# catree/InvCompCamTrack

Measured on AMD Instinct MI355X. Metric: aligned_Mpix_per_s (IC-GN, 1920x1080, 3-level pyramid), higher is better.
Workload: dtype f32; 1 GPU; R1080p-dense-se3: reference-faithful 6-DoF SE(3) tracker, 1920x1080, 3-level pyramid, 32400 8x8 patches tiling the frame, maxiter 10 fixed; points_per_pair_per_gpu=32400, psz=8, levels=3, maxiter=10, kernel_variant=0, collective=n/a, concurrent_streams=1, parallelism=single GPU

## Files before the change

include/ictr.h:

```cpp
#ifndef ICTR_H
#define ICTR_H

#include <stdbool.h>
#include <stddef.h>
#include <stdint.h>

#ifdef __cplusplus
extern "C" {
#endif

#define ICTR_OK 0
#define ICTR_ERR_INVALID 1
#define ICTR_ERR_NO_DEVICE 2
#define ICTR_ERR_HIP 3
#define ICTR_ERR_STATE 4

typedef struct ictr_optparam {
  int maxpttrack;
  int psz;
  int pszd2;
  int pszd2m3;
  int novals;
  int lv_f;
  int lv_l;
  bool donorm;
  bool dopatchnorm;
  int maxiter;
  float normdp_ratio;
  int verbosity;
} ictr_optparam;

int ictr_optparam_init(ictr_optparam *op, int lv_f, int lv_l, int psz, int maxiter, float normdp_ratio,
                       int donorm, int dopatchnorm, int maxpttrack, int verbosity);

const char *ictr_last_error(void);
int ictr_version(void);
int ictr_device_count(void);
int ictr_set_device(int device);
int ictr_stream_read_bandwidth(size_t bytes, int reps, double *gbps_out);
int ictr_debug_transpose_reduce(const float *vals, float *out, int *patch_of_lane, int *kind_of_lane,
                                int patches_per_wave );
int ictr_debug_wave_solve(const float *H36, const float *b6, int64_t n, int through_state, float *x6, int *rank,
                          int *nonzero, int *rowmap6, int *colmap6, float *lu36);
int ictr_debug_se3(const float *in, int64_t n, int log_not_exp, float *out);

typedef struct ictr_cam ictr_cam;
int ictr_cam_create(ictr_cam **out, int noscales, const float *fc, const float *cc, const int *wh, int padding);
void ictr_cam_destroy(ictr_cam *cam);
float ictr_cam_getfx(const ictr_cam *cam, int sc);
float ictr_cam_getfy(const ictr_cam *cam, int sc);
float ictr_cam_getcx(const ictr_cam *cam, int sc);
float ictr_cam_getcy(const ictr_cam *cam, int sc);
float ictr_cam_getswo(const ictr_cam *cam, int sc);
float ictr_cam_getsho(const ictr_cam *cam, int sc);
float ictr_cam_getsw(const ictr_cam *cam, int sc);
float ictr_cam_getsh(const ictr_cam *cam, int sc);

void ictr_se3_coeff_to_group_f(float *G12, const float *p6);
void ictr_se3_coeff_to_group_d(double *G12, const double *p6);
void ictr_se3_group_to_coeff_f(float *p6, const float *G12);
void ictr_se3_group_to_coeff_d(double *p6, const double *G12);
void ictr_solve6(const float *H36, const float *b6, float *x6);

typedef struct ictr_pyramid ictr_pyramid;
int ictr_pyramid_create(ictr_pyramid **out, const float *img, int w, int h, int lv_f, int getgrad, int pad);
int ictr_pyramid_create_device(ictr_pyramid **out, const float *img_dev, int w, int h, int lv_f, int getgrad,
                               int pad, void *hip_stream);
int ictr_pyramid_rebuild_device(ictr_pyramid *pyr, const float *img_dev, void *hip_stream);
int ictr_pyramid_rebuild(ictr_pyramid *pyr, const float *img, void *hip_stream);
int ictr_pyramid_create_from_host_planes(ictr_pyramid **out, const float **img_pyr, const float **dx_pyr,
                                         const float **dy_pyr, int w, int h, int lv_f, int pad);
void ictr_pyramid_destroy(ictr_pyramid *pyr);
int ictr_pyramid_levels(const ictr_pyramid *pyr);
int ictr_pyramid_level_dims(const ictr_pyramid *pyr, int level, int *sw, int *sh);
int ictr_pyramid_download(const ictr_pyramid *pyr, int level, int which, float *host_out);
const float *ictr_pyramid_device_plane(const ictr_pyramid *pyr, int level, int which);

int ictr_get_patch(const ictr_pyramid *pyr, int level, const float *mids, int64_t K, int psz, int dopatchnorm,
                   float *out);
int ictr_get_patch_grad(const ictr_pyramid *pyr, int level, const float *mids, int64_t K, int psz, int dopatchnorm,
                        float *out, float *out_dx, float *out_dy);
int ictr_ncc_score(const ictr_pyramid *pyr_back, const ictr_pyramid *pyr_ref, const ictr_pyramid *pyr_fwd, int level,
                   const float *mids, int64_t K, int psz, float w_back, float w_fwd, float *out_corr);

typedef struct ictr_pose ictr_pose;
int ictr_pose_create(ictr_pose **out, const ictr_cam *cam, const ictr_optparam *op);
void ictr_pose_destroy(ictr_pose *pose);
int ictr_pose_setpose_se3(ictr_pose *pose, const double *p_in, const double *meanshift3, double varval);
int ictr_pose_addpose_se3(ictr_pose *pose, const float *dp6);
int ictr_pose_subpose_se3(ictr_pose *pose, const float *dp6);
int ictr_pose_getpose_se3(const ictr_pose *pose, double *p_out6);
int ictr_pose_project_pt(const ictr_pose *pose, const float *pt3d, float *pt2d, int64_t nopoints, int sc);
int ictr_pose_project_pt_save_rotated(const ictr_pose *pose, const float *pt3d, float *pt3d_rot, float *pt2d,
                                      int64_t nopoints, int sc);
int ictr_pose_get_state(const ictr_pose *pose, float *p6, float *G12);

typedef struct ictr_odometer ictr_odometer;
int ictr_odometer_create(ictr_odometer **out, ictr_pose *pose, const ictr_optparam *op);
void ictr_odometer_destroy(ictr_odometer *odo);
int ictr_odometer_set3dpoints(ictr_odometer *odo, double *pt_in, int64_t nopoints_in);
int ictr_odometer_setpose(ictr_odometer *odo, const double *p_in, const ictr_pyramid *pyr_ref,
                          const ictr_pyramid *pyr_new);
int ictr_odometer_setpose_host(ictr_odometer *odo, const double *p_in, const float **img_ref,
                               const float **img_ref_dx, const float **img_ref_dy, const float **img_new);
int ictr_odometer_trackpose(ictr_odometer *odo, double *p_out);
const float *ictr_odometer_get2dpoints(ictr_odometer *odo);
int ictr_odometer_set_stream(ictr_odometer *odo, void *hip_stream);

typedef struct ictr_trace_rec {
  int level;
  int iter;
  float H[36];
  float b[6];
  float dp[6];
  float p[6];
} ictr_trace_rec;
int ictr_odometer_enable_trace(ictr_odometer *odo, int enable);
int ictr_odometer_trace(ictr_odometer *odo, ictr_trace_rec *out, int64_t capacity, int64_t *count);
int ictr_odometer_read_buffer(ictr_odometer *odo, int which, float *host_out, int64_t count);
int ictr_odometer_get_norm(const ictr_odometer *odo, double *meanshift3, double *varval);
#define ICTR_VARIANT_ANY_SIZE 0x2
#define ICTR_VARIANT_H_BY_SETUP 0x100
#define ICTR_VARIANT_LAUNCHES 0x2000
#define ICTR_VARIANT_ONE_LAUNCH 0x4000
#define ICTR_VARIANT_NO_GRAPH 0x8000
#define ICTR_VARIANT_SEPARATE_BEGIN 0x40000
#define ICTR_VARIANT_NO_TEAMS 0x80000
#define ICTR_VARIANT_NO_RESIDENT 0x200000
#define ICTR_VARIANT_DEBUG_MUTE 0x2000000
#define ICTR_VARIANT_GRAD_PLANES 0x8000000
#define ICTR_VARIANT_DYNAMIC_LOOP 0x10000000
#define ICTR_VARIANT_ALL                                                                                            \
  (ICTR_VARIANT_ANY_SIZE | ICTR_VARIANT_H_BY_SETUP | ICTR_VARIANT_LAUNCHES | ICTR_VARIANT_ONE_LAUNCH |              \
   ICTR_VARIANT_NO_GRAPH | ICTR_VARIANT_SEPARATE_BEGIN | ICTR_VARIANT_NO_TEAMS | ICTR_VARIANT_NO_RESIDENT |         \
   ICTR_VARIANT_DEBUG_MUTE | ICTR_VARIANT_GRAD_PLANES | ICTR_VARIANT_DYNAMIC_LOOP)
int ictr_odometer_set_variant(ictr_odometer *odo, int variant);
int ictr_odometer_set_team(ictr_odometer *odo, int target_points, int min_points, int max_points);
int ictr_odometer_set_robust(ictr_odometer *odo, int flags, float huber_k);
int ictr_odometer_last_path(const ictr_odometer *odo);
int ictr_odometer_last_team(const ictr_odometer *odo);

typedef struct ictr_batch ictr_batch;
int ictr_batch_create(ictr_batch **out, const ictr_cam *cam, const ictr_optparam *op, int64_t nproblems);
void ictr_batch_destroy(ictr_batch *b);
int ictr_batch_set_stream(ictr_batch *b, void *hip_stream);
int ictr_batch_set3dpoints(ictr_batch *b, int64_t problem, double *pt_in, int64_t nopoints_in);
int ictr_batch_set3dpoints_norm(ictr_batch *b, int64_t problem, double *pt_in, int64_t nopoints_in,
                                const double *meanshift3, double varval);
int ictr_batch_get_norm(const ictr_batch *b, int64_t problem, double *meanshift3, double *varval);
int ictr_batch_setpose(ictr_batch *b, int64_t problem, const double *p_in, const ictr_pyramid *pyr_ref,
                       const ictr_pyramid *pyr_new);
int ictr_batch_setpose_all(ictr_batch *b, const double *p_all, const ictr_pyramid *pyr_ref,
                           const ictr_pyramid *pyr_new);
int ictr_batch_track_async(ictr_batch *b);
int ictr_batch_get_poses(ictr_batch *b, double *p_out);
int ictr_batch_get_iterations(ictr_batch *b, int *iters);
int ictr_batch_get2dpoints(ictr_batch *b, int64_t problem, float *host_out );
int ictr_batch_set_variant(ictr_batch *b, int variant);
int ictr_batch_set_team(ictr_batch *b, int target_points, int min_points, int max_points);
#define ICTR_ROBUST_CLEAN 1
#define ICTR_ROBUST_COMPOSE 2
#define ICTR_ROBUST_HUBER 4
int ictr_batch_set_robust(ictr_batch *b, int flags, float huber_k);
int ictr_batch_read_buffer(ictr_batch *b, int64_t problem, int which, float *host_out, int64_t count);
int ictr_batch_set_timing(ictr_batch *b, int enable);
int ictr_batch_get_level_times(ictr_batch *b, float *ms_setup, float *ms_iters);
int ictr_batch_get_kernel_times(ictr_batch *b, float *ms_kernel);
int ictr_batch_get_first_iter_times(ictr_batch *b, float *ms_first);
int ictr_timebase_mark(void);
int ictr_batch_get_kernel_intervals(ictr_batch *b, float *start_ms, float *end_ms);
int ictr_batch_get_setup_intervals(ictr_batch *b, float *start_ms, float *end_ms);
int ictr_batch_last_path(const ictr_batch *b);
int ictr_batch_last_team(const ictr_batch *b);

int ictr_batch_enable_sharding(ictr_batch *b, int enable);
float *ictr_batch_reduction_buffer(ictr_batch *b);
int ictr_batch_set_reduction_buffer(ictr_batch *b, float *dev_ptr);
int ictr_batch_begin(ictr_batch *b);
int ictr_batch_level_allreduce_needed(ictr_batch *b);
int ictr_batch_level_accumulate(ictr_batch *b, int level);
int ictr_batch_level_finish(ictr_batch *b, int level);
int ictr_batch_iter_accumulate(ictr_batch *b, int level);
int ictr_batch_iter_finish(ictr_batch *b, int level);

int ictr_flow_gather(const void *disp_u, const void *disp_v, int is_f64, int fields_on_device, int H, int W,
                     const double *xy, int64_t K, double *out);
int ictr_extract_bil_patches(const double *img, int H, int W, int C, const double *pts, int64_t K, int pz, double *out);

typedef struct ictr_p2p ictr_p2p;
int ictr_p2p_create(ictr_p2p **out, int rank, int world, int64_t count );
int ictr_p2p_handle_bytes(void);
int ictr_p2p_local_handle(ictr_p2p *p, void *handle_out);
int ictr_p2p_connect(ictr_p2p *p, const void *all_handles);
int ictr_p2p_allreduce(ictr_p2p *p, float *dev_buf, int64_t count, void *hip_stream);
int ictr_p2p_error(ictr_p2p *p);
void ictr_p2p_destroy(ictr_p2p *p);
int ictr_batch_set_peer_exchange(ictr_batch *b, ictr_p2p *p);

int ictr_patchflow(const ictr_pyramid *pyr_a, const ictr_pyramid *pyr_b, const float *pts, int64_t K, int psz, int lv_f,
                   int lv_l, int maxiter, float eps, float *out, int *status, int *iters);
float ictr_patchflow_last_kernel_ms(void);

typedef struct ictr_icgn ictr_icgn;
#define ICTR_WARP_TRANSLATION 0
#define ICTR_WARP_SE2 1
#define ICTR_WARP_AFFINE 2
#define ICTR_WARP_HOMOGRAPHY 3
int ictr_icgn_create(ictr_icgn **out, int model, int w, int h, int lv_f, int lv_l, int maxiter, float eps,
                     const int *region_xywh, int64_t nproblems);
void ictr_icgn_destroy(ictr_icgn *g);
int ictr_icgn_set_stream(ictr_icgn *g, void *hip_stream);
int ictr_icgn_set_frames(ictr_icgn *g, int64_t problem, const ictr_pyramid *tmpl, const ictr_pyramid *cur);
int ictr_icgn_set_warp(ictr_icgn *g, int64_t problem, const double *M9);
int ictr_icgn_set_timing(ictr_icgn *g, int enable);
int ictr_icgn_run_async(ictr_icgn *g);
int ictr_icgn_get_results(ictr_icgn *g, double *M9_out, int *iters, float *last_dp);
int ictr_icgn_get_kernel_times(ictr_icgn *g, float *ms_per_level);
int ictr_icgn_set_rows(ictr_icgn *g, int row_lo, int row_hi);
int ictr_icgn_enable_sharding(ictr_icgn *g, int enable, float *red_dev );
int ictr_icgn_begin(ictr_icgn *g);
int ictr_icgn_hess_accumulate(ictr_icgn *g, int level);
int ictr_icgn_hess_finish(ictr_icgn *g, int level);
int ictr_icgn_iter_accumulate(ictr_icgn *g, int level);
int ictr_icgn_iter_finish(ictr_icgn *g, int level);

typedef struct ictr_sequence ictr_sequence;
int ictr_sequence_create(ictr_sequence **out, const ictr_cam *cam, const ictr_optparam *op, int64_t nworld, int stride);
void ictr_sequence_destroy(ictr_sequence *s);
int ictr_sequence_set_points(ictr_sequence *s, const double *pt3d);
int ictr_sequence_set_frames(ictr_sequence *s, const float *frames, int64_t nframes, int w, int h, int on_device);
int ictr_sequence_set_stream(ictr_sequence *s, void *hip_stream);
int ictr_sequence_set_robust(ictr_sequence *s, int flags, float huber_k);
int ictr_sequence_track_async(ictr_sequence *s, const double *p0);
int ictr_sequence_wait(ictr_sequence *s, double *poses, int32_t *npts, int32_t *iters);
int ictr_sequence_selection_hashes(const ictr_sequence *s, uint64_t *out);
int ictr_sequence_last_team(const ictr_sequence *s);

typedef struct ictr_ransac ictr_ransac;
int ictr_ransac_create(ictr_ransac **out, int64_t n, int64_t max_samples);
void ictr_ransac_destroy(ictr_ransac *r);
int ictr_ransac_set_points(ictr_ransac *r, const double *pt2d, const double *pt3d);
int ictr_ransac_run(ictr_ransac *r, const double *fc, const double *cc, double kc, int64_t nsamples, int64_t maxtrials,
                    double inlthresh, uint64_t seed, void *hip_stream);
int ictr_ransac_wait(ictr_ransac *r, int64_t *counts, double *R, double *t, double *p, uint64_t *inl_words,
                     int32_t *inl_cnt);
int ictr_ransac_samples(const ictr_ransac *r, int64_t *trial, int32_t *draws);
int ictr_ransac_chunk_size(const ictr_ransac *r);

#define ICTR_TRIANG_DLT 0
#define ICTR_TRIANG_GN 1
#define ICTR_TRIANG_LM 2
#define ICTR_TRIANG_DEPTH 3
#define ICTR_TRIANG_NONFINITE 1
#define ICTR_TRIANG_BEHIND 2
typedef struct ictr_triang_params {
  int32_t noiter;
  float minres;
  float damp_init, damp_fct, maxdamp;
} ictr_triang_params;
typedef struct ictr_triang ictr_triang;
int ictr_triang_create(ictr_triang **out, int64_t max_points, int64_t max_obs, int64_t max_frames);
void ictr_triang_destroy(ictr_triang *t);
int ictr_triang_set_cameras(ictr_triang *t, const float *P, int64_t nframes);
int ictr_triang_set_tracks(ictr_triang *t, int64_t n, const int64_t *offsets, const int32_t *view, const float *x,
                           const float *y);
int ictr_triang_run(ictr_triang *t, int mode, const ictr_triang_params *params, const float *init_pts,
                    const float *campos, const float *ptdir, void *hip_stream);
int ictr_triang_wait(ictr_triang *t, float *pts, float *cov, int32_t *iters, int32_t *status);
int ictr_triangulate_DLT(float *pt3d, float *AtAinv, const float *pt2d, const float *P, const int noviews);
int ictr_triangulate_full3D(float *pt3d, float *pt3d_cov, const float *pt2d, const float *P, const int noviews,
                            const int noiter, const float minres);
int ictr_triangulate_full3D_LM(float *pt3d, float *pt3d_cov, const float *pt2d, const float *P, const int noviews,
                               const int noiter, const float damp_init, const float damp_fct, const float minres,
                               const float maxdamp);
int ictr_triangulate_depthonly(float *pt3d, float *depth_cov, const float *campos, const float *ptdir, const float *pt2d,
                               const float *P, const int noviews, const int noiter, const float minres);

#ifdef __cplusplus
}
#endif
#endif
```

invcompcamtrack_amd/_lib.py:

```python
from __future__ import annotations

import ctypes as C
import os

import numpy as np

_HERE = os.path.dirname(os.path.abspath(__file__))
LIB_PATH = os.path.join(_HERE, "libictr_hip.so")

FP = C.POINTER(C.c_float)
DP = C.POINTER(C.c_double)
IP = C.POINTER(C.c_int)
FPP = C.POINTER(FP)
VP = C.c_void_p
I64 = C.c_int64


class IctrError(RuntimeError):
    pass


VARIANT_ANY_SIZE = 1 << 1
VARIANT_H_BY_SETUP = 1 << 8
VARIANT_LAUNCHES = 1 << 13
VARIANT_ONE_LAUNCH = 1 << 14
VARIANT_NO_GRAPH = 1 << 15
VARIANT_SEPARATE_BEGIN = 1 << 18
VARIANT_NO_TEAMS = 1 << 19
VARIANT_NO_RESIDENT = 1 << 21
VARIANT_DEBUG_MUTE = 1 << 25
VARIANT_GRAD_PLANES = 1 << 27
VARIANT_DYNAMIC_LOOP = 1 << 28
VARIANT_ALL = (VARIANT_ANY_SIZE | VARIANT_H_BY_SETUP | VARIANT_LAUNCHES | VARIANT_ONE_LAUNCH | VARIANT_NO_GRAPH
               | VARIANT_SEPARATE_BEGIN | VARIANT_NO_TEAMS | VARIANT_NO_RESIDENT | VARIANT_DEBUG_MUTE
               | VARIANT_GRAD_PLANES | VARIANT_DYNAMIC_LOOP)


class OptParam(C.Structure):
    _fields_ = [("maxpttrack", C.c_int), ("psz", C.c_int), ("pszd2", C.c_int), ("pszd2m3", C.c_int),
                ("novals", C.c_int), ("lv_f", C.c_int), ("lv_l", C.c_int), ("donorm", C.c_bool),
                ("dopatchnorm", C.c_bool), ("maxiter", C.c_int), ("normdp_ratio", C.c_float),
                ("verbosity", C.c_int)]


class TraceRec(C.Structure):
    _fields_ = [("level", C.c_int), ("iter", C.c_int), ("H", C.c_float * 36), ("b", C.c_float * 6),
                ("dp", C.c_float * 6), ("p", C.c_float * 6)]


class TriangParams(C.Structure):
    _fields_ = [("noiter", C.c_int32), ("minres", C.c_float), ("damp_init", C.c_float), ("damp_fct", C.c_float),
                ("maxdamp", C.c_float)]


SIGNATURES = {
    "ictr_optparam_init": (C.c_int, [C.POINTER(OptParam), C.c_int, C.c_int, C.c_int, C.c_int, C.c_float, C.c_int,
                                     C.c_int, C.c_int, C.c_int]),
    "ictr_last_error": (C.c_char_p, []),
    "ictr_version": (C.c_int, []),
    "ictr_device_count": (C.c_int, []),
    "ictr_set_device": (C.c_int, [C.c_int]),
    "ictr_stream_read_bandwidth": (C.c_int, [C.c_size_t, C.c_int, C.POINTER(C.c_double)]),
    "ictr_debug_transpose_reduce": (C.c_int, [FP, FP, IP, IP, C.c_int]),
    "ictr_debug_wave_solve": (C.c_int, [FP, FP, I64, C.c_int, FP, IP, IP, IP, IP, FP]),
    "ictr_debug_se3": (C.c_int, [FP, I64, C.c_int, FP]),
    "ictr_cam_create": (C.c_int, [C.POINTER(VP), C.c_int, FP, FP, IP, C.c_int]),
    "ictr_cam_destroy": (None, [VP]),
    "ictr_cam_getfx": (C.c_float, [VP, C.c_int]),
    "ictr_cam_getfy": (C.c_float, [VP, C.c_int]),
    "ictr_cam_getcx": (C.c_float, [VP, C.c_int]),
    "ictr_cam_getcy": (C.c_float, [VP, C.c_int]),
    "ictr_cam_getswo": (C.c_float, [VP, C.c_int]),
    "ictr_cam_getsho": (C.c_float, [VP, C.c_int]),
    "ictr_cam_getsw": (C.c_float, [VP, C.c_int]),
    "ictr_cam_getsh": (C.c_float, [VP, C.c_int]),
    "ictr_se3_coeff_to_group_f": (None, [FP, FP]),
    "ictr_se3_coeff_to_group_d": (None, [DP, DP]),
    "ictr_se3_group_to_coeff_f": (None, [FP, FP]),
    "ictr_se3_group_to_coeff_d": (None, [DP, DP]),
    "ictr_solve6": (None, [FP, FP, FP]),
    "ictr_pyramid_create": (C.c_int, [C.POINTER(VP), FP, C.c_int, C.c_int, C.c_int, C.c_int, C.c_int]),
    "ictr_pyramid_create_device": (C.c_int, [C.POINTER(VP), VP, C.c_int, C.c_int, C.c_int, C.c_int, C.c_int, VP]),
    "ictr_pyramid_rebuild_device": (C.c_int, [VP, VP, VP]),
    "ictr_pyramid_rebuild": (C.c_int, [VP, FP, VP]),
    "ictr_pyramid_create_from_host_planes": (C.c_int, [C.POINTER(VP), FPP, FPP, FPP, C.c_int, C.c_int, C.c_int,
                                                       C.c_int]),
    "ictr_pyramid_destroy": (None, [VP]),
    "ictr_pyramid_levels": (C.c_int, [VP]),
    "ictr_pyramid_level_dims": (C.c_int, [VP, C.c_int, IP, IP]),
    "ictr_pyramid_download": (C.c_int, [VP, C.c_int, C.c_int, FP]),
    "ictr_pyramid_device_plane": (VP, [VP, C.c_int, C.c_int]),
    "ictr_get_patch": (C.c_int, [VP, C.c_int, FP, I64, C.c_int, C.c_int, FP]),
    "ictr_get_patch_grad": (C.c_int, [VP, C.c_int, FP, I64, C.c_int, C.c_int, FP, FP, FP]),
    "ictr_ncc_score": (C.c_int, [VP, VP, VP, C.c_int, FP, I64, C.c_int, C.c_float, C.c_float, FP]),
    "ictr_pose_create": (C.c_int, [C.POINTER(VP), VP, C.POINTER(OptParam)]),
    "ictr_pose_destroy": (None, [VP]),
    "ictr_pose_setpose_se3": (C.c_int, [VP, DP, DP, C.c_double]),
    "ictr_pose_addpose_se3": (C.c_int, [VP, FP]),
    "ictr_pose_subpose_se3": (C.c_int, [VP, FP]),
    "ictr_pose_getpose_se3": (C.c_int, [VP, DP]),
    "ictr_pose_project_pt": (C.c_int, [VP, FP, FP, I64, C.c_int]),
    "ictr_pose_project_pt_save_rotated": (C.c_int, [VP, FP, FP, FP, I64, C.c_int]),
    "ictr_pose_get_state": (C.c_int, [VP, FP, FP]),
    "ictr_odometer_create": (C.c_int, [C.POINTER(VP), VP, C.POINTER(OptParam)]),
    "ictr_odometer_destroy": (None, [VP]),
    "ictr_odometer_set3dpoints": (C.c_int, [VP, DP, I64]),
    "ictr_odometer_setpose": (C.c_int, [VP, DP, VP, VP]),
    "ictr_odometer_setpose_host": (C.c_int, [VP, DP, FPP, FPP, FPP, FPP]),
    "ictr_odometer_trackpose": (C.c_int, [VP, DP]),
    "ictr_odometer_get2dpoints": (FP, [VP]),
    "ictr_odometer_set_stream": (C.c_int, [VP, VP]),
    "ictr_odometer_enable_trace": (C.c_int, [VP, C.c_int]),
    "ictr_odometer_trace": (C.c_int, [VP, C.POINTER(TraceRec), I64, C.POINTER(I64)]),
    "ictr_odometer_read_buffer": (C.c_int, [VP, C.c_int, FP, I64]),
    "ictr_odometer_get_norm": (C.c_int, [VP, DP, DP]),
    "ictr_odometer_set_variant": (C.c_int, [VP, C.c_int]),
    "ictr_odometer_set_team": (C.c_int, [VP, C.c_int, C.c_int, C.c_int]),
    "ictr_odometer_set_robust": (C.c_int, [VP, C.c_int, C.c_float]),
    "ictr_odometer_last_path": (C.c_int, [VP]),
    "ictr_odometer_last_team": (C.c_int, [VP]),
    "ictr_batch_create": (C.c_int, [C.POINTER(VP), VP, C.POINTER(OptParam), I64]),
    "ictr_batch_destroy": (None, [VP]),
    "ictr_batch_set_stream": (C.c_int, [VP, VP]),
    "ictr_batch_set3dpoints": (C.c_int, [VP, I64, DP, I64]),
    "ictr_batch_set3dpoints_norm": (C.c_int, [VP, I64, DP, I64, DP, C.c_double]),
    "ictr_batch_get_norm": (C.c_int, [VP, I64, DP, DP]),
    "ictr_batch_setpose": (C.c_int, [VP, I64, DP, VP, VP]),
    "ictr_batch_setpose_all": (C.c_int, [VP, DP, VP, VP]),
    "ictr_batch_track_async": (C.c_int, [VP]),
    "ictr_batch_get_poses": (C.c_int, [VP, DP]),
    "ictr_batch_get_iterations": (C.c_int, [VP, IP]),
    "ictr_batch_get2dpoints": (C.c_int, [VP, I64, FP]),
    "ictr_batch_set_variant": (C.c_int, [VP, C.c_int]),
    "ictr_batch_set_team": (C.c_int, [VP, C.c_int, C.c_int, C.c_int]),
    "ictr_batch_set_robust": (C.c_int, [VP, C.c_int, C.c_float]),
    "ictr_batch_read_buffer": (C.c_int, [VP, I64, C.c_int, FP, I64]),
    "ictr_batch_set_timing": (C.c_int, [VP, C.c_int]),
    "ictr_batch_get_level_times": (C.c_int, [VP, FP, FP]),
    "ictr_batch_get_kernel_times": (C.c_int, [VP, FP]),
    "ictr_batch_get_first_iter_times": (C.c_int, [VP, FP]),
    "ictr_batch_last_path": (C.c_int, [VP]),
    "ictr_batch_last_team": (C.c_int, [VP]),
    "ictr_timebase_mark": (C.c_int, []),
    "ictr_batch_get_kernel_intervals": (C.c_int, [VP, FP, FP]),
    "ictr_batch_get_setup_intervals": (C.c_int, [VP, FP, FP]),
    "ictr_batch_set_reduction_buffer": (C.c_int, [VP, VP]),
    "ictr_batch_enable_sharding": (C.c_int, [VP, C.c_int]),
    "ictr_batch_reduction_buffer": (VP, [VP]),
    "ictr_batch_begin": (C.c_int, [VP]),
    "ictr_batch_level_allreduce_needed": (C.c_int, [VP]),
    "ictr_batch_level_accumulate": (C.c_int, [VP, C.c_int]),
    "ictr_batch_level_finish": (C.c_int, [VP, C.c_int]),
    "ictr_batch_iter_accumulate": (C.c_int, [VP, C.c_int]),
    "ictr_batch_iter_finish": (C.c_int, [VP, C.c_int]),
    "ictr_flow_gather": (C.c_int, [VP, VP, C.c_int, C.c_int, C.c_int, C.c_int, DP, I64, DP]),
    "ictr_extract_bil_patches": (C.c_int, [DP, C.c_int, C.c_int, C.c_int, DP, I64, C.c_int, DP]),
    "ictr_p2p_create": (C.c_int, [C.POINTER(VP), C.c_int, C.c_int, I64]),
    "ictr_p2p_handle_bytes": (C.c_int, []),
    "ictr_p2p_local_handle": (C.c_int, [VP, VP]),
    "ictr_p2p_connect": (C.c_int, [VP, VP]),
    "ictr_p2p_allreduce": (C.c_int, [VP, VP, I64, VP]),
    "ictr_p2p_error": (C.c_int, [VP]),
    "ictr_p2p_destroy": (None, [VP]),
    "ictr_batch_set_peer_exchange": (C.c_int, [VP, VP]),
    "ictr_patchflow": (C.c_int, [VP, VP, FP, I64, C.c_int, C.c_int, C.c_int, C.c_int, C.c_float, FP, IP, IP]),
    "ictr_patchflow_last_kernel_ms": (C.c_float, []),
    "ictr_icgn_create": (C.c_int, [C.POINTER(VP), C.c_int, C.c_int, C.c_int, C.c_int, C.c_int, C.c_int, C.c_float, IP,
                                   I64]),
    "ictr_icgn_destroy": (None, [VP]),
    "ictr_icgn_set_stream": (C.c_int, [VP, VP]),
    "ictr_icgn_set_frames": (C.c_int, [VP, I64, VP, VP]),
    "ictr_icgn_set_warp": (C.c_int, [VP, I64, DP]),
    "ictr_icgn_set_timing": (C.c_int, [VP, C.c_int]),
    "ictr_icgn_run_async": (C.c_int, [VP]),
    "ictr_icgn_get_results": (C.c_int, [VP, DP, IP, FP]),
    "ictr_icgn_get_kernel_times": (C.c_int, [VP, FP]),
    "ictr_icgn_set_rows": (C.c_int, [VP, C.c_int, C.c_int]),
    "ictr_icgn_enable_sharding": (C.c_int, [VP, C.c_int, VP]),
    "ictr_icgn_begin": (C.c_int, [VP]),
    "ictr_icgn_hess_accumulate": (C.c_int, [VP, C.c_int]),
    "ictr_icgn_hess_finish": (C.c_int, [VP, C.c_int]),
    "ictr_icgn_iter_accumulate": (C.c_int, [VP, C.c_int]),
    "ictr_icgn_iter_finish": (C.c_int, [VP, C.c_int]),
    "ictr_sequence_create": (C.c_int, [C.POINTER(VP), VP, C.POINTER(OptParam), I64, C.c_int]),
    "ictr_sequence_destroy": (None, [VP]),
    "ictr_sequence_set_points": (C.c_int, [VP, DP]),
    "ictr_sequence_set_frames": (C.c_int, [VP, VP, I64, C.c_int, C.c_int, C.c_int]),
    "ictr_sequence_set_stream": (C.c_int, [VP, VP]),
    "ictr_sequence_set_robust": (C.c_int, [VP, C.c_int, C.c_float]),
    "ictr_sequence_track_async": (C.c_int, [VP, DP]),
    "ictr_sequence_wait": (C.c_int, [VP, DP, C.POINTER(C.c_int32), C.POINTER(C.c_int32)]),
    "ictr_sequence_selection_hashes": (C.c_int, [VP, C.POINTER(C.c_uint64)]),
    "ictr_sequence_last_team": (C.c_int, [VP]),
    "ictr_ransac_create": (C.c_int, [C.POINTER(VP), I64, I64]),
    "ictr_ransac_destroy": (None, [VP]),
    "ictr_ransac_set_points": (C.c_int, [VP, DP, DP]),
    "ictr_ransac_run": (C.c_int, [VP, DP, DP, C.c_double, I64, I64, C.c_double, C.c_uint64, VP]),
    "ictr_ransac_wait": (C.c_int, [VP, C.POINTER(I64), DP, DP, DP, C.POINTER(C.c_uint64), C.POINTER(C.c_int32)]),
    "ictr_ransac_samples": (C.c_int, [VP, C.POINTER(I64), C.POINTER(C.c_int32)]),
    "ictr_ransac_chunk_size": (C.c_int, [VP]),
    "ictr_triang_create": (C.c_int, [C.POINTER(VP), I64, I64, I64]),
    "ictr_triang_destroy": (None, [VP]),
    "ictr_triang_set_cameras": (C.c_int, [VP, FP, I64]),
    "ictr_triang_set_tracks": (C.c_int, [VP, I64, C.POINTER(I64), C.POINTER(C.c_int32), FP, FP]),
    "ictr_triang_run": (C.c_int, [VP, C.c_int, C.POINTER(TriangParams), FP, FP, FP, VP]),
    "ictr_triang_wait": (C.c_int, [VP, FP, FP, C.POINTER(C.c_int32), C.POINTER(C.c_int32)]),
    "ictr_triangulate_depthonly": (C.c_int, [FP, FP, FP, FP, FP, FP, C.c_int, C.c_int, C.c_float]),
}
SIGNATURES_REFERENCE_NAMES = {
    "ictr_triangulate_DLT": (C.c_int, [FP, FP, FP, FP, C.c_int]),
    "ictr_triangulate_full3D": (C.c_int, [FP, FP, FP, FP, C.c_int, C.c_int, C.c_float]),
    "ictr_triangulate_full3D_LM": (C.c_int, [FP, FP, FP, FP, C.c_int, C.c_int, C.c_float, C.c_float, C.c_float,
                                             C.c_float]),
}

_lib = None


def _preload_torch_hip_runtime():
    if os.environ.get("ICTR_SYSTEM_HIP") == "1":
        return None
    import sys
    tlib = None
    if "torch" in sys.modules:
        tlib = os.path.join(os.path.dirname(sys.modules["torch"].__file__), "lib", "libamdhip64.so")
    else:
        import importlib.util
        spec = importlib.util.find_spec("torch")
        if spec is not None and spec.origin:
            tlib = os.path.join(os.path.dirname(spec.origin), "lib", "libamdhip64.so")
    if tlib and os.path.exists(tlib):
        try:
            return C.CDLL(tlib, mode=C.RTLD_GLOBAL)
        except OSError:
            return None
    return None


def load():
    global _lib
    if _lib is not None:
        return _lib
    if not os.path.exists(LIB_PATH):
        raise IctrError(f"{LIB_PATH} not found: build it with `python -c 'import __graft_entry__ as g; g.build()'` "
                        "(hipcc --offload-arch=gfx950). There is no CPU fallback.")
    _preload_torch_hip_runtime()
    try:
        L = C.CDLL(LIB_PATH)
    except OSError as exc:
        raise IctrError(f"cannot load {LIB_PATH}: {exc}") from exc
    for name, (res, args) in list(SIGNATURES.items()) + list(SIGNATURES_REFERENCE_NAMES.items()):
        fn = getattr(L, name)
        fn.restype = res
        fn.argtypes = args
    _lib = L
    return L


def check(rc):
    if rc != 0:
        msg = load().ictr_last_error()
        raise IctrError(f"ictr error {rc}: {msg.decode() if msg else '?'}")


def fp(a):
    return a.ctypes.data_as(FP)


def dp(a):
    return a.ctypes.data_as(DP)


def f32c(a):
    return np.ascontiguousarray(a, dtype=np.float32)


def f64c(a):
    return np.ascontiguousarray(a, dtype=np.float64)
```

invcompcamtrack_amd/csrc/ictr_dev.h:

```cpp
#pragma once

#include <hip/hip_runtime.h>
#include <stdint.h>

#include "../../include/ictr.h"

namespace ictr {

constexpr int kBlock = 256;
constexpr int kWaves = kBlock / 64;
constexpr int kCoefStride = 16;
constexpr int kHUnique = 21;
constexpr int kRedStride = 27;
constexpr int kPartHStride = 32;
constexpr int kPartBStride = 8;
constexpr int kMaxGridX = 2048;

struct LevelCam {
  float fx, fy, cx, cy, swo, sho;
  int sw;
};

struct PlaneSet {
  const float *ref, *dx, *dy, *cur;
  const float *pack;
};

struct ProbState {
  float p[6];
  float G[12];
  float H[36];
  float LU[36];
  int piv[12];
  int luinfo[2];
  float b[6];
  float dp[6];
  float normdp;
  float normdp_init;
  int it;
  int active;
  int total_iters;
  int npts;
  unsigned reserved_;
  int pad_;
};

constexpr int kXchgMaxWorld = 16;
constexpr int kXchgPerPair = 64;
struct ResXchg {
  unsigned long long *peer[kXchgMaxWorld];
  unsigned long long *local;
  int rank, world;
  long long cap;
  unsigned *xseq;
};

struct DevTrace {
  ictr_trace_rec *rec;
  int *count;
  int capacity;
  int reserved_;
};

struct EngineDev {
  int B, M, P, n, nlev;
  int lv_f, lv_l, maxiter;
  float ratio;
  int dopatchnorm;
  int sharded;
  int otf;
  int robust;
  float huber_k;
  float *pt3d;
  float *pt3d_ref;
  float *pt2d;
  float *T, *Gx, *Gy;
  float *coef;
  ProbState *st;
  const PlaneSet *planes;
  float *partH;
  float *partb;
  float *red;
  DevTrace trace;
};

constexpr int kSeqBlock = 256;
constexpr int kSeqPPT = 16;
constexpr int kSeqChunk = kSeqBlock * kSeqPPT;
constexpr int kSeqFinish = 256;
struct SeqState {
  double pose[6];
  double G[12];
  double ms[3], varval;
  int npts;
  int pad_[3];
};
struct SeqArgs {
  const double *X;
  long long nw;
  int nblk;
  int stride, cap, M, n, donorm;
  int t;
  int tail;
  double fx, fy, cx, cy, w, h;
  double p0[6];
  ProbState *st;
  SeqState *ss;
  unsigned long long *mask;
  unsigned *cnt;
  int *sel;
  double *poses;
  unsigned long long *hash;
  int *npts_out, *iters_out;
  float *pt3d, *T, *Gx, *Gy, *coef;
};

constexpr int kRanHypBlock = 64;
constexpr int kRanScoreBlock = 256;
constexpr int kRanSelBlock = 1024;
constexpr int kRanMaxDraws = 1024;
struct RansacState {
  long long held;
  long long trials_used;
  long long kept;
  long long n_ic;
  int done;
  int pad_[3];
};
struct RansacArgs {
  const double *pts;
  int n, nwords;
  double fx, fy, cx, cy, kc, thr;
  unsigned long long seedmix;
  long long base;
  int k;
  long long nsamples, maxtrials;
  double *hyp;
  int *draws;
  int *status;
  unsigned *cnt;
  unsigned long long *words;
  RansacState *st;
  long long *o_trial;
  int *o_draws;
  double *o_R, *o_t;
  unsigned long long *o_words;
  int *o_cnt;
  int *o_keep;
  int *o_cntf;
};

struct PFLevel {
  const float *a, *ax, *ay, *b;
  int sw;
  float swo, sho, scale;
};
struct PFArgs {
  PFLevel lv[16];
  int lv_f, lv_l, P, maxiter, K;
  float eps2;
  float min_det;
  const float *pts;
  float *out;
  int *status;
  int *iters;
};

}
```

invcompcamtrack_amd/csrc/ictr_host.hip:

```cpp
#include <math.h>
#include <stdarg.h>
#include <stdio.h>
#include <stdlib.h>
#include <string.h>

#include <algorithm>
#include <atomic>
#include <deque>
#include <map>
#include <mutex>
#include <string>
#include <vector>

#include "ictr_dev.h"
#include "ictr_launch.h"
#include "se3_math.h"
#include "ictr_pose_hd.h"

using namespace ictr;

static thread_local std::string g_err;
int ictr::fail(int code, const char *fmt, ...) {
  char buf[512];
  va_list ap;
// ... 461 lines not shown
  if (e != hipSuccess) return fail(ICTR_ERR_HIP, "ncc_score failed: %s", hipGetErrorString(e));
  return ICTR_OK;
}

extern "C" int ictr_flow_gather(const void *disp_u, const void *disp_v, int is_f64, int fields_on_device, int H, int W,
                                const double *xy, int64_t K, double *out) {
  if (!disp_u || H < 1 || W < 1 || K < 0 || (K > 0 && (!xy || !out)))
    return fail(ICTR_ERR_INVALID, "flow_gather: bad arguments");
  if (K == 0) return ICTR_OK;
  if (int rc = need_device()) return rc;
  const size_t fb = (size_t)H * W * (is_f64 ? 8 : 4);
  char *d_f = nullptr;
  double *d_xy = nullptr;
  hipError_t e = hipMalloc((void **)&d_xy, sizeof(double) * 4 * K);
  const void *du = disp_u, *dv = disp_v;
  if (e == hipSuccess && !fields_on_device) {
    e = hipMalloc((void **)&d_f, fb * 2);
    if (e == hipSuccess) e = hipMemcpy(d_f, disp_u, fb, hipMemcpyHostToDevice);
    if (e == hipSuccess && disp_v) e = hipMemcpy(d_f + fb, disp_v, fb, hipMemcpyHostToDevice);
    du = d_f;
    dv = disp_v ? d_f + fb : nullptr;
  }
  if (e == hipSuccess) e = hipMemcpy(d_xy, xy, sizeof(double) * 2 * K, hipMemcpyHostToDevice);
  if (e == hipSuccess) {
    launch_flow_gather(du, dv, is_f64, H, W, d_xy, (int)K, d_xy + 2 * K, nullptr);
    e = hipMemcpy(out, d_xy + 2 * K, sizeof(double) * 2 * K, hipMemcpyDeviceToHost);
  }
  if (d_f) hipFree(d_f);
  if (d_xy) hipFree(d_xy);
  if (e != hipSuccess) return fail(ICTR_ERR_HIP, "flow_gather failed: %s", hipGetErrorString(e));
  return ICTR_OK;
}

extern "C" int ictr_extract_bil_patches(const double *img, int H, int W, int C, const double *pts, int64_t K, int pz,
                                        double *out) {
  const int half = pz / 2;
  if (!img || H < 2 || W < 2 || C < 1 || K < 0 || pz < 2 || (K > 0 && (!pts || !out)))
    return fail(ICTR_ERR_INVALID, "extract_bil_patches: bad arguments");
  for (int64_t k = 0; k < K; ++k) {
    const double fx = floor(pts[2 * k]), fy = floor(pts[2 * k + 1]);
    if (!(fx - half >= 0 && fy - half >= 0 && fx + half < W && fy + half < H))
      return fail(ICTR_ERR_INVALID, "extract_bil_patches: the window of point %lld leaves the image", (long long)k);
  }
  if (K == 0) return ICTR_OK;
  if (int rc = need_device()) return rc;
  const size_t ib = sizeof(double) * (size_t)H * W * C, ob = sizeof(double) * (size_t)K * 4 * half * half * C;
  double *d_img = nullptr, *d_pts = nullptr, *d_out = nullptr;
  hipError_t e = hipMalloc((void **)&d_img, ib);
  if (e == hipSuccess) e = hipMalloc((void **)&d_pts, sizeof(double) * 2 * K);
  if (e == hipSuccess) e = hipMalloc((void **)&d_out, ob);
  if (e == hipSuccess) e = hipMemcpy(d_img, img, ib, hipMemcpyHostToDevice);
  if (e == hipSuccess) e = hipMemcpy(d_pts, pts, sizeof(double) * 2 * K, hipMemcpyHostToDevice);
  if (e == hipSuccess) {
    launch_bil_patches(d_img, H, W, C, d_pts, (int)K, half, d_out, nullptr);
    e = hipMemcpy(out, d_out, ob, hipMemcpyDeviceToHost);
  }
  for (void *p_ : {(void *)d_img, (void *)d_pts, (void *)d_out})
    if (p_) hipFree(p_);
  if (e != hipSuccess) return fail(ICTR_ERR_HIP, "extract_bil_patches failed: %s", hipGetErrorString(e));
  return ICTR_OK;
}

struct ictr_pose {
  const ictr_cam *cam;
  const ictr_optparam *op;
  double meanshift[3] = {0, 0, 0};
  double varval = 0;
  float p[6] = {0, 0, 0, 0, 0, 0};
  float G[12] = {1, 0, 0, 0, 0, 1, 0, 0, 0, 0, 1, 0};
};

extern "C" int ictr_pose_create(ictr_pose **out, const ictr_cam *cam, const ictr_optparam *op) {
  if (!out || !cam || !op) return fail(ICTR_ERR_INVALID, "ictr_pose_create: NULL argument");
  ictr_pose *p = new ictr_pose;
  p->cam = cam;
  p->op = op;
  *out = p;
  return ICTR_OK;
}
extern "C" void ictr_pose_destroy(ictr_pose *pose) { delete pose; }
extern "C" int ictr_pose_setpose_se3(ictr_pose *pose, const double *p_in, const double *meanshift3, double varval) {
  if (!pose || !p_in) return fail(ICTR_ERR_INVALID, "setpose_se3: NULL argument");
  if (pose->op->donorm) {
    if (!meanshift3) return fail(ICTR_ERR_INVALID, "setpose_se3: donorm needs meanshift");
    pose->varval = varval;
    memcpy(pose->meanshift, meanshift3, sizeof(double) * 3);
  }
  host_setpose(pose->op->donorm, p_in, pose->meanshift, pose->varval, pose->p, pose->G);
  return ICTR_OK;
}
extern "C" int ictr_pose_addpose_se3(ictr_pose *pose, const float *dp) {
  if (!pose || !dp) return fail(ICTR_ERR_INVALID, "addpose_se3: NULL argument");
  for (int i = 0; i < 6; ++i) pose->p[i] += dp[i];
  se3_exp<float>(pose->G, pose->p);
  return ICTR_OK;
}
extern "C" int ictr_pose_subpose_se3(ictr_pose *pose, const float *dp) {
  if (!pose || !dp) return fail(ICTR_ERR_INVALID, "subpose_se3: NULL argument");
  for (int i = 0; i < 6; ++i) pose->p[i] -= dp[i];
  se3_exp<float>(pose->G, pose->p);
  return ICTR_OK;
}
extern "C" int ictr_pose_getpose_se3(const ictr_pose *pose, double *p_out) {
  if (!pose || !p_out) return fail(ICTR_ERR_INVALID, "getpose_se3: NULL argument");
  host_getpose(pose->op->donorm, pose->p, pose->G, pose->meanshift, pose->varval, p_out);
  return ICTR_OK;
}
extern "C" int ictr_pose_get_state(const ictr_pose *pose, float *p6, float *G12) {
  if (!pose) return fail(ICTR_ERR_INVALID, "pose is NULL");
  if (p6) memcpy(p6, pose->p, sizeof(float) * 6);
  if (G12) memcpy(G12, pose->G, sizeof(float) * 12);
  return ICTR_OK;
}

static int project_impl(const ictr_pose *pose, const float *pt3d, float *pt3d_rot, float *pt2d, int64_t nopoints,
                        int sc) {
  if (!pose || !pt3d || !pt2d || nopoints < 0 || sc < 0 || sc >= pose->cam->noscales)
    return fail(ICTR_ERR_INVALID, "project_pt: bad arguments");
  if (int rc = need_device()) return rc;
  const int M = pose->op->maxpttrack;
  if (nopoints > M) return fail(ICTR_ERR_INVALID, "project_pt: nopoints > maxpttrack");
  if (nopoints == 0) return ICTR_OK;
  float *d = nullptr;
  HIPCHK(hipMalloc((void **)&d, sizeof(float) * (size_t)(8 * M + 12)));
  float *d3 = d, *dr = d + 3 * M, *d2 = d + 6 * M, *dG = d + 8 * M;
  hipError_t e = hipMemcpy(d3, pt3d, sizeof(float) * 3 * M, hipMemcpyHostToDevice);
  if (e == hipSuccess) e = hipMemcpy(dG, pose->G, sizeof(float) * 12, hipMemcpyHostToDevice);
  if (e == hipSuccess) e = hipMemcpy(d2, pt2d, sizeof(float) * 2 * M, hipMemcpyHostToDevice);
  if (e == hipSuccess && pt3d_rot) e = hipMemcpy(dr, pt3d_rot, sizeof(float) * 3 * M, hipMemcpyHostToDevice);
  if (e == hipSuccess) {
    launch_project_generic(d3, pt3d_rot ? dr : nullptr, d2, (int)nopoints, M, dG, level_cam(pose->cam, sc), nullptr);
    e = hipMemcpy(pt2d, d2, sizeof(float) * 2 * M, hipMemcpyDeviceToHost);
    if (e == hipSuccess && pt3d_rot) e = hipMemcpy(pt3d_rot, dr, sizeof(float) * 3 * M, hipMemcpyDeviceToHost);
  }
  hipFree(d);
  if (e != hipSuccess) return fail(ICTR_ERR_HIP, "project_pt failed: %s", hipGetErrorString(e));
  return ICTR_OK;
}
extern "C" int ictr_pose_project_pt(const ictr_pose *pose, const float *pt3d, float *pt2d, int64_t nopoints, int sc) {
  return project_impl(pose, pt3d, nullptr, pt2d, nopoints, sc);
}
extern "C" int ictr_pose_project_pt_save_rotated(const ictr_pose *pose, const float *pt3d, float *pt3d_rot,
                                                 float *pt2d, int64_t nopoints, int sc) {
  if (!pt3d_rot) return fail(ICTR_ERR_INVALID, "project_pt_save_rotated: pt3d_rot is NULL");
  return project_impl(pose, pt3d, pt3d_rot, pt2d, nopoints, sc);
}

enum TrackForm : int {
  kFormLaunches = 0,
  kFormTrack1 = 1,
  kFormGraph = 2,
  kFormTrack1Begin = 3,
  kFormResident = 4,
};
struct TrackPlan {
  int form;
  int variant;
  int team, team_q;
  int project_here;
  int mute;
  ResidentGeom res;
  int setup_cpw[16], setup_gridx8[16];
};
struct Mailbox {
  unsigned long long *d = nullptr;
  size_t bytes = 0;
  unsigned epoch = 0;
};
struct ProbHost {
  int npts = 0;
  double meanshift[3] = {0, 0, 0};
  double varval = 0;
  float p[6] = {0, 0, 0, 0, 0, 0};
  float G[12] = {1, 0, 0, 0, 0, 1, 0, 0, 0, 0, 1, 0};
  const ictr_pyramid *ref = nullptr, *cur = nullptr;
  bool pose_set = false;
  int iters = 0;
};

struct ictr_batch {
  const ictr_cam *cam = nullptr;
  const ictr_optparam *op = nullptr;
  int B = 0, M = 0, n = 0, nlev = 0, P = 0;
  hipStream_t stream = nullptr;
  int variant = 0;
  int robust = 0;
  float huber_k = 0.0f;
  int sharded = 0;
  int gridx = 1;
  int cpw = 64, gridx8 = 1;
  bool trace_on = false;
  bool projected = false;
  float *d_pt3d = nullptr, *d_pt3d_ref = nullptr, *d_pt2d = nullptr, *d_T = nullptr, *d_Gx = nullptr,
        *d_Gy = nullptr, *d_coef = nullptr, *d_partH = nullptr, *d_partb = nullptr, *d_red = nullptr;
  ProbState *d_st = nullptr;
  PlaneSet *d_planes = nullptr;
  ictr_trace_rec *d_trace = nullptr;
  int *d_trace_count = nullptr;
  int trace_cap = 0;
  std::vector<ProbHost> probs;
  std::vector<ProbState> h_st;
  std::vector<PlaneSet> h_planes;
  std::vector<float> h_pt2d;
  std::vector<float> h_stage;
  bool timing = false;
  std::vector<hipEvent_t> ev;
  std::vector<char> ev_used;
  std::vector<hipEvent_t> evk;
  int evk_iters = 0;
  bool evk_valid = true;
  ResXchg xchg = {};
  unsigned *d_xseq = nullptr;
  int otf = 0;
  int maxpts = 0;
  TrackPlan plan = {};
  hipGraphExec_t gexec = nullptr;
  std::string gkey;
  hipStream_t cap_stream = nullptr;
  bool graph_broken = false;
  int phase_it = 0;
  float *d_red_own = nullptr;
  ProbState *h_st_pin = nullptr;
  ProbState *d_st_mirror = nullptr;
  char *h_up_pin = nullptr;
  Mailbox team_mail, res_mail;
  int team_target = 0;
  int team_lo = 128, team_hi = 8192;
  int *h_team_err = nullptr;
  int *d_team_err = nullptr;
  hipEvent_t done_ev = nullptr, up_ev = nullptr;
  bool done_valid = false, up_pending = false;
};

static size_t up_planes_offset(int B) { return (sizeof(ProbState) * (size_t)B + 15) / 16 * 16; }
int ictr::env_int(const char *name, int dflt) {
  const char *s = getenv(name);
  return s ? atoi(s) : dflt;
}

static void batch_free(ictr_batch *b) {
  if (!b) return;
  for (hipEvent_t e : b->ev) (void)hipEventDestroy(e);
  for (hipEvent_t e : b->evk) (void)hipEventDestroy(e);
  if (b->gexec) (void)hipGraphExecDestroy(b->gexec);
  if (b->cap_stream) (void)hipStreamDestroy(b->cap_stream);
  if (b->done_ev) (void)hipEventDestroy(b->done_ev);
  if (b->up_ev) (void)hipEventDestroy(b->up_ev);
  if (b->h_st_pin) (void)hipHostFree(b->h_st_pin);
  if (b->h_up_pin) (void)hipHostFree(b->h_up_pin);
  if (b->h_team_err) (void)hipHostFree(b->h_team_err);
  if (b->team_mail.d) (void)hipFree(b->team_mail.d);
  if (b->res_mail.d) (void)hipFree(b->res_mail.d);
  if (b->d_xseq) (void)hipFree(b->d_xseq);
  b->d_red = b->d_red_own;
  for (void *p : {(void *)b->d_pt3d, (void *)b->d_pt3d_ref, (void *)b->d_pt2d, (void *)b->d_T, (void *)b->d_Gx,
                  (void *)b->d_Gy, (void *)b->d_coef, (void *)b->d_partH, (void *)b->d_partb, (void *)b->d_red,
                  (void *)b->d_st, (void *)b->d_trace, (void *)b->d_trace_count})
    if (p) hipFree(p);
  delete b;
}

static int engine_variant(const ictr_batch *b) { return b->variant | (b->robust ? ICTR_VARIANT_ANY_SIZE : 0); }

static EngineDev engine_dev(const ictr_batch *b) {
  EngineDev e;
  memset(&e, 0, sizeof(e));
  e.B = b->B;
  e.M = b->M;
  e.P = b->P;
  e.n = b->n;
  e.nlev = b->nlev;
  e.lv_f = b->op->lv_f;
  e.lv_l = b->op->lv_l;
  e.maxiter = b->op->maxiter;
  e.ratio = b->op->normdp_ratio;
  e.dopatchnorm = b->op->dopatchnorm ? 1 : 0;
  e.sharded = b->sharded;
  e.otf = b->otf;
  e.robust = b->robust;
  e.huber_k = b->huber_k;
  e.pt3d = b->d_pt3d;
  e.pt3d_ref = b->d_pt3d_ref;
  e.pt2d = b->d_pt2d;
  e.T = b->d_T;
  e.Gx = b->d_Gx;
  e.Gy = b->d_Gy;
  e.coef = b->d_coef;
  e.st = b->d_st;
  e.planes = b->d_planes;
  e.partH = b->d_partH;
  e.partb = b->d_partb;
  e.red = b->d_red;
  e.trace.rec = b->trace_on ? b->d_trace : nullptr;
  e.trace.count = b->d_trace_count;
  e.trace.capacity = b->trace_cap;
  return e;
}

static int check_op(const ictr_optparam *op, const ictr_cam *cam) {
  if (op->psz < 1 || op->psz > 64) return fail(ICTR_ERR_INVALID, "psz must be 1..64");
  if (op->novals != op->psz * op->psz || op->pszd2 != op->psz / 2)
    return fail(ICTR_ERR_INVALID, "optparam derived fields inconsistent (use ictr_optparam_init)");
  if (op->lv_l < 0 || op->lv_f < op->lv_l || op->lv_f >= cam->noscales)
    return fail(ICTR_ERR_INVALID, "need 0 <= lv_l <= lv_f < cam.noscales");
  if (op->maxpttrack < 1) return fail(ICTR_ERR_INVALID, "maxpttrack must be >= 1");
  if (cam->padding < op->psz) return fail(ICTR_ERR_INVALID, "camera padding must be >= psz");
  return ICTR_OK;
}

extern "C" int ictr_batch_create(ictr_batch **out, const ictr_cam *cam, const ictr_optparam *op, int64_t nproblems) {
  if (!out || !cam || !op || nproblems < 1 || nproblems > 65535)
    return fail(ICTR_ERR_INVALID, "batch_create: bad arguments (1..65535 problems)");
  if (int rc = check_op(op, cam)) return rc;
  if (int rc = need_device()) return rc;
  ictr_batch *b = new ictr_batch;
  b->cam = cam;
  b->op = op;
  b->B = (int)nproblems;
  b->M = op->maxpttrack;
  b->P = op->psz;
  b->n = op->novals;
  b->nlev = op->lv_f + 1;
  b->team_target = env_int("ICTR_TEAM_TARGET", 0);
  b->team_lo = env_int("ICTR_TEAM_MINPTS", 128);
  b->team_hi = env_int("ICTR_TEAM_MAXPTS", 8192);
  const size_t B = b->B, M = b->M, n = b->n, L = b->nlev;
  const int ppw = (b->n <= 64 && 64 % b->n == 0) ? 64 / b->n : 1;
  const int64_t groups = (b->M + ppw - 1) / ppw;
  const int64_t cap = std::min<int64_t>(kMaxGridX, std::max<int64_t>(64, 2 * kMaxGridX / (int64_t)B));
  b->gridx = (int)std::min<int64_t>(std::max<int64_t>((groups + kWaves - 1) / kWaves, 1), cap);
  b->trace_cap = std::max(1, (int)L * std::max(1, op->maxiter));
  hipError_t e = hipSuccess;
  auto alloc = [&](void **p, size_t bytes) {
    if (e == hipSuccess) e = hipMalloc(p, bytes);
    if (e == hipSuccess) e = hipMemset(*p, 0, bytes);
  };
  alloc((void **)&b->d_pt3d, sizeof(float) * B * 3 * M);
  alloc((void **)&b->d_pt3d_ref, sizeof(float) * B * 3 * M);
  alloc((void **)&b->d_pt2d, sizeof(float) * B * L * 2 * M);
  alloc((void **)&b->d_T, sizeof(float) * B * M * n);
  alloc((void **)&b->d_Gx, sizeof(float) * B * M * n);
  alloc((void **)&b->d_Gy, sizeof(float) * B * M * n);
  alloc((void **)&b->d_coef, sizeof(float) * B * M * kCoefStride);
  alloc((void **)&b->d_partH, sizeof(float) * B * b->gridx * kPartHStride);
  alloc((void **)&b->d_partb, sizeof(float) * B * b->gridx * kPartBStride);
  alloc((void **)&b->d_red, sizeof(float) * B * kRedStride);
  alloc((void **)&b->d_st, up_planes_offset(B) + sizeof(PlaneSet) * B * L);
  if (e == hipSuccess) b->d_planes = reinterpret_cast<PlaneSet *>(reinterpret_cast<char *>(b->d_st) + up_planes_offset(B));
  alloc((void **)&b->d_trace, sizeof(ictr_trace_rec) * b->trace_cap);
  alloc((void **)&b->d_trace_count, sizeof(int));
  if (e == hipSuccess) e = hipHostMalloc((void **)&b->h_st_pin, sizeof(ProbState) * B, hipHostMallocDefault);
  if (e == hipSuccess)
    e = hipHostMalloc((void **)&b->h_up_pin, up_planes_offset(B) + sizeof(PlaneSet) * B * L, hipHostMallocDefault);
  if (e == hipSuccess && hipHostGetDevicePointer((void **)&b->d_st_mirror, b->h_st_pin, 0) != hipSuccess) {
    (void)hipGetLastError();
    b->d_st_mirror = nullptr;
  }
  if (e == hipSuccess) e = hipEventCreateWithFlags(&b->done_ev, hipEventDisableTiming);
  if (e == hipSuccess) e = hipEventCreateWithFlags(&b->up_ev, hipEventDisableTiming);
  if (e != hipSuccess) {
    batch_free(b);
    return fail(ICTR_ERR_HIP, "batch_create: device allocation failed: %s", hipGetErrorString(e));
  }
  b->d_red_own = b->d_red;
  b->probs.resize(B);
  b->h_st.resize(B);
  b->h_planes.resize(B * L);
  b->h_pt2d.assign(2 * M, 0.0f);
  b->h_stage.assign(3 * M, 0.0f);
  *out = b;
  return ICTR_OK;
}
extern "C" void ictr_batch_destroy(ictr_batch *b) { batch_free(b); }
extern "C" int ictr_batch_set_stream(ictr_batch *b, void *hip_stream) {
  if (!b) return fail(ICTR_ERR_INVALID, "batch is NULL");
  b->stream = (hipStream_t)hip_stream;
  return ICTR_OK;
}
extern "C" int ictr_batch_set_robust(ictr_batch *b, int flags, float huber_k) {
  if (!b) return fail(ICTR_ERR_INVALID, "batch is NULL");
  if (flags & ~(ICTR_ROBUST_CLEAN | ICTR_ROBUST_COMPOSE | ICTR_ROBUST_HUBER))
    return fail(ICTR_ERR_INVALID, "set_robust: unknown flag bits 0x%x", flags);
  if ((flags & ICTR_ROBUST_HUBER) && !(huber_k > 0.0f))
    return fail(ICTR_ERR_INVALID, "set_robust: the Huber threshold must be positive");
  b->robust = flags;
  b->huber_k = huber_k;
  return ICTR_OK;
}
extern "C" int ictr_batch_set_team(ictr_batch *b, int target_points, int min_points, int max_points) {
  if (!b) return fail(ICTR_ERR_INVALID, "batch is NULL");
  if (min_points < 0 || max_points < min_points)
    return fail(ICTR_ERR_INVALID, "set_team: need 0 <= min_points <= max_points");
  b->team_target = target_points;
  b->team_lo = min_points;
  b->team_hi = max_points;
  return ICTR_OK;
}
extern "C" int ictr_batch_set_peer_exchange(ictr_batch *b, ictr_p2p *p) {
  if (!b) return fail(ICTR_ERR_INVALID, "batch is NULL");
  if (!p) {
    memset(&b->xchg, 0, sizeof(b->xchg));
    return ICTR_OK;
  }
  ResXchg x;
  if (ictr_p2p_fill_xchg_(p, &x)) return fail(ICTR_ERR_STATE, "set_peer_exchange: the p2p object is not connected");
  if (x.cap < (long long)kXchgPerPair * b->B)
    return fail(ICTR_ERR_INVALID, "set_peer_exchange: the mailboxes hold %lld granules per rank, %d x %d needed", x.cap,
                kXchgPerPair, b->B);
  if (!b->d_xseq) HIPCHK(hipMalloc((void **)&b->d_xseq, sizeof(unsigned) * b->B));
  HIPCHK(hipMemsetAsync(b->d_xseq, 0, sizeof(unsigned) * b->B, b->stream));
  x.xseq = b->d_xseq;
  b->xchg = x;
  return ICTR_OK;
}

extern "C" int ictr_batch_set_variant(ictr_batch *b, int variant) {
  if (!b) return fail(ICTR_ERR_INVALID, "batch is NULL");
  if (variant & ~ICTR_VARIANT_ALL)
    return fail(ICTR_ERR_INVALID, "set_variant: unknown selection bits 0x%x (known: ICTR_VARIANT_ANY_SIZE, H_BY_SETUP, "
                                  "LAUNCHES, ONE_LAUNCH, NO_GRAPH, SEPARATE_BEGIN, NO_TEAMS, NO_RESIDENT, DEBUG_MUTE, "
                                  "GRAD_PLANES, DYNAMIC_LOOP = 0x%x)", variant & ~ICTR_VARIANT_ALL, ICTR_VARIANT_ALL);
  b->variant = variant;
  return ICTR_OK;
}

static int set3dpoints_impl(ictr_batch *b, int64_t problem, double *pt_in, int64_t nopoints_in, const double *given_ms,
                            double given_var) {
  if (!b || problem < 0 || problem >= b->B || nopoints_in < 0 || (nopoints_in > 0 && !pt_in))
    return fail(ICTR_ERR_INVALID, "set3dpoints: bad arguments");
  ProbHost &ph = b->probs[problem];
  const size_t M = b->M, n = b->n;
  HIPCHK(hipMemsetAsync(b->d_T + problem * M * n, 0, sizeof(float) * M * n, b->stream));
  HIPCHK(hipMemsetAsync(b->d_Gx + problem * M * n, 0, sizeof(float) * M * n, b->stream));
  HIPCHK(hipMemsetAsync(b->d_Gy + problem * M * n, 0, sizeof(float) * M * n, b->stream));
  HIPCHK(hipMemsetAsync(b->d_coef + problem * M * kCoefStride, 0, sizeof(float) * M * kCoefStride, b->stream));
  ph.meanshift[0] = ph.meanshift[1] = ph.meanshift[2] = 0;
  ph.varval = 0;
  ph.npts = (int)std::min<int64_t>(nopoints_in, b->M);
  ph.pose_set = false;
  const int np = ph.npts;
  double *p1 = pt_in, *p2 = pt_in + nopoints_in, *p3 = pt_in + 2 * nopoints_in;
  std::fill(b->h_stage.begin(), b->h_stage.end(), 0.0f);
  float *s = b->h_stage.data();
  if (b->op->donorm) {
    const double nd = (double)np;
    if (given_ms) {
      memcpy(ph.meanshift, given_ms, sizeof(double) * 3);
    } else {
      for (int i = 0; i < np; ++i) ph.meanshift[0] += p1[i];
      for (int i = 0; i < np; ++i) ph.meanshift[1] += p2[i];
      for (int i = 0; i < np; ++i) ph.meanshift[2] += p3[i];
      ph.meanshift[0] /= nd;
      ph.meanshift[1] /= nd;
      ph.meanshift[2] /= nd;
    }
    for (int i = 0; i < np; ++i) {
      p1[i] -= ph.meanshift[0];
      p2[i] -= ph.meanshift[1];
      p3[i] -= ph.meanshift[2];
      ph.varval += p1[i] * p1[i] + p2[i] * p2[i] + p3[i] * p3[i];
    }
    ph.varval /= nd;
    if (given_ms) ph.varval = given_var;
    for (int i = 0; i < np; ++i) {
      s[i] = (float)(p1[i] / ph.varval);
      s[i + M] = (float)(p2[i] / ph.varval);
      s[i + 2 * M] = (float)(p3[i] / ph.varval);
    }
  } else {
    for (int i = 0; i < np; ++i) {
      s[i] = (float)p1[i];
      s[i + M] = (float)p2[i];
      s[i + 2 * M] = (float)p3[i];
    }
  }
  HIPCHK(hipMemcpyAsync(b->d_pt3d + problem * 3 * M, s, sizeof(float) * 3 * M, hipMemcpyHostToDevice, b->stream));
  HIPCHK(hipStreamSynchronize(b->stream));
  return ICTR_OK;
}
extern "C" int ictr_batch_set3dpoints(ictr_batch *b, int64_t problem, double *pt_in, int64_t nopoints_in) {
  return set3dpoints_impl(b, problem, pt_in, nopoints_in, nullptr, 0.0);
}
extern "C" int ictr_batch_set3dpoints_norm(ictr_batch *b, int64_t problem, double *pt_in, int64_t nopoints_in,
                                           const double *meanshift3, double varval) {
  if (!meanshift3) return fail(ICTR_ERR_INVALID, "set3dpoints_norm: meanshift is NULL");
  return set3dpoints_impl(b, problem, pt_in, nopoints_in, meanshift3, varval);
}
extern "C" int ictr_batch_get_norm(const ictr_batch *b, int64_t problem, double *meanshift3, double *varval) {
  if (!b || problem < 0 || problem >= b->B) return fail(ICTR_ERR_INVALID, "get_norm: bad arguments");
  if (meanshift3) memcpy(meanshift3, b->probs[problem].meanshift, sizeof(double) * 3);
  if (varval) *varval = b->probs[problem].varval;
  return ICTR_OK;
}

extern "C" int ictr_batch_setpose(ictr_batch *b, int64_t problem, const double *p_in, const ictr_pyramid *pyr_ref,
                                  const ictr_pyramid *pyr_new) {
  if (!b || problem < 0 || problem >= b->B || !p_in || !pyr_ref || !pyr_new)
    return fail(ICTR_ERR_INVALID, "setpose: bad arguments");
  for (const ictr_pyramid *py : {pyr_ref, pyr_new}) {
    if (py->nlev < b->nlev || py->pad != b->cam->padding)
      return fail(ICTR_ERR_INVALID, "setpose: pyramid has %d levels / pad %d, engine needs %d / %d", py->nlev, py->pad,
                  b->nlev, b->cam->padding);
    for (int l = 0; l < b->nlev; ++l)
      if (py->sw[l] != (int)b->cam->sw[l] || py->sh[l] < (int)b->cam->sh[l])
        return fail(ICTR_ERR_INVALID, "setpose: pyramid level %d is %dx%d, camera expects %dx%d", l, py->sw[l],
                    py->sh[l], (int)b->cam->sw[l], (int)b->cam->sh[l]);
  }
  if (!pyr_ref->getgrad) return fail(ICTR_ERR_INVALID, "setpose: reference pyramid has no gradients");
  ProbHost &ph = b->probs[problem];
  host_setpose(b->op->donorm, p_in, ph.meanshift, ph.varval, ph.p, ph.G);
  ph.ref = pyr_ref;
  ph.cur = pyr_new;
  ph.pose_set = true;
  b->projected = false;
  return ICTR_OK;
}

extern "C" int ictr_batch_setpose_all(ictr_batch *b, const double *p_all, const ictr_pyramid *pyr_ref,
                                      const ictr_pyramid *pyr_new) {
  if (!b || !p_all) return fail(ICTR_ERR_INVALID, "setpose_all: bad arguments");
  for (int64_t k = 0; k < b->B; ++k)
    if (int rc = ictr_batch_setpose(b, k, p_all + 6 * k, pyr_ref, pyr_new)) return rc;
  return ICTR_OK;
}

static int cpw_forced() {
  const char *env = getenv("ICTR_CPW");
  const int v = env ? atoi(env) : 0;
  return v >= 1 && v <= 64 ? v : 0;
}
static int begin_prepare(ictr_batch *b) {
  if (int rc = check_op(b->op, b->cam)) return rc;
  if (b->op->maxpttrack != b->M || b->op->psz != b->P || b->op->lv_f + 1 != b->nlev)
    return fail(ICTR_ERR_STATE, "optparam maxpttrack/psz/lv_f changed after creation");
  b->done_valid = false;
  b->phase_it = 0;
  bool all_builder = true, any_image_only = false;
  if (b->timing) std::fill(b->ev_used.begin(), b->ev_used.end(), 0);
  int maxpts = 0;
  for (int i = 0; i < b->B; ++i) {
    const ProbHost &ph = b->probs[i];
    if (!ph.pose_set) return fail(ICTR_ERR_STATE, "problem %d: SetPose has not been called", i);
    ProbState &st = b->h_st[i];
    memset(&st, 0, sizeof(st));
    memcpy(st.p, ph.p, sizeof(st.p));
    memcpy(st.G, ph.G, sizeof(st.G));
    st.npts = ph.npts;
    st.normdp = st.normdp_init = 1e-10f;
    maxpts = std::max(maxpts, ph.npts);
    for (int l = 0; l < b->nlev; ++l) {
      PlaneSet &ps = b->h_planes[(size_t)i * b->nlev + l];
      ps.ref = ph.ref->img[l];
      ps.dx = ph.ref->dx[l];
      ps.dy = ph.ref->dy[l];
      ps.cur = ph.cur->img[l];
      ps.pack = ph.ref->pack[l];
    }
    if (!ph.ref->builder_made) all_builder = false;
    if (ph.ref->getgrad == 2) any_image_only = true;
  }
  if (any_image_only && !all_builder)
    return fail(ICTR_ERR_STATE, "a batch cannot mix image-only reference pyramids (getgrad = 2) with pyramids made from "
                                "caller-supplied planes: the setup kernel reads either the planes or the image, for all "
                                "problems of a launch");
  b->otf = !all_builder ? 0 : (any_image_only ? 2 : 1);

  b->maxpts = maxpts;
  {
    const int64_t total = (int64_t)std::max(maxpts, 1) * b->B;
    int cpw = 4;
    while (cpw < 64 && total / cpw > 32768) cpw *= 2;
    if (const int v = cpw_forced()) cpw = v;
    b->cpw = cpw;
    const int64_t chunks = ((int64_t)std::max(maxpts, 1) + cpw - 1) / cpw;
    const int64_t want = (chunks + kWaves - 1) / kWaves;
    const int64_t capx = std::max<int64_t>(1, (int64_t)b->gridx);
    b->gridx8 = (int)std::min<int64_t>(std::max<int64_t>(want, 1), capx);
    if (b->gridx8 >= 64)
      b->gridx8 = (int)std::min<int64_t>((b->gridx8 + 7) / 8 * 8, capx / 8 * 8);
  }
  if (b->otf == 2 && (b->P != 8 || b->robust || (engine_variant(b) & ICTR_VARIANT_ANY_SIZE)))
    return fail(ICTR_ERR_STATE, "a reference pyramid without gradient planes (getgrad = 2: gradients formed on the fly) is "
                                "served by the 8x8 setup kernel k_ref8 only: psz 8, no robustness option, variant bit 1 "
                                "clear (small problems then run the per-iteration launches instead of the one-launch "
                                "tracker)");
  return ICTR_OK;
}
static int begin_device(ictr_batch *b, bool project = true) {
  const int maxpts = project ? b->maxpts : 0;
  {
    const size_t nst = sizeof(ProbState) * b->B, npl = sizeof(PlaneSet) * b->h_planes.size();
    if (b->up_pending) HIPCHK(hipEventSynchronize(b->up_ev));
    const size_t off = up_planes_offset(b->B);
    memcpy(b->h_up_pin, b->h_st.data(), nst);
    memcpy(b->h_up_pin + off, b->h_planes.data(), npl);
    HIPCHK(hipMemcpyAsync(b->d_st, b->h_up_pin, off + npl, hipMemcpyHostToDevice, b->stream));
    HIPCHK(hipEventRecord(b->up_ev, b->stream));
    b->up_pending = true;
  }
  if (maxpts > 0) {
    LevelCam cams[16];
    for (int l = 0; l < b->nlev; ++l) cams[l] = level_cam(b->cam, l);
    launch_project_ref(engine_dev(b), cams, maxpts, b->stream);
  } else {
    HIPCHK(hipMemsetAsync(b->d_trace_count, 0, sizeof(int), b->stream));
  }
  HIPCHK(hipGetLastError());
  return ICTR_OK;
}
extern "C" int ictr_batch_begin(ictr_batch *b) {
  if (!b) return fail(ICTR_ERR_INVALID, "batch is NULL");
  if (int rc = begin_prepare(b)) return rc;
  if (int rc = begin_device(b)) return rc;
  b->projected = true;
  return ICTR_OK;
}

extern "C" int ictr_batch_enable_sharding(ictr_batch *b, int enable) {
  if (!b) return fail(ICTR_ERR_INVALID, "batch is NULL");
  b->sharded = enable ? 1 : 0;
  return ICTR_OK;
}
extern "C" float *ictr_batch_reduction_buffer(ictr_batch *b) { return b ? b->d_red : nullptr; }

static LevelLaunch level_launch(const ictr_batch *b, const TrackPlan *p, int level) {
  const bool res = p && p->form == kFormResident;
  LevelLaunch ll;
  ll.level = level;
  ll.variant = p ? p->variant : engine_variant(b);
  ll.gridx = b->gridx;
  ll.cpw = res ? p->setup_cpw[level] : b->cpw;
  ll.gridx8 = res ? p->setup_gridx8[level] : b->gridx8;
  return ll;
}
static int level_ok(ictr_batch *b, int level) {
  if (!b) return fail(ICTR_ERR_INVALID, "batch is NULL");
  if (!b->projected) return fail(ICTR_ERR_STATE, "ictr_batch_begin has not run since the last SetPose");
  if (level < b->op->lv_l || level > b->op->lv_f) return fail(ICTR_ERR_INVALID, "level out of range");
  return ICTR_OK;
}
extern "C" int ictr_batch_level_allreduce_needed(ictr_batch *b) {
  if (!b) return 1;
  return defer_h(engine_dev(b), engine_variant(b)) ? 0 : 1;
}
extern "C" int ictr_batch_level_accumulate(ictr_batch *b, int level) {
  if (int rc = level_ok(b, level)) return rc;
  b->phase_it = 0;
  launch_ref_level(engine_dev(b), level_cam(b->cam, level), level_launch(b, nullptr, level), true, b->stream);
  HIPCHK(hipGetLastError());
  return ICTR_OK;
}
extern "C" int ictr_batch_level_finish(ictr_batch *b, int level) {
  if (int rc = level_ok(b, level)) return rc;
  b->phase_it = 0;
  if (b->sharded) launch_level_finish(engine_dev(b), level_launch(b, nullptr, level), b->stream);
  HIPCHK(hipGetLastError());
  return ICTR_OK;
}
extern "C" int ictr_batch_iter_accumulate(ictr_batch *b, int level) {
  if (int rc = level_ok(b, level)) return rc;
  const bool tk = b->timing && b->phase_it < b->evk_iters && (int)b->evk.size() >= 2 * b->nlev * b->evk_iters;
  const EngineDev e = engine_dev(b);
  const LevelCam lc = level_cam(b->cam, level);
  const LevelLaunch ll = level_launch(b, nullptr, level);
  const int first = b->phase_it == 0;
  const int ke = 2 * (level * b->evk_iters + b->phase_it);
  launch_iter_main(e, lc, ll, first, b->stream, tk ? b->evk[ke] : nullptr, tk ? b->evk[ke + 1] : nullptr);
  if (tk && b->phase_it + 1 == std::min(b->op->maxiter, b->evk_iters)) b->ev_used[level] = 2;
  b->phase_it++;
  launch_iter_tail(e, ll, first, b->stream);
  HIPCHK(hipGetLastError());
  return ICTR_OK;
}
extern "C" int ictr_batch_iter_finish(ictr_batch *b, int level) {
  if (int rc = level_ok(b, level)) return rc;
  if (b->sharded) launch_iter_finish(engine_dev(b), level_launch(b, nullptr, level), b->phase_it == 1, b->stream);
  HIPCHK(hipGetLastError());
  return ICTR_OK;
}

int ictr::cu_count() {
  static std::atomic<int> n_cu[64];
  int dev = 0;
  if (hipGetDevice(&dev) != hipSuccess || dev < 0 || dev >= 64) {
    (void)hipGetLastError();
    dev = 0;
  }
  int v = n_cu[dev].load(std::memory_order_relaxed);
  if (v == 0) {
    if (hipDeviceGetAttribute(&v, hipDeviceAttributeMultiprocessorCount, dev) != hipSuccess || v < 1) {
      (void)hipGetLastError();
      v = 256;
    }
    n_cu[dev].store(v, std::memory_order_relaxed);
  }
  return v;
}

constexpr int kTrack1Waves = 8;
constexpr int kTeamMaxWorkgroups = 4096;

static int team_points(const ictr_batch *b) {
  if (b->team_target != 0) return b->team_target >= 8 ? b->team_target : 0;
  const int n = b->maxpts;
  const int upper = std::min(64, (n + 39) / 40), lower = (n + 159) / 160;
  const int fit = std::max(1, cu_count() / std::max(1, b->B));
  if (fit < lower && n <= 384) return 0;
  const int team = std::min(upper, std::max(lower, fit));
  return team < 2 ? 0 : (n + team - 1) / team;
}
static int track1_team(const ictr_batch *b, int *q) {
  if (b->P != 8 || (engine_variant(b) & ICTR_VARIANT_ANY_SIZE)) return 1;
  if (b->maxpts <= b->team_lo || b->maxpts > b->team_hi) return 1;
  if ((int64_t)b->nlev * (1 + std::max(0, b->op->maxiter)) >= 4000) return 1;
  const int target = team_points(b);
  if (target < 1) return 1;
  const int team = track1_team_size(b->maxpts, target);
  if (team < 2 || (int64_t)team * b->B > kTeamMaxWorkgroups) return 1;
  *q = track1_team_q(b->maxpts, target);
  return team;
}

static bool resident_plan(const ictr_batch *b, TrackPlan *p) {
  if (b->P != 8 || b->robust || b->sharded || b->op->dopatchnorm || b->op->maxiter < 1) return false;
  const bool xchg = b->xchg.world > 1;
  const bool big_batch = b->maxpts >= 500 && (int64_t)b->B * b->maxpts >= 48000;
  if (b->maxpts < 8193 && !xchg && !big_batch) return false;
  static const int max_slots = env_int("ICTR_RESIDENT_SLOTS", 1 << 20);
  for (int np : {16, 32}) {
    const int bpc = resident_blocks_per_cu(np);
    if (bpc < 1) continue;
    const int q = resident_points_per_workgroup(np);
    const int parts = std::max(1, (b->maxpts + q - 1) / q);
    const int64_t capacity = (int64_t)bpc * cu_count();
    const int slots = (int)std::min<int64_t>(std::min<int64_t>(b->B, max_slots), capacity / (parts + 1));
    if (slots < 1) continue;
    if (np == 16 && slots < b->B && !xchg) continue;
    if ((int64_t)((b->B + slots - 1) / slots) * b->op->maxiter >= 4000) return false;
    p->res = ResidentGeom{parts, slots, np};
    return true;
  }
  return false;
}
static void resident_setup_plan(const ictr_batch *b, bool forced_cpw, TrackPlan *p) {
  auto blocks_for = [&](int c) {
    const int64_t want = (((int64_t)std::max(b->maxpts, 1) + c - 1) / c + kWaves - 1) / kWaves;
    int g = (int)std::min<int64_t>(std::max<int64_t>(want, 1), std::max(b->gridx8, 1));
    if (g >= 64) g = std::min((g + 7) / 8 * 8, b->gridx8);
    return g;
  };
  const int64_t enough = 2 * (int64_t)cu_count() - 16;
  for (int sl = b->op->lv_l; sl <= b->op->lv_f; ++sl) {
    int cpw_l = b->cpw;
    if (!forced_cpw) {
      for (int c = b->B <= 2 ? 16 : 32; c > cpw_l; c /= 2)
        if ((int64_t)b->B * blocks_for(c) >= enough) {
          cpw_l = c;
          break;
        }
      if (sl > 0 && b->B >= 8 && cpw_l >= 16 && (int64_t)b->B * blocks_for(64) >= enough) cpw_l = 64;
    }
    p->setup_cpw[sl] = cpw_l;
    p->setup_gridx8[sl] = cpw_l != b->cpw ? blocks_for(cpw_l) : b->gridx8;
  }
}

static TrackPlan plan_tracking(const ictr_batch *b, bool begun) {
  TrackPlan p;
  memset(&p, 0, sizeof(p));
  const int v = engine_variant(b);
  p.variant = v;
  p.team = 1;
  p.mute = (v & ICTR_VARIANT_DEBUG_MUTE) ? 1 : 0;
  const bool resident = !(v & (ICTR_VARIANT_NO_RESIDENT | ICTR_VARIANT_LAUNCHES | ICTR_VARIANT_ANY_SIZE)) &&
                        resident_plan(b, &p);
  bool t1 = !b->sharded && !b->timing && !(v & ICTR_VARIANT_LAUNCHES) && b->xchg.world <= 1 && b->otf != 2 &&
            !(b->maxpts < 8193 && resident) && b->maxpts >= 1;
  if (t1) {
    int q = 0;
    const int team = (v & ICTR_VARIANT_NO_TEAMS) ? 1 : track1_team(b, &q);
    if (team > 1) {
      p.team = team;
      p.team_q = q;
    } else if ((size_t)b->maxpts * 64 > 128 * 1024) {
      t1 = false;
    } else if (!(v & ICTR_VARIANT_ONE_LAUNCH)) {
      const int limit = b->B >= 16 ? 384 : 192;
      t1 = (int64_t)b->maxpts * b->n <= (int64_t)limit * 64;
    }
  }
  if (t1) {
    p.res = ResidentGeom{0, 0, 0};
    const bool separate = begun || b->trace_on || !b->d_st_mirror || (v & ICTR_VARIANT_SEPARATE_BEGIN);
    const size_t up = sizeof(ProbState) * b->B + sizeof(PlaneSet) * b->h_planes.size();
    p.form = (!separate && up <= track1_blob_bytes()) ? kFormTrack1Begin : kFormTrack1;
    p.project_here = p.form == kFormTrack1 && !separate;
  } else if (resident) {
    p.form = kFormResident;
    resident_setup_plan(b, cpw_forced() != 0, &p);
  } else if (!b->sharded && !b->timing && !b->graph_broken && !(v & ICTR_VARIANT_NO_GRAPH) &&
             (int64_t)b->maxpts * b->B <= 65536) {
    p.form = kFormGraph;
  } else {
    p.form = kFormLaunches;
  }
  return p;
}

struct TeamFlight {
  hipEvent_t ev;
  int weight;
};
struct TeamDevice {
  std::deque<TeamFlight> flights;
  std::vector<hipEvent_t> events;
};
static std::mutex g_team_mu;
static std::map<int, TeamDevice> g_team_dev;
template <class F>
static int team_launch(int weight, hipStream_t s, F &&launch) {
  int dev = 0;
  if (hipGetDevice(&dev) != hipSuccess) {
    (void)hipGetLastError();
    dev = 0;
  }
  const int budget = 4 * cu_count() - 4;
  std::lock_guard<std::mutex> lk(g_team_mu);
  TeamDevice &d = g_team_dev[dev];
  while (!d.flights.empty() && hipEventQuery(d.flights.front().ev) == hipSuccess) {
    d.events.push_back(d.flights.front().ev);
    d.flights.pop_front();
  }
  (void)hipGetLastError();
  int load = 0;
  for (const TeamFlight &f : d.flights) load += f.weight;
  for (size_t i = 0; i < d.flights.size() && load + weight > budget; ++i) {
    HIPCHK(hipStreamWaitEvent(s, d.flights[i].ev, 0));
    load -= d.flights[i].weight;
  }
  hipEvent_t ev = nullptr;
  if (!d.events.empty()) {
    ev = d.events.back();
    d.events.pop_back();
  } else {
    HIPCHK(hipEventCreateWithFlags(&ev, hipEventDisableTiming));
  }
  const int rc = launch();
  hipError_t er = rc == ICTR_OK ? hipEventRecord(ev, s) : hipSuccess;
  if (rc != ICTR_OK || er != hipSuccess) {
    d.events.push_back(ev);
    if (rc != ICTR_OK) return rc;
    return fail(ICTR_ERR_HIP, "team_launch: hipEventRecord failed: %s", hipGetErrorString(er));
  }
  d.flights.push_back(TeamFlight{ev, weight});
  return ICTR_OK;
}

static double team_timeout_s() {
  const char *s = getenv("ICTR_TEAM_TIMEOUT_S");
  return s ? std::max(0.001, atof(s)) : 5.0;
}
static int exchange_prepare(ictr_batch *b, Mailbox *m, size_t need, const char *what, int mute, hipStream_t s,
                            Exchange *x) {
  if (need > m->bytes) {
    if (m->d) {
      HIPCHK(hipStreamSynchronize(s));
      HIPCHK(hipFree(m->d));
      *m = Mailbox{};
    }
    hipError_t e = hipExtMallocWithFlags((void **)&m->d, need, hipDeviceMallocUncached);
    if (e != hipSuccess) {
      (void)hipGetLastError();
      e = hipMalloc((void **)&m->d, need);
    }
    if (e == hipSuccess) e = hipMemsetAsync(m->d, 0, need, s);
    if (e != hipSuccess) return fail(ICTR_ERR_HIP, "%s mailbox allocation failed: %s", what, hipGetErrorString(e));
    m->bytes = need;
    m->epoch = 0;
  }
  if (!b->h_team_err) {
    HIPCHK(hipHostMalloc((void **)&b->h_team_err, sizeof(int), hipHostMallocDefault));
    *b->h_team_err = 0;
    HIPCHK(hipHostGetDevicePointer((void **)&b->d_team_err, b->h_team_err, 0));
  }
  m->epoch += 1;
  if (m->epoch >= (1u << 20)) {
    HIPCHK(hipMemsetAsync(m->d, 0, m->bytes, s));
    m->epoch = 1;
  }
  x->tag0 = m->epoch << 12;
  x->limit = (unsigned long long)(team_timeout_s() * 1e8);
  x->mail = m->d;
  x->err = b->d_team_err;
  x->mute = mute;
  return ICTR_OK;
}
static int team_prepare(ictr_batch *b, const TrackPlan &p, T1Team *tm) {
  memset(tm, 0, sizeof(*tm));
  tm->team = 1;
  if (p.team < 2) return ICTR_OK;
  tm->team = p.team;
  tm->q = p.team_q;
  return exchange_prepare(b, &b->team_mail, track1_team_mail_bytes(b->B, p.team), "team", p.mute, b->stream, &tm->x);
}
static int track1_launch(ictr_batch *b, const EngineDev &e, const TrackPlan &p, const void *blob, ProbState *host_st,
                         bool project_here) {
  LevelCam cams[16];
  for (int l = 0; l < b->nlev; ++l) cams[l] = level_cam(b->cam, l);
  T1Team tm;
  if (int rc = team_prepare(b, p, &tm)) return rc;
  auto launch = [&]() -> int {
    HIPCHK(launch_track1(e, cams, b->maxpts, kTrack1Waves, blob, host_st, b->stream, tm.team > 1 ? &tm : nullptr,
                         project_here, (p.variant & ICTR_VARIANT_ANY_SIZE) != 0));
    return ICTR_OK;
  };
  if (tm.team > 1) return team_launch(4 * (tm.team - 1), b->stream, launch);
  return launch();
}

static int launch_resident(ictr_batch *b, const EngineDev &e, const LevelCam &lc, const LevelLaunch &ll,
                           const TrackPlan &p, hipStream_t s) {
  const ResidentGeom &g = p.res;
  Exchange x;
  if (int rc = exchange_prepare(b, &b->res_mail, resident_mail_bytes(g.parts, g.slots), "resident", p.mute, s, &x)) return rc;
  const int bpc = std::max(1, std::min(4, resident_blocks_per_cu(g.np)));
  const int weight = g.slots * (g.parts + 1) * ((4 + bpc - 1) / bpc);
  return team_launch(weight, s, [&]() -> int {
    HIPCHK(launch_level_resident(e, lc, ll.level, g, tail_partials(e, ll), x, b->xchg.world > 1 ? &b->xchg : nullptr, s));
    return ICTR_OK;
  });
}

static int enqueue_level_kernels(ictr_batch *b, const EngineDev &e, const TrackPlan &p, hipStream_t s, bool events) {
  const int mi = b->op->maxiter;
  const bool resident = p.form == kFormResident;
  const bool tk = !resident && events && (int)b->evk.size() >= 2 * b->nlev * mi && mi <= b->evk_iters;
  b->evk_valid = tk;
  for (int sl = b->op->lv_f; sl >= b->op->lv_l; --sl) {
    const LevelCam lc = level_cam(b->cam, sl);
    if (events) HIPCHK(hipEventRecord(b->ev[3 * sl + 0], s));
    const LevelLaunch ll = level_launch(b, &p, sl);
    launch_ref_level(e, lc, ll, !resident, s);
    if (events) HIPCHK(hipEventRecord(b->ev[3 * sl + 1], s));
    if (resident) {
      if (int rc = launch_resident(b, e, lc, ll, p, s)) return rc;
    } else {
      for (int it = 0; it < mi; ++it) {
        const int ke = 2 * (sl * b->evk_iters + it);
        launch_iter_main(e, lc, ll, it == 0, s, tk ? b->evk[ke] : nullptr, tk ? b->evk[ke + 1] : nullptr);
        launch_iter_tail(e, ll, it == 0, s);
      }
    }
    if (events) {
      HIPCHK(hipEventRecord(b->ev[3 * sl + 2], s));
      b->ev_used[sl] = 1;
    }
  }
  return ICTR_OK;
}

template <class T>
static void key_put(std::string &k, const T &v) { k.append(reinterpret_cast<const char *>(&v), sizeof(T)); }
static std::string graph_key(const ictr_batch *b, const EngineDev &e, const TrackPlan &p) {
  static_assert(sizeof(EngineDev) == 14 * 4 + 14 * 8 + 2 * 4, "EngineDev must have no padding (graph_key)");
  static_assert(sizeof(TrackPlan) % 4 == 0 && sizeof(LevelCam) == 7 * 4, "plain ints and floats only");
  std::string k;
  key_put(k, e);
  key_put(k, p);
  for (int l = 0; l < b->nlev; ++l) key_put(k, level_cam(b->cam, l));
  for (int v : {b->cpw, b->gridx, b->gridx8}) key_put(k, v);
  return k;
}
static bool build_graph(ictr_batch *b, const EngineDev &e, const TrackPlan &p, const std::string &key) {
  if (b->gexec) {
    (void)hipGraphExecDestroy(b->gexec);
    b->gexec = nullptr;
  }
  b->gkey.clear();
  if (!b->cap_stream && hipStreamCreateWithFlags(&b->cap_stream, hipStreamNonBlocking) != hipSuccess) return false;
  if (hipStreamBeginCapture(b->cap_stream, hipStreamCaptureModeThreadLocal) != hipSuccess) return false;
  const int rc = enqueue_level_kernels(b, e, p, b->cap_stream, false);
  hipGraph_t g = nullptr;
  const hipError_t ec = hipStreamEndCapture(b->cap_stream, &g);
  bool ok = rc == ICTR_OK && ec == hipSuccess && g != nullptr;
  if (ok) ok = hipGraphInstantiate(&b->gexec, g, nullptr, nullptr, 0) == hipSuccess;
  if (g) (void)hipGraphDestroy(g);
  if (!ok) {
    (void)hipGetLastError();
    b->gexec = nullptr;
    return false;
  }
  b->gkey = key;
  return true;
}

static int enqueue_levels(ictr_batch *b) {
  const EngineDev e = engine_dev(b);
  TrackPlan &p = b->plan;
  if (b->xchg.world > 1 && p.form != kFormResident)
    return fail(ICTR_ERR_STATE, "a peer exchange is set (sharded resident form) but this tracking cannot run in the "
                                "resident-iteration form (8x8 patches, no robustness option, no patch normalisation, builder-"
                                "made pyramids, at most 4000 pair-rounds x iterations per level)");
  if (p.form == kFormTrack1)
    return track1_launch(b, e, p, nullptr, p.project_here ? b->d_st_mirror : nullptr, p.project_here != 0);
  if (p.form == kFormGraph) {
    const std::string key = graph_key(b, e, p);
    if ((b->gexec && key == b->gkey) || build_graph(b, e, p, key)) {
      HIPCHK(hipGraphLaunch(b->gexec, b->stream));
      return ICTR_OK;
    }
    b->graph_broken = true;
    p.form = kFormLaunches;
  }
  if (b->timing) std::fill(b->ev_used.begin(), b->ev_used.end(), 0);
  if (int rc = enqueue_level_kernels(b, e, p, b->stream, b->timing)) return rc;
  HIPCHK(hipGetLastError());
  return ICTR_OK;
}

static int track_enqueue(ictr_batch *b) {
  if (b->h_team_err && *(volatile int *)b->h_team_err) {
    HIPCHK(hipStreamSynchronize(b->stream));
    *(volatile int *)b->h_team_err = 0;
  }
  const bool begun = b->projected;
  if (!begun)
    if (int rc = begin_prepare(b)) return rc;
  b->plan = plan_tracking(b, begun);
  const TrackPlan &p = b->plan;
  if (!begun) {
    if (p.form != kFormTrack1Begin)
      if (int rc = begin_device(b, !p.project_here)) return rc;
    b->projected = true;
  }
  bool mirrored = false;
  if (p.form == kFormTrack1Begin) {
    const size_t nst = sizeof(ProbState) * b->B, npl = sizeof(PlaneSet) * b->h_planes.size();
    unsigned char blob[4096];
    memcpy(blob, b->h_st.data(), nst);
    memcpy(blob + nst, b->h_planes.data(), npl);
    if (int rc = track1_launch(b, engine_dev(b), p, blob, b->d_st_mirror, false)) return rc;
    mirrored = true;
  } else {
    if (int rc = enqueue_levels(b)) return rc;
    mirrored = p.project_here != 0;
  }
  if (!mirrored)
    HIPCHK(hipMemcpyAsync(b->h_st_pin, b->d_st, sizeof(ProbState) * b->B, hipMemcpyDeviceToHost, b->stream));
  HIPCHK(hipEventRecord(b->done_ev, b->stream));
  b->done_valid = true;
  return ICTR_OK;
}

extern "C" int ictr_batch_track_async(ictr_batch *b) {
  if (!b) return fail(ICTR_ERR_INVALID, "batch is NULL");
  if (b->sharded) return fail(ICTR_ERR_STATE, "sharded batches are driven phase by phase (see ictr.h)");
  b->projected = false;
  return track_enqueue(b);
}
static int team_error_check(const ictr_batch *b) {
  if (b->h_team_err && *(volatile int *)b->h_team_err)
    return fail(ICTR_ERR_HIP, "%s: a workgroup waited in vain for its peers' partial sums (in-launch exchange timed out "
                              "after %.3f s; are all workgroups of the launch resident?); the results of this tracking "
                              "are invalid",
                b->plan.form == kFormResident ? "resident-iteration form (k_level_resident)" : "one-launch tracker, team form (k_track1_p8)",
                team_timeout_s());
  return ICTR_OK;
}
static int batch_wait(ictr_batch *b) {
  if (b->done_valid)
    HIPCHK(hipEventSynchronize(b->done_ev));
  else
    HIPCHK(hipStreamSynchronize(b->stream));
  return team_error_check(b);
}

extern "C" int ictr_batch_set_timing(ictr_batch *b, int enable) {
  if (!b) return fail(ICTR_ERR_INVALID, "batch is NULL");
  if (enable && b->ev.empty()) {
    b->ev.resize(3 * b->nlev);
    b->ev_used.assign(b->nlev, 0);
    for (auto &e : b->ev) HIPCHK(hipEventCreate(&e));
    b->evk_iters = std::max(1, b->op->maxiter);
    b->evk.resize((size_t)2 * b->nlev * b->evk_iters);
    for (auto &e : b->evk) HIPCHK(hipEventCreate(&e));
  }
  b->timing = enable != 0;
  return ICTR_OK;
}
extern "C" int ictr_batch_get_level_times(ictr_batch *b, float *ms_setup, float *ms_iters) {
  if (!b || !ms_setup || !ms_iters) return fail(ICTR_ERR_INVALID, "get_level_times: NULL argument");
  if (b->ev.empty()) return fail(ICTR_ERR_STATE, "timing was never enabled");
  if (int rc = batch_wait(b)) return rc;
  for (int l = 0; l < b->nlev; ++l) {
    ms_setup[l] = ms_iters[l] = 0.0f;
    if (b->ev_used[l] != 1) continue;
    HIPCHK(hipEventElapsedTime(&ms_setup[l], b->ev[3 * l + 0], b->ev[3 * l + 1]));
    HIPCHK(hipEventElapsedTime(&ms_iters[l], b->ev[3 * l + 1], b->ev[3 * l + 2]));
  }
  return ICTR_OK;
}
extern "C" int ictr_batch_get_kernel_times(ictr_batch *b, float *ms_kernel) {
  if (!b || !ms_kernel) return fail(ICTR_ERR_INVALID, "get_kernel_times: NULL argument");
  if (b->evk.empty()) return fail(ICTR_ERR_STATE, "timing was never enabled");
  if (int rc = batch_wait(b)) return rc;
  const int mi = std::min(b->op->maxiter, b->evk_iters);
  for (int l = 0; l < b->nlev; ++l) {
    ms_kernel[l] = 0.0f;
    if (!b->ev_used[l] || !b->evk_valid) continue;
    for (int it = 0; it < mi; ++it) {
      float ms = 0.0f;
      HIPCHK(hipEventElapsedTime(&ms, b->evk[2 * (l * b->evk_iters + it)], b->evk[2 * (l * b->evk_iters + it) + 1]));
      ms_kernel[l] += ms;
    }
  }
  return ICTR_OK;
}
extern "C" int ictr_batch_get_first_iter_times(ictr_batch *b, float *ms_first) {
  if (!b || !ms_first) return fail(ICTR_ERR_INVALID, "get_first_iter_times: NULL argument");
  if (b->evk.empty()) return fail(ICTR_ERR_STATE, "timing was never enabled");
  if (int rc = batch_wait(b)) return rc;
  for (int l = 0; l < b->nlev; ++l) {
    ms_first[l] = 0.0f;
    if (!b->ev_used[l] || !b->evk_valid || b->op->maxiter < 1) continue;
    HIPCHK(hipEventElapsedTime(&ms_first[l], b->evk[2 * (l * b->evk_iters)], b->evk[2 * (l * b->evk_iters) + 1]));
  }
  return ICTR_OK;
}
static hipEvent_t g_timebase = nullptr;
extern "C" int ictr_timebase_mark(void) {
  if (int rc = need_device()) return rc;
  if (!g_timebase) HIPCHK(hipEventCreate(&g_timebase));
  HIPCHK(hipDeviceSynchronize());
  HIPCHK(hipEventRecord(g_timebase, nullptr));
  HIPCHK(hipEventSynchronize(g_timebase));
  return ICTR_OK;
}
extern "C" int ictr_batch_get_kernel_intervals(ictr_batch *b, float *start_ms, float *end_ms) {
  if (!b || !start_ms || !end_ms) return fail(ICTR_ERR_INVALID, "get_kernel_intervals: NULL argument");
  if (b->evk.empty()) return fail(ICTR_ERR_STATE, "timing was never enabled");
  if (!g_timebase) return fail(ICTR_ERR_STATE, "ictr_timebase_mark has not been called");
  if (int rc = batch_wait(b)) return rc;
  const int mi = std::min(b->op->maxiter, b->evk_iters);
  for (int l = 0; l < b->nlev; ++l)
    for (int it = 0; it < b->evk_iters; ++it) {
      const int k = l * b->evk_iters + it;
      start_ms[k] = end_ms[k] = 0.0f;
      if (!b->ev_used[l] || !b->evk_valid || it >= mi) continue;
      HIPCHK(hipEventElapsedTime(&start_ms[k], g_timebase, b->evk[2 * k]));
      HIPCHK(hipEventElapsedTime(&end_ms[k], g_timebase, b->evk[2 * k + 1]));
    }
  return ICTR_OK;
}
extern "C" int ictr_batch_get_setup_intervals(ictr_batch *b, float *start_ms, float *end_ms) {
  if (!b || !start_ms || !end_ms) return fail(ICTR_ERR_INVALID, "get_setup_intervals: NULL argument");
  if (b->ev.empty()) return fail(ICTR_ERR_STATE, "timing was never enabled");
  if (!g_timebase) return fail(ICTR_ERR_STATE, "ictr_timebase_mark has not been called");
  if (int rc = batch_wait(b)) return rc;
  for (int l = 0; l < b->nlev; ++l) {
    start_ms[l] = end_ms[l] = 0.0f;
    if (b->ev_used[l] != 1) continue;
    HIPCHK(hipEventElapsedTime(&start_ms[l], g_timebase, b->ev[3 * l + 0]));
    HIPCHK(hipEventElapsedTime(&end_ms[l], g_timebase, b->ev[3 * l + 1]));
  }
  return ICTR_OK;
}
extern "C" int ictr_batch_last_path(const ictr_batch *b) { return b ? b->plan.form : -1; }
extern "C" int ictr_batch_last_team(const ictr_batch *b) {
  return b ? ((b->plan.form == kFormTrack1 || b->plan.form == kFormTrack1Begin) ? b->plan.team : 1) : -1;
}
extern "C" int ictr_batch_set_reduction_buffer(ictr_batch *b, float *dev_ptr) {
  if (!b) return fail(ICTR_ERR_INVALID, "batch is NULL");
  b->d_red = dev_ptr ? dev_ptr : b->d_red_own;
  return ICTR_OK;
}

static int batch_fetch_state(ictr_batch *b) {
  if (b->done_valid) {
    HIPCHK(hipEventSynchronize(b->done_ev));
    memcpy(b->h_st.data(), b->h_st_pin, sizeof(ProbState) * b->B);
  } else {
    HIPCHK(hipMemcpyAsync(b->h_st.data(), b->d_st, sizeof(ProbState) * b->B, hipMemcpyDeviceToHost, b->stream));
    HIPCHK(hipStreamSynchronize(b->stream));
  }
  if (int rc = team_error_check(b)) return rc;
  for (int i = 0; i < b->B; ++i) {
    memcpy(b->probs[i].p, b->h_st[i].p, sizeof(float) * 6);
    memcpy(b->probs[i].G, b->h_st[i].G, sizeof(float) * 12);
    b->probs[i].iters = b->h_st[i].total_iters;
  }
  return ICTR_OK;
}
extern "C" int ictr_batch_get_poses(ictr_batch *b, double *p_out) {
  if (!b || !p_out) return fail(ICTR_ERR_INVALID, "get_poses: NULL argument");
  if (int rc = batch_fetch_state(b)) return rc;
  for (int i = 0; i < b->B; ++i) {
    const ProbHost &ph = b->probs[i];
    host_getpose(b->op->donorm, ph.p, ph.G, ph.meanshift, ph.varval, p_out + 6 * i);
  }
  return ICTR_OK;
}
extern "C" int ictr_batch_get_iterations(ictr_batch *b, int *iters) {
  if (!b || !iters) return fail(ICTR_ERR_INVALID, "get_iterations: NULL argument");
  for (int i = 0; i < b->B; ++i) iters[i] = b->probs[i].iters;
  return ICTR_OK;
}
extern "C" int ictr_batch_get2dpoints(ictr_batch *b, int64_t problem, float *host_out) {
  if (!b || problem < 0 || problem >= b->B || !host_out) return fail(ICTR_ERR_INVALID, "get2dpoints: bad arguments");
  if (!b->projected)
    if (int rc = ictr_batch_begin(b)) return rc;
  const size_t M = b->M;
  HIPCHK(hipMemcpyAsync(host_out, b->d_pt2d + ((size_t)problem * b->nlev + b->op->lv_l) * 2 * M, sizeof(float) * 2 * M,
                        hipMemcpyDeviceToHost, b->stream));
  HIPCHK(hipStreamSynchronize(b->stream));
  return ICTR_OK;
}

struct ictr_odometer {
// ... 505 lines not shown
```

invcompcamtrack_amd/csrc/ictr_kernels.hip:

```cpp
#include <algorithm>

#include <hip/hip_ext.h>

#include "ictr_dev.h"
#include "ictr_launch.h"
#include "ictr_devfn.h"
#include "se3_math.h"

namespace ictr {

struct AllCams {
  LevelCam lc[16];
};

__global__ __launch_bounds__(kBlock) void k_project_ref(EngineDev e, AllCams cams) {
  const int b = blockIdx.y;
  const ProbState &st = e.st[b];
  const int i = blockIdx.x * kBlock + threadIdx.x;
  if (i == 0 && b == 0 && e.trace.count != nullptr) *e.trace.count = 0;
  if (i >= st.npts) return;
  const float *p3 = e.pt3d + (size_t)b * 3 * e.M;
  float *p3r = e.pt3d_ref + (size_t)b * 3 * e.M;
  const float X = p3[i], Y = p3[i + e.M], Z = p3[i + 2 * e.M];
  const float tx = st.G[0] * X + st.G[1] * Y + st.G[2] * Z + st.G[3];
// ... 497 lines not shown
    const float X = p3[ip], Y = p3[ip + M], Z = p3[ip + 2 * M];
    const float4 *c4 = reinterpret_cast<const float4 *>(coefb + (size_t)ip * kCoefStride);
    const float4 q0 = c4[0], q1 = c4[1], q2 = c4[2];
    const float tx = G[0] * X + G[1] * Y + G[2] * Z + G[3];
    const float ty = G[4] * X + G[5] * Y + G[6] * Z + G[7];
    const float tz = G[8] * X + G[9] * Y + G[10] * Z + G[11];
    const float mx = (tx / tz) * lc.fx + lc.cx;
    const float my = (ty / tz) * lc.fy + lc.cy;
    const bool vis = pv && in_view(mx, my, lc.swo, lc.sho);
    const Taps tp = make_taps(vis ? mx : 1.0f, vis ? my : 1.0f, 4);
    const int base_v = tp.row0 * sw + tp.col0;
    const int so_v = (base_v - sw - 1) * 4;
    {
      float4 *r4 = reinterpret_cast<float4 *>(rec + lane * kRec);
      r4[0] = make_float4(tp.w1, tp.w0, tp.w3, tp.w2);
      r4[1] = make_float4(q0.z, q0.w, q1.x, q1.y);
      r4[2] = make_float4(q2.x, q2.y, q2.z, q2.w);
      r4[3] = make_float4(q0.x, q1.w, vis ? 1.0f : 0.0f, 0.0f);
    }
    __builtin_amdgcn_fence(__ATOMIC_RELEASE, "wavefront");
    __builtin_amdgcn_wave_barrier();
    __builtin_amdgcn_fence(__ATOMIC_ACQUIRE, "wavefront");

    const int nsteps = (cnt + kU - 1) / kU;
    auto issue = [&](PatchLoads<kU> &L, int sidx) {
#pragma unroll
      for (int u = 0; u < kU; ++u) {
        const int jraw = sidx + u * nsteps;
        const int jj = min(jraw, cnt - 1);
        constexpr int aux = 2;
        L.rec[u] = (jraw < cnt) ? jj : 64;
        const int so = rlane(so_v, jj);
        const int po4 = (i0 + jj) * 256;
        const int off_cd = ((lane >> 3) * sw + (lane & 7)) * 4, off_ab = off_cd + sw * 4;
        L.t[u] = __builtin_bit_cast(float, __builtin_amdgcn_raw_buffer_load_b32(rT, lane * 4, po4, aux));
        L.gx[u] = __builtin_bit_cast(float, __builtin_amdgcn_raw_buffer_load_b32(rGx, lane * 4, po4, aux));
        L.gy[u] = __builtin_bit_cast(float, __builtin_amdgcn_raw_buffer_load_b32(rGy, lane * 4, po4, aux));
        L.cur[u].ab = __builtin_bit_cast(f32x2_a4, __builtin_amdgcn_raw_buffer_load_b64(rcur, off_ab, so, 0));
        L.cur[u].top = __builtin_bit_cast(f32x2_a4, __builtin_amdgcn_raw_buffer_load_b64(rcur, off_cd, so, 0));
      }
    };
    auto reduce = [&](const PatchLoads<kU> &L) {
#pragma unroll
      for (int u = 0; u < kU; ++u) {
        asm volatile("" : "+v"(acc01), "+v"(acc23), "+v"(acc45) : : "memory");
        const float4 *r4 = rec4 + L.rec[u] * 4;
        const float4 wv = r4[0], qx = r4[1], qy = r4[2], qz = r4[3];
        float inew = wv.y * L.cur[u].ab.y + wv.x * L.cur[u].ab.x + wv.w * L.cur[u].top.y + wv.z * L.cur[u].top.x;
        if constexpr (PN) inew -= wave_sum(inew) / 64.0f;
        const float gx = L.gx[u], gy = L.gy[u];
        const float r = (L.t[u] - inew) * qz.z;
        const f32x2_t g2 = {gx * r, gy * r}, gr2 = {g2.x, g2.x}, hr2 = {g2.y, g2.y};
        acc01 = __builtin_elementwise_fma(g2, (f32x2_t){qz.x, qz.y}, acc01);
        acc23 = __builtin_elementwise_fma(gr2, (f32x2_t){qx.x, qx.y},
                                          __builtin_elementwise_fma(hr2, (f32x2_t){qy.x, qy.y}, acc23));
        acc45 = __builtin_elementwise_fma(gr2, (f32x2_t){qx.z, qx.w},
                                          __builtin_elementwise_fma(hr2, (f32x2_t){qy.z, qy.w}, acc45));
      }
    };
    PatchLoads<kU> A, B;
    issue(A, 0);
    for (int sidx = 0; sidx < nsteps; sidx += 2) {
      if (sidx + 1 < nsteps) issue(B, sidx + 1);
      reduce(A);
      if (sidx + 2 < nsteps) issue(A, sidx + 2);
      if (sidx + 1 < nsteps) reduce(B);
    }
    __builtin_amdgcn_fence(__ATOMIC_RELEASE, "wavefront");
    __builtin_amdgcn_wave_barrier();
  }

  const float acc[6] = {acc01.x, acc01.y, acc23.x, acc23.y, acc45.x, acc45.y};
#pragma unroll
  for (int k = 0; k < 6; ++k) {
    const float v = wave_sum(acc[k]);
    if (lane == 0) sW[wave][k] = v;
  }
  __syncthreads();
  if (threadIdx.x < 6) {
    const float v = (sW[0][threadIdx.x] + sW[1][threadIdx.x]) + (sW[2][threadIdx.x] + sW[3][threadIdx.x]);
    e.partb[((size_t)b * gridDim.x + blockIdx.x) * kPartBStride + threadIdx.x] = v;
  }
}

typedef float f32x4_a4 __attribute__((ext_vector_type(4), aligned(4)));
typedef const f32x4_a4 __attribute__((address_space(1))) *gconst_f32x4a;
struct TapLoadsOTF {
  f32x4_a4 r0, r1;
  f32x2_a4 up, dn;
};
__device__ __forceinline__ TapLoadsOTF taps_issue_otf(gconst_f32 img_at_base, int loff, int sw) {
  TapLoadsOTF t;
  gconst_f32 q = img_at_base + loff;
  t.r0 = *reinterpret_cast<gconst_f32x4a>(q - 2);
  t.r1 = *reinterpret_cast<gconst_f32x4a>(q - sw - 2);
  t.up = *reinterpret_cast<gconst_f32x2>(q + sw - 1);
  t.dn = *reinterpret_cast<gconst_f32x2>(q - 2 * sw - 1);
  return t;
}
__device__ __forceinline__ void taps_blend_otf(const TapLoadsOTF &t, float w0, float w1, float w2, float w3, bool interior,
                                               int ix, int iy, int w, int h, float &tv, float &gx, float &gy) {
  const float a = t.r0[2], b = t.r0[1], c = t.r1[2], d = t.r1[1];
  tv = w0 * a + w1 * b + w2 * c + w3 * d;
  float xa = t.r0[3] - t.r0[1], xb = t.r0[2] - t.r0[0], xc = t.r1[3] - t.r1[1], xd = t.r1[2] - t.r1[0];
  float ya = t.up.y - t.r1[2], yb = t.up.x - t.r1[1], yc = t.r0[2] - t.dn.y, yd = t.r0[1] - t.dn.x;
  if (!interior) {
    const bool colA = ix >= 0 && ix < w, colB = ix - 1 >= 0 && ix - 1 < w, rowA = iy >= 0 && iy < h, rowC = iy - 1 >= 0 && iy - 1 < h;
    const bool dxA = ix >= 1 && ix <= w - 2, dxB = ix - 1 >= 1 && ix - 1 <= w - 2;
    const bool dyA = iy >= 1 && iy <= h - 2, dyC = iy - 1 >= 1 && iy - 1 <= h - 2;
    xa = (dxA && rowA) ? xa : 0.0f;
    xb = (dxB && rowA) ? xb : 0.0f;
    xc = (dxA && rowC) ? xc : 0.0f;
    xd = (dxB && rowC) ? xd : 0.0f;
    ya = (dyA && colA) ? ya : 0.0f;
    yb = (dyA && colB) ? yb : 0.0f;
    yc = (dyC && colA) ? yc : 0.0f;
    yd = (dyC && colB) ? yd : 0.0f;
  }
  gx = w0 * xa + w1 * xb + w2 * xc + w3 * xd;
  gy = w0 * ya + w1 * yb + w2 * yc + w3 * yd;
}

template <int I, int N, class Fn>
__device__ __forceinline__ void res_static_for(Fn &&fn) {
  if constexpr (I < N) {
    fn(std::integral_constant<int, I>{});
    res_static_for<I + 1, N>(fn);
  }
}

template <int kU>
struct RefLoads {
  TapLoads4 p4[kU];
  TapLoadsOTF o[kU];
  int rec[kU];
  int vis[kU];
  int inner[kU];
  int tx[kU], ty[kU];
};

template <bool PN, int kU, bool PK, bool OTF = false, bool ST = false>
__global__ __launch_bounds__(kBlock) void k_ref8(EngineDev e, LevelCam lc, int level, int cpw) {
  static_assert(PK != OTF, "the taps come from either the packed planes or the image plane");
  static_assert(!ST || (OTF && !PN), "the static form exists for on-the-fly gradients without patch normalisation");
  __shared__ __attribute__((aligned(16))) float sRec[kWaves][64 * kRec];
  __shared__ float sW[kWaves][kPartHStride];
  const int b = blockIdx.y;
  const ProbState &st = e.st[b];
  const int npts = st.npts;
  const int M = e.M;
  const PlaneSet pl = e.planes[b * e.nlev + level];
  const float *__restrict__ pt2d = e.pt2d + ((size_t)b * e.nlev + level) * 2 * M;
  const float *__restrict__ p3r = e.pt3d_ref + (size_t)b * 3 * M;
  float *T = e.T + (size_t)b * M * 64;
  float *Gx = e.Gx + (size_t)b * M * 64;
  float *Gy = e.Gy + (size_t)b * M * 64;
  float *coefb = e.coef + (size_t)b * M * kCoefStride;
  gconst_f32 pref = (gconst_f32)pl.ref;
  gconst_f32x4 ppack = (gconst_f32x4)pl.pack;
  const int sw = lc.sw;
  const int wl = (int)lc.swo, hl = (int)lc.sho, padl = (sw - wl) / 2;

  const int lane = threadIdx.x & 63;
  const int wave = __builtin_amdgcn_readfirstlane(threadIdx.x >> 6);
  const int loff = (lane >> 3) * sw + (lane & 7);
  float *rec = sRec[wave];
  const float4 *rec4 = reinterpret_cast<const float4 *>(rec);

  float accH = 0.0f;

  const int nchunks = (npts + cpw - 1) / cpw;
  for (int ch = xcd_band_block(blockIdx.x, gridDim.x) * kWaves + wave; ch < nchunks; ch += gridDim.x * kWaves) {
    const int i0 = ch * cpw;
    const int cnt = min(cpw, npts - i0);
    const bool pv = lane < cnt;
    const int ip = i0 + (pv ? lane : 0);
    const float mx = pt2d[ip], my = pt2d[ip + M];
    const bool vis = pv && in_view(mx, my, lc.swo, lc.sho);
    const Taps tp = make_taps(vis ? mx : 1.0f, vis ? my : 1.0f, 4);
#ifndef ICTR_REF8_TOUCH
#define ICTR_REF8_TOUCH 6
#endif
    constexpr int kTouch = ST ? ICTR_REF8_TOUCH : 0;
    float touch[kTouch > 0 ? kTouch : 1];
    if constexpr (kTouch > 0) {
      const int kBig = 1 << 28;
      const int rmin = row_min_dpp(vis ? tp.row0 : kBig), rmax = -row_min_dpp(vis ? -tp.row0 : kBig);
      const int cmin = row_min_dpp(vis ? tp.col0 : kBig), cmax = -row_min_dpp(vis ? -tp.col0 : kBig);
      const int li = lane & 15, nrows = rmax - rmin + 11;
      const unsigned long long a_first = (unsigned long long)(pl.ref + (size_t)(rmin - 2 + li) * sw + (cmin - 2));
      const unsigned long long a_last = (unsigned long long)(pl.ref + (size_t)(rmin - 2 + li) * sw + (cmax + 8)) + 3;
      const unsigned long long a0 = a_first & ~127ull;
      const int nl = (int)(((a_last | 127ull) - a0 + 1) >> 7);
      const bool box = rmin < kBig && nrows <= 16 && li < nrows && nl <= kTouch;
#pragma unroll
      for (int k = 0; k < kTouch; ++k) {
        touch[k] = 0.0f;
        if (box && k < nl) touch[k] = *(gconst_f32)(a0 + 128ull * k);
      }
    }
    float cx[6], cy[6];
    float4 *c4 = reinterpret_cast<float4 *>(coefb + (size_t)ip * kCoefStride);
    if (vis) {
      sd_coefs(p3r[ip], p3r[ip + M], p3r[ip + 2 * M], lc.fx, lc.fy, cx, cy);
      c4[0] = make_float4(cx[0], cx[1], cx[2], cx[3]);
      c4[1] = make_float4(cx[4], cx[5], cy[0], cy[1]);
      c4[2] = make_float4(cy[2], cy[3], cy[4], cy[5]);
    } else {
      const float4 a0 = c4[0], a1 = c4[1], a2 = c4[2];
      cx[0] = a0.x; cx[1] = a0.y; cx[2] = a0.z; cx[3] = a0.w; cx[4] = a1.x; cx[5] = a1.y;
      cy[0] = a1.z; cy[1] = a1.w; cy[2] = a2.x; cy[3] = a2.y; cy[4] = a2.z; cy[5] = a2.w;
    }
    const int base_v = tp.row0 * sw + tp.col0;
    const int vis_v = vis ? 1 : 0;
    const int tx_v = tp.col0 - padl, ty_v = tp.row0 - padl;
    {
      float4 *r4 = reinterpret_cast<float4 *>(rec + lane * kRec);
      r4[0] = make_float4(tp.w0, tp.w1, tp.w2, tp.w3);
      r4[1] = make_float4(cx[0], cx[1], cx[2], cx[3]);
      r4[2] = make_float4(cx[4], cx[5], cy[0], cy[1]);
      r4[3] = make_float4(cy[2], cy[3], cy[4], cy[5]);
    }
    __builtin_amdgcn_fence(__ATOMIC_RELEASE, "wavefront");
    __builtin_amdgcn_wave_barrier();
    __builtin_amdgcn_fence(__ATOMIC_ACQUIRE, "wavefront");

    float sxx_v = 0.0f, sxy_v = 0.0f, syy_v = 0.0f;
    const int nsteps = (cnt + kU - 1) / kU;
    auto issue = [&](RefLoads<kU> &L, int sidx) {
#pragma unroll
      for (int u = 0; u < kU; ++u) {
        const int jraw = sidx + u * nsteps;
        const int jj = min(jraw, cnt - 1);
        L.rec[u] = (jraw < cnt) ? jj : -1;
        const int base = rlane(base_v, jj);
        L.vis[u] = rlane(vis_v, jj);
        if (L.vis[u]) {
          if constexpr (OTF) {
            L.tx[u] = rlane(tx_v, jj);
            L.ty[u] = rlane(ty_v, jj);
            L.inner[u] = (L.tx[u] >= 2 && L.tx[u] + 7 <= wl - 2 && L.ty[u] >= 2 && L.ty[u] + 7 <= hl - 2) ? 1 : 0;
            L.o[u] = taps_issue_otf(pref + base, loff, sw);
          } else {
            L.p4[u] = taps_issue4(ppack + base, loff, sw, lane);
          }
        }
      }
    };
    auto patch_sums = [&](float gx, float gy, int j) {
      const float sxx = wave_sum_dpp(gx * gx), sxy = wave_sum_dpp(gx * gy), syy = wave_sum_dpp(gy * gy);
      const bool mine = lane == j;
      sxx_v = mine ? sxx : sxx_v;
      sxy_v = mine ? sxy : sxy_v;
      syy_v = mine ? syy : syy_v;
    };
    auto reduce = [&](const RefLoads<kU> &L) {
#pragma unroll
      for (int u = 0; u < kU; ++u) {
        if (L.rec[u] < 0 || !L.vis[u]) continue;
        float gx, gy;
        {
          const float4 w = rec4[L.rec[u] * 4 + 0];
          float t;
          if constexpr (OTF) {
            taps_blend_otf(L.o[u], w.x, w.y, w.z, w.w, L.inner[u] != 0, L.tx[u] + (lane & 7), L.ty[u] + (lane >> 3), wl, hl,
                           t, gx, gy);
          } else {
            t = taps_blend4(L.p4[u], 0, w.x, w.y, w.z, w.w, lane);
            gx = taps_blend4(L.p4[u], 1, w.x, w.y, w.z, w.w, lane);
            gy = taps_blend4(L.p4[u], 2, w.x, w.y, w.z, w.w, lane);
          }
          if constexpr (PN) t -= wave_sum(t) / 64.0f;
          const size_t po = (size_t)(i0 + L.rec[u]) * 64;
          __builtin_nontemporal_store(t, T + po + lane);
          __builtin_nontemporal_store(gx, Gx + po + lane);
          __builtin_nontemporal_store(gy, Gy + po + lane);
        }
        patch_sums(gx, gy, L.rec[u]);
      }
    };
    if constexpr (ST) {
      const int inner_v = (tx_v >= 2 && tx_v + 7 <= wl - 2 && ty_v >= 2 && ty_v + 7 <= hl - 2) ? 1 : 0;
      if constexpr (kTouch > 0) {
#pragma unroll
        for (int k = 0; k < kTouch; ++k) asm volatile("" ::"v"(touch[k]));
      }
      for (int g0 = 0; g0 < cnt; g0 += 16) {
        const unsigned vmask = (unsigned)(__builtin_amdgcn_ballot_w64(vis) >> g0) & 0xffffu;
#ifndef ICTR_REF8_D
#define ICTR_REF8_D 3
#endif
        constexpr int kD = ICTR_REF8_D;
        TapLoadsOTF W3[kD];
        auto issue_s = [&](int j) {
#if defined(ICTR_REF8_ABL) && (ICTR_REF8_ABL & 2)
          if ((vmask >> j) & 1u) W3[j % kD] = taps_issue_otf(pref + 2 * sw + 2 + (rlane(base_v, g0 + j) & 7), loff, sw);
#else
          if ((vmask >> j) & 1u) W3[j % kD] = taps_issue_otf(pref + rlane(base_v, g0 + j), loff, sw);
#endif
        };
        res_static_for<0, kD>([&](auto jc) { issue_s(decltype(jc)::value); });
        TrAcc<16> accS, accX;
        tr_for_each_patch<16, 0>([&](auto jc) {
          constexpr int j = decltype(jc)::value;
          float gx = 0.0f, gy = 0.0f;
          if ((vmask >> j) & 1u) {
            const float4 w = rec4[(g0 + j) * 4 + 0];
            float t;
            taps_blend_otf(W3[j % kD], w.x, w.y, w.z, w.w, rlane(inner_v, g0 + j) != 0, rlane(tx_v, g0 + j) + (lane & 7),
                           rlane(ty_v, g0 + j) + (lane >> 3), wl, hl, t, gx, gy);
            const size_t po = (size_t)(i0 + g0 + j) * 64;
#if defined(ICTR_REF8_ABL) && (ICTR_REF8_ABL & 1)
            gx += t * 1e-30f;
#else
            __builtin_nontemporal_store(t, T + po + lane);
            __builtin_nontemporal_store(gx, Gx + po + lane);
            __builtin_nontemporal_store(gy, Gy + po + lane);
#endif
          }
          if constexpr (j + kD < 16) issue_s(j + kD);
          accS.template push<j>(gx * gx, gy * gy, lane);
          accX.template push<j>(gx * gy, 0.0f, lane);
        });
        const int pp = lane & 15;
        const float sxx = lane_gather(accS.F, tr_lane_of<16>(pp, 0)), syy = lane_gather(accS.F, tr_lane_of<16>(pp, 1));
        const float sxy = lane_gather(accX.F, tr_lane_of<16>(pp, 0));
        const bool mine = (lane >> 4) == (g0 >> 4);
        sxx_v = mine ? sxx : sxx_v;
        sxy_v = mine ? sxy : sxy_v;
        syy_v = mine ? syy : syy_v;
      }
    } else {
    RefLoads<kU> A, B;
    issue(A, 0);
    for (int sidx = 0; sidx < nsteps; sidx += 2) {
      if (sidx + 1 < nsteps) issue(B, sidx + 1);
      reduce(A);
      if (sidx + 2 < nsteps) issue(A, sidx + 2);
      if (sidx + 1 < nsteps) reduce(B);
    }
    }
    for (unsigned long long stale = __builtin_amdgcn_ballot_w64(pv && !vis); stale; stale &= stale - 1) {
      const int j = __builtin_ctzll(stale);
      const size_t po = (size_t)(i0 + j) * 64;
      patch_sums((Gx + po)[lane], (Gy + po)[lane], j);
    }
    {
      const float4 k0 = rec4[lane * 4 + 1], k1 = rec4[lane * 4 + 2], k2 = rec4[lane * 4 + 3];
      const float ax[6] = {k0.x, k0.y, k0.z, k0.w, k1.x, k1.y}, ay[6] = {k1.z, k1.w, k2.x, k2.y, k2.z, k2.w};
      float uj[6], vj[6];
#pragma unroll
      for (int j = 0; j < 6; ++j) {
        uj[j] = __builtin_fmaf(ax[j], sxx_v, ay[j] * sxy_v);
        vj[j] = __builtin_fmaf(ax[j], sxy_v, ay[j] * syy_v);
      }
      int jk = 0;
#pragma unroll
      for (int j = 0; j < 6; ++j)
#pragma unroll
        for (int k = j; k < 6; ++k, ++jk) {
          const float h = wave_sum_dpp(__builtin_fmaf(ax[k], uj[j], ay[k] * vj[j]));
          accH += lane == jk ? h : 0.0f;
          if (jk % 3 == 2) asm volatile("" : "+v"(accH));
        }
    }
    __builtin_amdgcn_fence(__ATOMIC_RELEASE, "wavefront");
    __builtin_amdgcn_wave_barrier();
  }

  if (lane < kPartHStride) sW[wave][lane] = lane < kHUnique ? accH : 0.0f;
  __syncthreads();
  if (threadIdx.x < kHUnique) {
    const float v = (sW[0][threadIdx.x] + sW[1][threadIdx.x]) + (sW[2][threadIdx.x] + sW[3][threadIdx.x]);
    e.partH[((size_t)b * gridDim.x + blockIdx.x) * kPartHStride + threadIdx.x] = v;
  }
}

struct TapLoads4x4 {
  f32x2_a4 ab, top;
};
__device__ __forceinline__ TapLoads4x4 taps4_issue(gconst_f32 plane, int idx, int sw, bool ok, bool toprow) {
  TapLoads4x4 t;
  f32x2_a4 z = {0.0f, 0.0f};
  t.ab = z;
  t.top = z;
  if (ok) {
    t.ab = *reinterpret_cast<gconst_f32x2>(plane + (idx - 1));
    if (toprow) t.top = *reinterpret_cast<gconst_f32x2>(plane + (idx - sw - 1));
  }
  return t;
}
__device__ __forceinline__ float taps4_blend(const TapLoads4x4 &t, float w0, float w1, float w2, float w3, bool toprow) {
  const float a = t.ab.y, b = t.ab.x;
  const float cu = __shfl_up(a, 4, 64), du = __shfl_up(b, 4, 64);
  const float c = toprow ? t.top.y : cu, d = toprow ? t.top.x : du;
  return w0 * a + w1 * b + w2 * c + w3 * d;
}
struct TapLoadsP4 {
  f32x4_t l, r, tl, tr;
};
__device__ __forceinline__ float tapsP4_blend(const TapLoadsP4 &t, int k, float w0, float w1, float w2, float w3, bool toprow) {
  const float a = t.r[k], b = t.l[k];
  const float cu = __shfl_up(a, 4, 64), du = __shfl_up(b, 4, 64);
  const float c = toprow ? t.tr[k] : cu, d = toprow ? t.tl[k] : du;
  return w0 * a + w1 * b + w2 * c + w3 * d;
}

template <int kU>
struct Iter4Loads {
  float t[kU], gx[kU], gy[kU];
  TapLoads4x4 cur[kU];
  int jj[kU];
};

template <bool PN, bool WH, int kU = 2>
__global__ __launch_bounds__(kBlock) void k_iter4(EngineDev e, LevelCam lc, int level, int cpw) {
  __shared__ __attribute__((aligned(16))) float sRec[kWaves][64 * kRec];
  __shared__ float sW[kWaves][kPartBStride];
  __shared__ float sWH[WH ? kWaves : 1][kPartHStride];
  const int b = blockIdx.y;
  const ProbState &st = e.st[b];
  if (!st.active) return;
  const int npts = st.npts;
  const int M = e.M;
  const PlaneSet pl = e.planes[b * e.nlev + level];
  const float *__restrict__ p3 = e.pt3d + (size_t)b * 3 * M;
  const float *__restrict__ T = e.T + (size_t)b * M * 16;
  const float *__restrict__ Gx = e.Gx + (size_t)b * M * 16;
  const float *__restrict__ Gy = e.Gy + (size_t)b * M * 16;
  const float *__restrict__ coefb = e.coef + (size_t)b * M * kCoefStride;
  gconst_f32 cur = (gconst_f32)pl.cur;
  const int sw = lc.sw;

  float G[12];
#pragma unroll
  for (int k = 0; k < 12; ++k) G[k] = st.G[k];

  const int lane = threadIdx.x & 63;
  const int wave = __builtin_amdgcn_readfirstlane(threadIdx.x >> 6);
  const int sub = lane >> 4, q = lane & 15;
  const bool toprow = q < 4;
  const int loff = (q >> 2) * sw + (q & 3);
  float *rec = sRec[wave];
  const float4 *rec4 = reinterpret_cast<const float4 *>(rec);

  float acc[6];
#pragma unroll
  for (int k = 0; k < 6; ++k) acc[k] = 0.0f;
  float accH[WH ? kHUnique : 1];
#pragma unroll
  for (int j = 0; j < (WH ? kHUnique : 1); ++j) accH[j] = 0.0f;

  const int nchunks = (npts + cpw - 1) / cpw;
  for (int ch = xcd_band_block(blockIdx.x, gridDim.x) * kWaves + wave; ch < nchunks; ch += gridDim.x * kWaves) {
    const int i0 = ch * cpw;
    const int cnt = min(cpw, npts - i0);
    const bool pv = lane < cnt;
    const int ip = i0 + (pv ? lane : 0);
    const float X = p3[ip], Y = p3[ip + M], Z = p3[ip + 2 * M];
    const float4 *c4 = reinterpret_cast<const float4 *>(coefb + (size_t)ip * kCoefStride);
    const float4 q0 = c4[0], q1 = c4[1], q2 = c4[2];
    const float tx = G[0] * X + G[1] * Y + G[2] * Z + G[3];
    const float ty = G[4] * X + G[5] * Y + G[6] * Z + G[7];
    const float tz = G[8] * X + G[9] * Y + G[10] * Z + G[11];
    const float mx = (tx / tz) * lc.fx + lc.cx;
    const float my = (ty / tz) * lc.fy + lc.cy;
    const bool vis = pv && in_view(mx, my, lc.swo, lc.sho);
    const Taps tp = make_taps(vis ? mx : 1.0f, vis ? my : 1.0f, 2);
    const int base_v = tp.row0 * sw + tp.col0;
    {
      float4 *r4 = reinterpret_cast<float4 *>(rec + lane * kRec);
      r4[0] = make_float4(tp.w0, tp.w1, tp.w2, tp.w3);
      r4[1] = make_float4(q0.x, q0.z, q0.w, q1.x);
      r4[2] = make_float4(q1.y, q1.w, q2.x, q2.y);
      r4[3] = make_float4(q2.z, q2.w, vis ? 1.0f : 0.0f, 0.0f);
    }
    __builtin_amdgcn_fence(__ATOMIC_RELEASE, "wavefront");
    __builtin_amdgcn_wave_barrier();
    __builtin_amdgcn_fence(__ATOMIC_ACQUIRE, "wavefront");

    const int nws = (cnt + 3) >> 2;
    const int nsteps = (nws + kU - 1) / kU;
    auto issue = [&](Iter4Loads<kU> &L, int sidx) {
#pragma unroll
      for (int u = 0; u < kU; ++u) {
        const int ws = sidx + u * nsteps;
        const int j = 4 * ws + sub;
        const bool ok = (ws < nws) & (j < cnt);
        L.jj[u] = ok ? j : -1;
        const int base = __shfl(base_v, ok ? j : 0, 64);
        const size_t po = (size_t)(i0 + 4 * min(ws, nws - 1)) * 16;
        L.t[u] = L.gx[u] = L.gy[u] = 0.0f;
        if (ok) {
          L.t[u] = __builtin_nontemporal_load(T + po + lane);
          L.gx[u] = __builtin_nontemporal_load(Gx + po + lane);
          L.gy[u] = __builtin_nontemporal_load(Gy + po + lane);
        }
        L.cur[u] = taps4_issue(cur, base + loff, sw, ok, toprow);
      }
    };
    auto reduce = [&](const Iter4Loads<kU> &L) {
#pragma unroll
      for (int u = 0; u < kU; ++u) {
        const bool ok = L.jj[u] >= 0;
        const int ri = (ok ? L.jj[u] : 0) * 4;
        const float4 w = rec4[ri + 0], k0 = rec4[ri + 1], k1 = rec4[ri + 2], k2 = rec4[ri + 3];
        float inew = taps4_blend(L.cur[u], w.x, w.y, w.z, w.w, toprow);
        if constexpr (PN) inew -= group_sum(inew, 16) / 16.0f;
        const float r = ok ? (L.t[u] - inew) * k2.z : 0.0f;
        const float gx = L.gx[u], gy = L.gy[u];
        {
#pragma clang fp contract(fast)
          acc[0] += (gx * k0.x) * r;
          acc[1] += (gy * k1.y) * r;
          acc[2] += (gx * k0.y + gy * k1.z) * r;
          acc[3] += (gx * k0.z + gy * k1.w) * r;
          acc[4] += (gx * k0.w + gy * k2.x) * r;
          acc[5] += (gx * k1.x + gy * k2.y) * r;
          if constexpr (WH) {
            float sd[6];
            sd[0] = gx * k0.x;
            sd[1] = gy * k1.y;
            sd[2] = gx * k0.y + gy * k1.z;
            sd[3] = gx * k0.z + gy * k1.w;
            sd[4] = gx * k0.w + gy * k2.x;
            sd[5] = gx * k1.x + gy * k2.y;
            int jk = 0;
// ... 519 lines not shown
```

invcompcamtrack_amd/csrc/ictr_launch.h:

```cpp
#pragma once

#include <stddef.h>

#include "ictr_dev.h"

struct ictr_pyramid;
struct ictr_p2p;

struct ictr_pyramid_view {
  int nlev, pad;
  const int *w, *h, *sw;
  float *const *img, *const *dx, *const *dy;
  int getgrad;
};
extern "C" int ictr_pyramid_view_(const ictr_pyramid *p, ictr_pyramid_view *v);
extern "C" int ictr_p2p_fill_xchg_(const ictr_p2p *p, ictr::ResXchg *x);
extern "C" const char *ictr_last_error(void);

namespace ictr {

int fail(int code, const char *fmt, ...);
#define HIPCHK(expr)                                                                                  \
  do {                                                                                                \
    hipError_t _e = (expr);                                                                           \
    if (_e != hipSuccess) return fail(ICTR_ERR_HIP, "%s failed: %s", #expr, hipGetErrorString(_e));   \
  } while (0)
int need_device();
int env_int(const char *name, int dflt);
int cu_count();

struct LevelLaunch {
  int level;
  int variant;
  int gridx;
  int cpw;
  int gridx8;
};
struct ResidentGeom {
  int parts, slots, np;
};
struct Exchange {
  unsigned tag0;
  unsigned long long limit;
  unsigned long long *mail;
  int *err;
  int mute;
};
struct T1Team {
  int team, q;
  Exchange x;
};

void launch_stream_read(const float *src, size_t nfloats, float *sink, hipStream_t s);
void launch_pyr_pack(const float *img, const float *dx, const float *dy, float *pack, size_t n, hipStream_t s);
void launch_pyr_level(const float *src, int first, int pw, int ph, int psw, float *img, float *dx, float *dy, float *pack,
                      int w, int h, int pad, int sw, int sh, int getgrad, hipStream_t s);
void launch_getpatch(const float *img, const float *dx, const float *dy, const float *mids, int K, int P, int sw,
                     int dopatchnorm, float *out, float *out_dx, float *out_dy, hipStream_t s);
void launch_ncc(const float *img_b, const float *img_r, const float *img_f, const float *mids, int K, int P, int sw,
                float swo, float sho, float w_back, float w_fwd, float *out, hipStream_t s);
void launch_flow_gather(const void *du, const void *dv, int is_f64, int H, int W, const double *xy, int K, double *out,
                        hipStream_t s);
void launch_bil_patches(const double *img, int H, int W, int C, const double *pts, int K, int half, double *out,
                        hipStream_t s);
void launch_project_generic(const float *pt3d, float *pt3d_rot, float *pt2d, int n, int M, const float *G, LevelCam lc,
                            hipStream_t s);
void launch_project_ref(const EngineDev &e, const LevelCam *cams, int maxpts, hipStream_t s);
bool defer_h(const EngineDev &e, int variant);
int tail_partials(const EngineDev &e, const LevelLaunch &ll);
void launch_ref_level(const EngineDev &e, const LevelCam &lc, const LevelLaunch &ll, bool tail, hipStream_t s);
void launch_level_finish(const EngineDev &e, const LevelLaunch &ll, hipStream_t s);
void launch_iter_main(const EngineDev &e, const LevelCam &lc, const LevelLaunch &ll, int first, hipStream_t s,
                      hipEvent_t ev0, hipEvent_t ev1);
void launch_iter_tail(const EngineDev &e, const LevelLaunch &ll, int first, hipStream_t s);
void launch_iter_finish(const EngineDev &e, const LevelLaunch &ll, int first, hipStream_t s);
hipError_t launch_debug_wave_solve(const float *H, const float *b, int n, ProbState *st, int through_state, float *x,
                                   int *rank, int *nonzero, int *rowmap, int *colmap, float *lu, hipStream_t s);
hipError_t launch_debug_se3(const float *in, float *out, long long n, int log_not_exp, hipStream_t s);

size_t track1_plan(int npts_cap, int n, int p8, int waves, int *tmpl_lds);
size_t track1_blob_bytes(void);
int track1_team_q(int maxpts, int target);
int track1_team_size(int maxpts, int target);
size_t track1_team_mail_bytes(int B, int team);
hipError_t launch_track1(const EngineDev &e, const LevelCam *cams, int maxpts, int waves, const void *blob,
                         ProbState *host_st, hipStream_t s, const T1Team *tm, bool project_here = false,
                         bool any_size = false);

size_t resident_mail_bytes(int parts, int slots);
int resident_points_per_workgroup(int np);
int resident_blocks_per_cu(int np);
hipError_t launch_level_resident(const EngineDev &e, const LevelCam &lc, int level, const ResidentGeom &g, int nblk,
                                 const Exchange &x, const ResXchg *xchg, hipStream_t s);
hipError_t launch_debug_transpose_reduce(const float *vals, float *out, int *patch_of_lane, int *kind_of_lane, int np,
                                         hipStream_t s);

void launch_seq_select(const SeqArgs &a, hipStream_t s);
void launch_ransac_chunk(const RansacArgs &a, int tile, hipStream_t s);
void launch_ransac_finish(const RansacArgs &a, hipStream_t s);
void launch_patchflow(const PFArgs &a, hipStream_t s);

}
```

invcompcamtrack_amd/csrc/ictr_resident.hip:

```cpp
#include <string.h>

#include <type_traits>

#include "ictr_dev.h"
#include "ictr_launch.h"
#include "ictr_devfn.h"
#include "se3_math.h"

namespace ictr {

constexpr int kResWaves = 4;
constexpr int kResThreads = 64 * kResWaves;
constexpr int kResSlot = 8;
#ifndef ICTR_RES_AUX
#define ICTR_RES_AUX 2
#endif
#ifndef ICTR_RES_D
#define ICTR_RES_D 4
#endif
constexpr int kResD = ICTR_RES_D;

struct ResArgs {
  LevelCam lc;
  int level;
  int parts, slots;
  int nblk;
  int dbg_mute;
  int prof_slot;
  ResXchg x;
  unsigned tag0;
  unsigned long long limit;
  unsigned long long *mail;
  int *err;
};

__host__ __device__ __forceinline__ size_t res_slot_granules(int parts) { return (size_t)2 * parts * kResSlot + 2 * 16; }

struct ResPoll {
  unsigned long long limit;
  int *err;
  int dead;
};
#define RES_EACH8(X) X(0) X(1) X(2) X(3) X(4) X(5) X(6) X(7)
__device__ __forceinline__ void res_poll(ResPoll &pc, const unsigned long long *(&src)[8], unsigned long long (&g)[8],
                                         unsigned tag, int lane) {
  const unsigned long long empty = (unsigned long long)tag << 32;
#define RES_LOAD(u) g[u] = src[u] ? __hip_atomic_load(src[u], __ATOMIC_RELAXED, __HIP_MEMORY_SCOPE_AGENT) : empty;
  RES_EACH8(RES_LOAD)
  if (pc.dead) return;
  unsigned long long h[8];
  __builtin_amdgcn_s_sleep(4);
#define RES_LOADH(u) h[u] = src[u] ? __hip_atomic_load(src[u], __ATOMIC_RELAXED, __HIP_MEMORY_SCOPE_AGENT) : empty;
  RES_EACH8(RES_LOADH)
  bool started = false;
  unsigned long long t0 = 0;
  for (;;) {
    bool miss = false;
#define RES_MISS(u) miss |= (unsigned)(g[u] >> 32) != tag;
    RES_EACH8(RES_MISS)
    if (__builtin_amdgcn_ballot_w64(miss) == 0) break;
    if (!started) {
      t0 = wall_clock64();
      started = true;
    } else if (wall_clock64() - t0 > pc.limit) {
      if (lane == 0) __hip_atomic_store(pc.err, 1, __ATOMIC_RELAXED, __HIP_MEMORY_SCOPE_SYSTEM);
      pc.dead = 1;
      break;
    }
#define RES_ROTATE(u)                                                                                         \
  if ((unsigned)(g[u] >> 32) != tag) {                                                                        \
    g[u] = h[u];                                                                                              \
    h[u] = __hip_atomic_load(src[u], __ATOMIC_RELAXED, __HIP_MEMORY_SCOPE_AGENT);                             \
  }
    RES_EACH8(RES_ROTATE)
  }
}
__device__ __forceinline__ unsigned long long res_poll1(ResPoll &pc, const unsigned long long *src, unsigned tag, int lane) {
  const unsigned long long empty = (unsigned long long)tag << 32;
  unsigned long long g = src ? __hip_atomic_load(src, __ATOMIC_RELAXED, __HIP_MEMORY_SCOPE_AGENT) : empty;
  if (pc.dead) return g;
  __builtin_amdgcn_s_sleep(3);
  unsigned long long h1 = src ? __hip_atomic_load(src, __ATOMIC_RELAXED, __HIP_MEMORY_SCOPE_AGENT) : empty;
  __builtin_amdgcn_s_sleep(3);
  unsigned long long h2 = src ? __hip_atomic_load(src, __ATOMIC_RELAXED, __HIP_MEMORY_SCOPE_AGENT) : empty;
  bool started = false;
  unsigned long long t0 = 0;
  while (__builtin_amdgcn_ballot_w64((unsigned)(g >> 32) != tag) != 0) {
    if (!started) {
      t0 = wall_clock64();
      started = true;
    } else if (wall_clock64() - t0 > pc.limit) {
      if (lane == 0) __hip_atomic_store(pc.err, 1, __ATOMIC_RELAXED, __HIP_MEMORY_SCOPE_SYSTEM);
      pc.dead = 1;
      break;
    }
    if ((unsigned)(g >> 32) != tag) {
      g = h1;
      h1 = h2;
      h2 = __hip_atomic_load(src, __ATOMIC_RELAXED, __HIP_MEMORY_SCOPE_AGENT);
    }
  }
  return g;
}

template <int NP>
__global__ __launch_bounds__(64) void k_debug_transpose_reduce(const float *__restrict__ vals, float *__restrict__ out,
                                                               int *__restrict__ patch_of_lane, int *__restrict__ kind_of_lane) {
  const int lane = threadIdx.x;
  TrAcc<NP> acc;
  tr_for_each_patch<NP, 0>([&](auto jc) {
    constexpr int j = decltype(jc)::value;
    acc.template push<j>(vals[lane * 64 + 2 * j], vals[lane * 64 + 2 * j + 1], lane);
  });
  out[lane] = acc.F;
  patch_of_lane[lane] = tr_patch_of_lane<NP>(lane);
  kind_of_lane[lane] = tr_kind_of_lane(lane);
}
hipError_t launch_debug_transpose_reduce(const float *vals, float *out, int *pl, int *kl, int np, hipStream_t s) {
  if (np == 16)
    hipLaunchKernelGGL(k_debug_transpose_reduce<16>, dim3(1), dim3(64), 0, s, vals, out, pl, kl);
  else
    hipLaunchKernelGGL(k_debug_transpose_reduce<32>, dim3(1), dim3(64), 0, s, vals, out, pl, kl);
  return hipGetLastError();
}

__device__ __forceinline__ double res_xchg_sum(const ResXchg &x, ResPoll &pc, int pair, unsigned xs, int off, int n, float v,
                                               int lane) {
  const unsigned tag = 0x80000000u | xs;
  const size_t par = (size_t)(xs & 1u) * x.world;
  const size_t idx = (size_t)pair * kXchgPerPair + off + lane;
  if (lane < n) {
    const unsigned long long g = ((unsigned long long)tag << 32) | (unsigned long long)__builtin_bit_cast(unsigned, v);
    for (int r = 0; r < x.world; ++r)
      __hip_atomic_store(x.peer[r] + (par + x.rank) * x.cap + idx, g, __ATOMIC_RELAXED, __HIP_MEMORY_SCOPE_SYSTEM);
  }
  double sum = 0.0;
  bool started = false;
  unsigned long long t0 = 0;
  const unsigned long long empty = (unsigned long long)tag << 32;
  for (int r0 = 0; r0 < x.world; r0 += 8) {
    unsigned long long g[8];
#pragma unroll
    for (int u = 0; u < 8; ++u)
      g[u] = (lane < n && r0 + u < x.world)
                 ? __hip_atomic_load(x.local + (par + r0 + u) * x.cap + idx, __ATOMIC_RELAXED, __HIP_MEMORY_SCOPE_SYSTEM)
                 : empty;
    while (!pc.dead) {
      bool miss = false;
#pragma unroll
      for (int u = 0; u < 8; ++u) miss |= (unsigned)(g[u] >> 32) != tag;
      if (__builtin_amdgcn_ballot_w64(miss) == 0) break;
      if (!started) {
        t0 = wall_clock64();
        started = true;
      } else if (wall_clock64() - t0 > pc.limit) {
        if (lane == 0) __hip_atomic_store(pc.err, 1, __ATOMIC_RELAXED, __HIP_MEMORY_SCOPE_SYSTEM);
        pc.dead = 1;
        break;
      }
      __builtin_amdgcn_s_sleep(1);
#pragma unroll
      for (int u = 0; u < 8; ++u)
        if ((unsigned)(g[u] >> 32) != tag)
          g[u] = __hip_atomic_load(x.local + (par + r0 + u) * x.cap + idx, __ATOMIC_RELAXED, __HIP_MEMORY_SCOPE_SYSTEM);
    }
#pragma unroll
    for (int u = 0; u < 8; ++u) sum += (double)__builtin_bit_cast(float, (unsigned)(g[u] & 0xffffffffu));
  }
  return sum;
}

__device__ __forceinline__ double res_sum8(double v) {
#define RES_DPP64(ctrl)                                                                              \
  {                                                                                                  \
    const int lo = dpp_mov<ctrl>(__double2loint(v)), hi = dpp_mov<ctrl>(__double2hiint(v));          \
    v += __hiloint2double(hi, lo);                                                                   \
  }
  RES_DPP64(0xB1)
  RES_DPP64(0x4E)
  RES_DPP64(0x141)
  return v;
}

typedef float f32x2_t __attribute__((ext_vector_type(2)));
#ifdef ICTR_RES_PROF
#define RES_MARK(k)                        \
  {                                        \
    t1_ = __builtin_readcyclecounter();    \
    tp_[k] += t1_ - t0_;                   \
    t0_ = t1_;                             \
  }
constexpr int kTrIters = 128;
__device__ unsigned long long g_res_trace[16][kTrIters][4];
#define RES_STAMP(row, it, k) \
  if ((row) >= 0 && (it) < kTrIters && tid == 0) g_res_trace[row][it][k] = wall_clock64();
#else
#define RES_MARK(k)
#define RES_STAMP(row, it, k)
#endif
struct ResWin {
  f32x2_a4 ab, cd;
};

__device__ __forceinline__ void res_setprio(int p) {
  if (p == 0) __builtin_amdgcn_s_setprio(0);
  else if (p == 1) __builtin_amdgcn_s_setprio(1);
  else if (p == 2) __builtin_amdgcn_s_setprio(2);
  else __builtin_amdgcn_s_setprio(3);
}

template <int NP>
__global__ __launch_bounds__(kResThreads, 4) void k_level_resident(EngineDev e, ResArgs a) {
  constexpr int kResPPW = NP, kResQ = kResWaves * NP;
  __shared__ __attribute__((aligned(16))) float4 sRecW[kResWaves][kResPPW];
  __shared__ float sT[kResWaves][kResPPW * 64];
  __shared__ float sPart[kResWaves][8];
  __shared__ double sRed[kResWaves][8];
  __shared__ float sG[16];
  __shared__ ProbState sSt;

  const int parts = a.parts;
  const int group = parts + 1;
  const int slot = (int)blockIdx.x / group;
  const int part = (int)blockIdx.x - slot * group;
  const int tid = threadIdx.x;
  const int lane = tid & 63;
  const int wave = __builtin_amdgcn_readfirstlane(tid >> 6);
  const int M = e.M;
  unsigned long long *gbox = a.mail + (size_t)slot * res_slot_granules(parts);
  unsigned long long *bbox = gbox + (size_t)2 * parts * kResSlot;
  ResPoll pc;
  pc.limit = a.limit;
  pc.err = a.err;
  pc.dead = 0;
  unsigned seq = 0;
#ifdef ICTR_RES_PROF
  const int tr_row = part == parts ? (slot < 8 ? 8 + slot : -1) : ((part == 0 && slot < 8) ? slot : -1);
  int tr_it = 0;
  unsigned long long tp_[8] = {0, 0, 0, 0, 0, 0, 0, 0}, t0_ = __builtin_readcyclecounter(), t1_ = 0;
#endif

  if (part == parts) {
    __builtin_amdgcn_s_setprio(3);
    SolveOpts sopt = solve_opts(e);
    sopt.robust = 0;
    __shared__ double sRedH[kResThreads / 32][32];
    __shared__ float sH[32];
    for (int b = slot, round = 0; b < e.B; b += a.slots, ++round) {
      const ProbState &gst = e.st[b];
      int active = ((0 < e.maxiter) & (1.0f > e.ratio)) ? 1 : 0;
      {
        const unsigned *src = reinterpret_cast<const unsigned *>(&gst);
        unsigned *dst = reinterpret_cast<unsigned *>(&sSt);
        for (int i = tid; i < (int)(sizeof(ProbState) / 4); i += kResThreads) dst[i] = src[i];
      }
      {
        const int j = tid & 31, sl = tid >> 5;
        double sacc = 0.0;
        const float *ph = e.partH + (size_t)b * a.nblk * kPartHStride + j;
        if (j < kHUnique) {
#pragma unroll 8
          for (int k = sl; k < a.nblk; k += kResThreads / 32) sacc += (double)ph[(size_t)k * kPartHStride];
        }
        sRedH[sl][j] = sacc;
      }
      __syncthreads();
      if (tid < kHUnique) {
        double sacc = 0.0;
#pragma unroll
        for (int sl = 0; sl < kResThreads / 32; ++sl) sacc += sRedH[sl][tid];
        sH[tid] = (float)sacc;
      }
      __syncthreads();
      unsigned xs = 0;
      if (wave == 0) {
        float hl = lane < kHUnique ? sH[lane] : 0.0f;
        if (a.x.world > 1) {
          xs = a.x.xseq[b] + 1u;
          hl = (float)res_xchg_sum(a.x, pc, b, xs, 12, kHUnique, hl, lane);
          __builtin_amdgcn_fence(__ATOMIC_RELEASE, "wavefront");
          __builtin_amdgcn_wave_barrier();
          if (lane < kHUnique) sH[lane] = hl;
          __builtin_amdgcn_fence(__ATOMIC_RELEASE, "wavefront");
          __builtin_amdgcn_wave_barrier();
          __builtin_amdgcn_fence(__ATOMIC_ACQUIRE, "wavefront");
        }
        WaveSolver S;
        ws_factor(S, sH[h_unique_index(lane)], lane);
        ws_store_factor(S, sSt, lane);
        if (lane == 0) level_reset(sSt, e);
      }
      __syncthreads();
      while (active) {
        seq += 1;
        const unsigned tag = a.tag0 + seq;
        const unsigned long long *gslot = gbox + (size_t)(seq & 1u) * parts * kResSlot;
        unsigned long long *bslot = bbox + (size_t)(seq & 1u) * 16;
        RES_MARK(0)
        RES_STAMP(tr_row, tr_it, 0)
        const int k = lane >> 3, rr = lane & 7;
        double accd = 0.0;
        for (int r0 = 0; r0 < parts; r0 += 64 * kResWaves) {
          const unsigned long long *src[8];
          unsigned long long g[8];
#define RES_SRC(u)                                                                   \
  {                                                                                  \
    const int r = r0 + (wave * 8 + u) * 8 + rr;                                      \
    src[u] = (k < 6 && r < parts) ? gslot + (size_t)r * kResSlot + k : nullptr;      \
  }
          RES_EACH8(RES_SRC)
          res_poll(pc, src, g, tag, lane);
#define RES_ACC(u) accd += (double)__builtin_bit_cast(float, (unsigned)(g[u] & 0xffffffffu));
          RES_EACH8(RES_ACC)
        }
        const double tot = res_sum8(accd);
        RES_MARK(1)
        RES_STAMP(tr_row, tr_it, 1)
        if (rr == 0 && k < 6) sRed[wave][k] = tot;
        __syncthreads();
        RES_MARK(2)
        RES_STAMP(tr_row, tr_it, 2)
        if (wave == 0) {
          double bsum = 0.0;
          if (lane < 6)
            for (int w = 0; w < kResWaves; ++w) bsum += sRed[w][lane];
          if (a.x.world > 1) {
            xs += 1u;
            const float hi = (float)bsum;
            const float lo = (float)(bsum - (double)hi);
            const float pv = lane < 6 ? hi : lane_gather(lo, lane - 6);
            const double t = res_xchg_sum(a.x, pc, b, xs, 0, 12, pv, lane);
            const int l6 = lane + 6;
            bsum = t + __hiloint2double(lane_gather(__double2hiint(t), l6), lane_gather(__double2loint(t), l6));
          }
          WaveSolver S;
          float G[12];
          ws_load_state(S, sSt, lane, G);
          ws_load_factor(S, sSt, lane);
          ws_iterate(S, (float)bsum, sopt, a.level, b, lane, G);
          ws_store_state(S, sSt, lane, G);
          float gv = 0.0f;
#pragma unroll
          for (int q = 0; q < 12; ++q) gv = lane == q ? G[q] : gv;
          const int act = pc.dead ? 0 : S.active;
          if (lane == 12) gv = __builtin_bit_cast(float, act);
          if (lane < 13)
            __hip_atomic_store(bslot + lane,
                               ((unsigned long long)tag << 32) | (unsigned long long)__builtin_bit_cast(unsigned, gv),
                               __ATOMIC_RELAXED, __HIP_MEMORY_SCOPE_AGENT);
          if (lane == 0) sG[12] = __builtin_bit_cast(float, act);
          RES_MARK(3)
          RES_STAMP(tr_row, tr_it, 3)
        }
#ifdef ICTR_RES_PROF
        tr_it += 1;
#endif
        __syncthreads();
        active = __builtin_amdgcn_readfirstlane(__builtin_bit_cast(int, sG[12]));
      }
      if (wave == 0) {
        if (a.x.world > 1 && lane == 0) a.x.xseq[b] = xs;
        const unsigned *src = reinterpret_cast<const unsigned *>(&sSt);
        unsigned *dst = reinterpret_cast<unsigned *>(e.st + b);
        for (int i = lane; i < (int)(sizeof(ProbState) / 4); i += 64) dst[i] = src[i];
      }
      __syncthreads();
    }
#ifdef ICTR_RES_PROF
    if (slot == a.prof_slot && tid == 0)
      for (int k = 0; k < 8; ++k) e.partH[8 + k] = (float)tp_[k];
#endif
    return;
  }

  const LevelCam lc = a.lc;
  const int sw = lc.sw;
  const unsigned off_cd = (unsigned)((lane >> 3) * sw + (lane & 7)) * 4u;
  const unsigned off_ab = off_cd + (unsigned)sw * 4u;
  float4 *const recs = sRecW[wave];
  float *const tw = sT[wave] + lane;
  const int my_patch = tr_patch_of_lane<NP>(lane);
  const int my_kind = tr_kind_of_lane(lane);
  for (int b = slot, round = 0; b < e.B; b += a.slots, ++round) {
    res_setprio((slot + round) & 3);
    const ProbState &gst = e.st[b];
    const int npts = gst.npts;
    int active = ((0 < e.maxiter) & (1.0f > e.ratio)) ? 1 : 0;
    if (!active) continue;
    const int i0 = part * kResQ + wave * kResPPW;
    const int cnt = min(kResPPW, max(0, npts - i0));
    const float *cur_plane;
    {
      const unsigned long long pc64 = reinterpret_cast<unsigned long long>(e.planes[b * e.nlev + a.level].cur);
      const unsigned lo = __builtin_amdgcn_readfirstlane((unsigned)pc64), hi = __builtin_amdgcn_readfirstlane((unsigned)(pc64 >> 32));
      cur_plane = reinterpret_cast<const float *>(((unsigned long long)hi << 32) | lo);
    }
    const __amdgpu_buffer_rsrc_t rcur =
        __builtin_amdgcn_make_buffer_rsrc(const_cast<float *>(cur_plane), 0, 0x7fffffff, 0x00020000);
    f32x2_t Gxy[kResPPW];
    const float *gT = e.T + ((size_t)b * M + i0) * 64 + lane;
    const float *gGx = e.Gx + ((size_t)b * M + i0) * 64 + lane;
    const float *gGy = e.Gy + ((size_t)b * M + i0) * 64 + lane;
    const bool pv = lane < cnt;
    float c6[6] = {0.0f, 0.0f, 0.0f, 0.0f, 0.0f, 0.0f};
    const int nbytes = __builtin_amdgcn_readfirstlane(cnt * 256);
    auto bounded = [&](const float *q) {
      const unsigned long long v = reinterpret_cast<unsigned long long>(q - lane);
      const unsigned lo = __builtin_amdgcn_readfirstlane((unsigned)v), hi = __builtin_amdgcn_readfirstlane((unsigned)(v >> 32));
      return __builtin_amdgcn_make_buffer_rsrc(reinterpret_cast<float *>(((unsigned long long)hi << 32) | lo), 0, nbytes,
                                               0x00020000);
    };
    const __amdgpu_buffer_rsrc_t rT = bounded(gT), rGx = bounded(gGx), rGy = bounded(gGy);
    const int loff = lane * 4;
#pragma unroll
    for (int j = 0; j < kResPPW; ++j) {
      Gxy[j].x = __builtin_bit_cast(float, __builtin_amdgcn_raw_buffer_load_b32(rGx, loff, j * 256, ICTR_RES_AUX));
      Gxy[j].y = __builtin_bit_cast(float, __builtin_amdgcn_raw_buffer_load_b32(rGy, loff, j * 256, ICTR_RES_AUX));
    }
#pragma unroll
    for (int j0 = 0; j0 < kResPPW; j0 += 8) {
      float t8[8];
#pragma unroll
      for (int u = 0; u < 8; ++u) t8[u] = __builtin_bit_cast(float, __builtin_amdgcn_raw_buffer_load_b32(rT, loff, (j0 + u) * 256, ICTR_RES_AUX));
#pragma unroll
      for (int u = 0; u < 8; ++u) tw[(j0 + u) * 64] = t8[u];
    }
    if (my_patch < cnt && tr_primary_lane<NP>(lane)) {
      const float *cl = e.coef + ((size_t)b * M + i0 + my_patch) * kCoefStride + (my_kind ? 6 : 0);
#pragma unroll
      for (int k = 0; k < 6; ++k) c6[k] = cl[k];
    }
    float X = 0.0f, Y = 0.0f, Z = 1.0f;
    if (pv) {
      const float *p3 = e.pt3d + (size_t)b * 3 * M;
      X = p3[i0 + lane], Y = p3[i0 + lane + M], Z = p3[i0 + lane + 2 * M];
    }
    if (tid < 12) sG[tid] = gst.G[tid];
    __syncthreads();

    while (active) {
      RES_MARK(0)
      RES_STAMP(tr_row, tr_it, 0)
      int base_v;
      float vis_f;
      {
        float Gc[12];
#pragma unroll
        for (int k = 0; k < 12; ++k) Gc[k] = sG[k];
        const float tx = Gc[0] * X + Gc[1] * Y + Gc[2] * Z + Gc[3];
        const float ty = Gc[4] * X + Gc[5] * Y + Gc[6] * Z + Gc[7];
        const float tz = Gc[8] * X + Gc[9] * Y + Gc[10] * Z + Gc[11];
        const float mx = (tx / tz) * lc.fx + lc.cx;
        const float my = (ty / tz) * lc.fy + lc.cy;
        const bool vis = pv && in_view(mx, my, lc.swo, lc.sho);
        const Taps tp = make_taps(vis ? mx : 1.0f, vis ? my : 1.0f, 4);
        base_v = ((tp.row0 - 1) * sw + tp.col0 - 1) * 4;
        vis_f = vis ? 1.0f : 0.0f;
        if (lane < kResPPW) recs[lane] = make_float4(tp.w1, tp.w0, tp.w3, tp.w2);
      }
      __builtin_amdgcn_fence(__ATOMIC_RELEASE, "wavefront");
      __builtin_amdgcn_wave_barrier();
      __builtin_amdgcn_fence(__ATOMIC_ACQUIRE, "wavefront");
      RES_MARK(1)
      ResWin W[kResD];
      auto issue = [&](int j) {
#if defined(ICTR_RES_ABL) && ICTR_RES_ABL == 2
        if (j >= kResD) return;
#endif
#if defined(ICTR_RES_ABL) && ICTR_RES_ABL == 1
        const int soff = 0;
#else
        const int soff = rlane(base_v, j);
#endif
        W[j % kResD].cd = __builtin_bit_cast(f32x2_a4, __builtin_amdgcn_raw_buffer_load_b64(rcur, (int)off_cd, soff, 0));
        W[j % kResD].ab = __builtin_bit_cast(f32x2_a4, __builtin_amdgcn_raw_buffer_load_b64(rcur, (int)off_ab, soff, 0));
      };
#pragma unroll
      for (int j = 0; j < kResD; ++j) issue(j);
      TrAcc<NP> acc;
      float4 wv_n = recs[0];
      float t_n = tw[0];
      tr_for_each_patch<NP, 0>([&](auto jc) {
        constexpr int j = decltype(jc)::value;
        const float4 wv = wv_n;
        const float t = t_n;
        asm volatile("" ::: "memory");
        if constexpr (j + 1 < kResPPW) {
          wv_n = recs[j + 1];
          t_n = tw[(j + 1) * 64];
        }
        const ResWin w = W[j % kResD];
        const f32x2_t pab = f32x2_t{wv.x, wv.y} * f32x2_t{w.ab.x, w.ab.y}, pcd = f32x2_t{wv.z, wv.w} * f32x2_t{w.cd.x, w.cd.y};
        const float inew = ((pab.y + pab.x) + pcd.y) + pcd.x;
        if constexpr (j + kResD < kResPPW) issue(j + kResD);
        const float r = t - inew;
        const f32x2_t gr = Gxy[j] * f32x2_t{r, r};
        acc.template push<j>(gr.x, gr.y, lane);
      });
      const float F = acc.F;
      RES_MARK(2)
      RES_STAMP(tr_row, tr_it, 1)
      {
        const float val = F * lane_gather(vis_f, my_patch);
        float o = 0.0f;
#pragma unroll
        for (int k = 0; k < 6; ++k) {
          const float v = wave_sum_dpp(c6[k] * val);
          o = lane == k ? v : o;
        }
        if (lane < 6) sPart[wave][lane] = o;
      }
      __syncthreads();
      RES_MARK(3)
      RES_STAMP(tr_row, tr_it, 2)
      seq += 1;
      const unsigned tag = a.tag0 + seq;
      unsigned long long *gslot = gbox + (size_t)(seq & 1u) * parts * kResSlot;
      const unsigned long long *bslot = bbox + (size_t)(seq & 1u) * 16;
      if (wave == 0) {
        int lane_v = lane;
        asm volatile("" : "+v"(lane_v));
        float bs = 0.0f;
        if (lane < 6) bs = (sPart[0][lane] + sPart[1][lane]) + (sPart[2][lane] + sPart[3][lane]);
        if (lane < 6 && part + 1 != a.dbg_mute)
          __hip_atomic_store(gslot + (size_t)part * kResSlot + lane_v,
                             ((unsigned long long)tag << 32) | (unsigned long long)__builtin_bit_cast(unsigned, bs),
                             __ATOMIC_RELAXED, __HIP_MEMORY_SCOPE_AGENT);
        const unsigned long long g = res_poll1(pc, lane < 13 ? bslot + lane_v : nullptr, tag, lane);
        if (lane < 13) sG[lane] = (lane == 12 && pc.dead) ? 0.0f : __builtin_bit_cast(float, (unsigned)(g & 0xffffffffu));
        RES_MARK(4)
        RES_STAMP(tr_row, tr_it, 3)
      }
#ifdef ICTR_RES_PROF
      tr_it += 1;
#endif
      __syncthreads();
      active = __builtin_amdgcn_readfirstlane(__builtin_bit_cast(int, sG[12]));
    }
    RES_MARK(5)
    __syncthreads();
  }
#ifdef ICTR_RES_PROF
  if (slot == a.prof_slot && part == 0 && tid == 0)
    for (int k = 0; k < 8; ++k) e.partH[k] = (float)tp_[k];
#endif
}

#ifdef ICTR_RES_PROF
extern "C" int ictr_prof_res_trace(unsigned long long *out, int clear) {
  if (out && hipMemcpyFromSymbol(out, HIP_SYMBOL(g_res_trace), sizeof(g_res_trace)) != hipSuccess) return 1;
  if (clear) {
    static unsigned long long z[16][kTrIters][4];
    if (hipMemcpyToSymbol(HIP_SYMBOL(g_res_trace), z, sizeof(z)) != hipSuccess) return 1;
  }
  return 0;
}
#endif
size_t resident_mail_bytes(int parts, int slots) {
  return sizeof(unsigned long long) * (size_t)slots * res_slot_granules(parts);
}
int resident_points_per_workgroup(int np) { return kResWaves * np; }
template <int NP>
static int res_occupancy() {
  int v = 0;
  if (hipOccupancyMaxActiveBlocksPerMultiprocessor(&v, reinterpret_cast<const void *>(&k_level_resident<NP>),
                                                   kResThreads, 0) != hipSuccess) {
    (void)hipGetLastError();
    v = 0;
  }
  return v;
}
int resident_blocks_per_cu(int np) {
  static const int n[2] = {res_occupancy<16>(), res_occupancy<32>()};
  return n[np == 32 ? 1 : 0];
}
hipError_t launch_level_resident(const EngineDev &e, const LevelCam &lc, int level, const ResidentGeom &g, int nblk,
                                 const Exchange &x, const ResXchg *xchg, hipStream_t s) {
  ResArgs a;
  if (xchg)
    a.x = *xchg;
  else
    memset(&a.x, 0, sizeof(a.x));
  {
    const char *ps = getenv("ICTR_RES_PROF_SLOT");
    a.prof_slot = ps ? atoi(ps) : 0;
  }
  a.nblk = nblk;
  a.lc = lc;
  a.level = level;
  a.parts = g.parts;
  a.slots = g.slots;
  a.dbg_mute = x.mute;
  a.tag0 = x.tag0;
  a.limit = x.limit;
  a.mail = x.mail;
  a.err = x.err;
  const dim3 grid((g.parts + 1) * g.slots), blk(kResThreads);
  if (g.np == 32)
    hipLaunchKernelGGL((k_level_resident<32>), grid, blk, 0, s, e, a);
  else
    hipLaunchKernelGGL((k_level_resident<16>), grid, blk, 0, s, e, a);
  return hipGetLastError();
}

}
```

invcompcamtrack_amd/tracker.py:

```python
from __future__ import annotations

import ctypes as C

import numpy as np

from . import _lib
from ._lib import OptParam, TraceRec, check, dp, f32c, f64c, fp

__all__ = ["optparam", "CamClass", "PoseClass", "OdometerClass", "Pyramid", "TrackBatch", "locality_order",
           "util_constructpyramide", "util_getPatch", "util_getPatch_grad", "ncc_score", "util_SE3_coeff_to_group",
           "util_SE3_group_to_coeff", "solve6", "device_count", "timebase_mark"]


def device_count():
    return _lib.load().ictr_device_count()


def timebase_mark():
    check(_lib.load().ictr_timebase_mark())


def optparam(lv_f, lv_l, psz, maxiter, normdp_ratio, donorm, dopatchnorm, maxpttrack, verbosity=0):
    op = OptParam()
    check(_lib.load().ictr_optparam_init(C.byref(op), lv_f, lv_l, psz, maxiter, normdp_ratio, int(donorm),
# ... 74 lines not shown
        check(_lib.load().ictr_pyramid_level_dims(self._h, level, C.byref(sw), C.byref(sh)))
        return sw.value, sh.value

    def download(self, level, which=0):
        sw, sh = self.level_dims(level)
        out = np.empty((sh, sw), np.float32)
        check(_lib.load().ictr_pyramid_download(self._h, level, which, fp(out)))
        return out

    def device_plane(self, level, which=0):
        return _lib.load().ictr_pyramid_device_plane(self._h, level, which)


def util_constructpyramide(img, lv_f, getgrad, imgpadding):
    return Pyramid(img, lv_f, imgpadding, bool(getgrad))


def util_getPatch(pyr, level, mids, op):
    mids = np.atleast_2d(np.asarray(mids, np.float32))
    K = mids.shape[0]
    soa = np.ascontiguousarray(mids.T)
    out = np.empty((K, op.novals), np.float32)
    check(_lib.load().ictr_get_patch(pyr._h, level, fp(soa), K, op.psz, int(op.dopatchnorm), fp(out)))
    return out


def util_getPatch_grad(pyr, level, mids, op):
    mids = np.atleast_2d(np.asarray(mids, np.float32))
    K = mids.shape[0]
    soa = np.ascontiguousarray(mids.T)
    o = [np.empty((K, op.novals), np.float32) for _ in range(3)]
    check(_lib.load().ictr_get_patch_grad(pyr._h, level, fp(soa), K, op.psz, int(op.dopatchnorm), fp(o[0]), fp(o[1]),
                                          fp(o[2])))
    return tuple(o)


def ncc_score(pyr_back, pyr_ref, pyr_fwd, level, mids_back, mids_ref, mids_fwd, psz, w_back, w_fwd):
    mb, mr, mf = (np.atleast_2d(np.asarray(m, np.float32)) for m in (mids_back, mids_ref, mids_fwd))
    K = mr.shape[0]
    soa = np.ascontiguousarray(np.concatenate([mb.T, mr.T, mf.T], 0), np.float32)
    out = np.empty(K, np.float32)
    check(_lib.load().ictr_ncc_score(pyr_back._h, pyr_ref._h, pyr_fwd._h, level, fp(soa), K, psz, float(w_back),
                                     float(w_fwd), fp(out)))
    return out


def util_SE3_coeff_to_group(p):
    L = _lib.load()
    p = np.ascontiguousarray(p)
    if p.dtype == np.float32:
        G = np.empty(12, np.float32)
        L.ictr_se3_coeff_to_group_f(fp(G), fp(p))
    else:
        p = f64c(p)
        G = np.empty(12, np.float64)
        L.ictr_se3_coeff_to_group_d(dp(G), dp(p))
    return G


def util_SE3_group_to_coeff(G):
    L = _lib.load()
    G = np.ascontiguousarray(G)
    if G.dtype == np.float32:
        p = np.empty(6, np.float32)
        L.ictr_se3_group_to_coeff_f(fp(p), fp(G))
    else:
        G = f64c(G)
        p = np.empty(6, np.float64)
        L.ictr_se3_group_to_coeff_d(dp(p), dp(G))
    return p


def locality_order(pts3d, p, fc, cc):
    pts3d = np.asarray(pts3d, np.float64)
    G = util_SE3_coeff_to_group(np.asarray(p, np.float64)).reshape(3, 4)
    Xc = G[:, :3] @ pts3d + G[:, 3:4]
    z = np.where(np.abs(Xc[2]) > 1e-12, Xc[2], 1e-12)
    x = Xc[0] / z * float(fc[0]) + float(cc[0])
    y = Xc[1] / z * float(fc[1]) + float(cc[1])
    ok = np.isfinite(x) & np.isfinite(y)
    xi = np.clip(np.where(ok, x, -1.0), -1.0, 65534.0).astype(np.int64) + 1
    yi = np.clip(np.where(ok, y, -1.0), -1.0, 65534.0).astype(np.int64) + 1

    def spread(v):
        v = (v | (v << 8)) & 0x00FF00FF
        v = (v | (v << 4)) & 0x0F0F0F0F
        v = (v | (v << 2)) & 0x33333333
        return (v | (v << 1)) & 0x55555555
    return np.argsort(spread(xi) | (spread(yi) << 1), kind="stable")


def solve6(H, b):
    H = f32c(H).reshape(36)
    b = f32c(b)
    x = np.empty(6, np.float32)
    _lib.load().ictr_solve6(fp(H), fp(b), fp(x))
    return x


class PoseClass:

    def __init__(self, camobj, op):
        self.camobj, self.op = camobj, op
        self._h = C.c_void_p()
        check(_lib.load().ictr_pose_create(C.byref(self._h), camobj._h, C.byref(op)))

    def __del__(self):
        if getattr(self, "_h", None) and _lib is not None and getattr(_lib, "load", None):
            _lib.load().ictr_pose_destroy(self._h)
            self._h = None

    def setpose_se3(self, p_in, meanshift_in=(0.0, 0.0, 0.0), varval_in=0.0):
        p_in, ms = f64c(p_in), f64c(meanshift_in)
        check(_lib.load().ictr_pose_setpose_se3(self._h, dp(p_in), dp(ms), float(varval_in)))

    def addpose_se3(self, p_in):
        p_in = f32c(p_in)
        check(_lib.load().ictr_pose_addpose_se3(self._h, fp(p_in)))

    def subpose_se3(self, p_in):
        p_in = f32c(p_in)
        check(_lib.load().ictr_pose_subpose_se3(self._h, fp(p_in)))

    def getPose_se3(self):
        out = np.empty(6, np.float64)
        check(_lib.load().ictr_pose_getpose_se3(self._h, dp(out)))
        return out

    def project_pt(self, pt3d, nopoints, sc, pt2d=None):
        M = self.op.maxpttrack
        pt3d = f32c(pt3d).reshape(3 * M)
        pt2d = np.zeros(2 * M, np.float32) if pt2d is None else pt2d
        check(_lib.load().ictr_pose_project_pt(self._h, fp(pt3d), fp(pt2d), nopoints, sc))
        return pt2d

    def project_pt_save_rotated(self, pt3d, nopoints, sc):
        M = self.op.maxpttrack
        pt3d = f32c(pt3d).reshape(3 * M)
        rot = np.zeros(3 * M, np.float32)
        pt2d = np.zeros(2 * M, np.float32)
        check(_lib.load().ictr_pose_project_pt_save_rotated(self._h, fp(pt3d), fp(rot), fp(pt2d), nopoints, sc))
        return rot, pt2d

    def state(self):
        p, G = np.empty(6, np.float32), np.empty(12, np.float32)
        check(_lib.load().ictr_pose_get_state(self._h, fp(p), fp(G)))
        return p, G


def _path_name(form, team):
    name = {0: "k_iter* (per-iteration launches)", 1: "k_track1 (one launch per tracking)",
            2: "k_iter* (per-iteration launches replayed as one hipGraph)",
            3: "k_track1 (one launch per tracking, begin phase and read-back included)",
            4: "k_level_resident (one launch per level: all iterations, templates resident in registers)"}.get(form, "?")
    return name + (f" x {team} workgroups per problem" if team > 1 else "")


class OdometerClass:

    def __init__(self, pose_in, op_in):
        self.pose, self.op = pose_in, op_in
        self._h = C.c_void_p()
        self._keep = None
        check(_lib.load().ictr_odometer_create(C.byref(self._h), pose_in._h, C.byref(op_in)))

    def __del__(self):
        if getattr(self, "_h", None) and _lib is not None and getattr(_lib, "load", None):
            _lib.load().ictr_odometer_destroy(self._h)
            self._h = None

    def set_stream(self, stream_ptr):
        check(_lib.load().ictr_odometer_set_stream(self._h, C.c_void_p(stream_ptr or 0)))

    def set_variant(self, variant):
        check(_lib.load().ictr_odometer_set_variant(self._h, int(variant)))

    def set_team(self, target_points, min_points=0, max_points=1 << 30):
        check(_lib.load().ictr_odometer_set_team(self._h, int(target_points), int(min_points), int(max_points)))

    def set_robust(self, clean_invisible=False, compositional=False, huber_k=0.0):
        flags = (1 if clean_invisible else 0) | (2 if compositional else 0) | (4 if huber_k != 0 else 0)
        check(_lib.load().ictr_odometer_set_robust(self._h, flags, float(huber_k)))

    def Set3Dpoints(self, pt_in, nopoints_in=None):
        if not (isinstance(pt_in, np.ndarray) and pt_in.dtype == np.float64 and pt_in.flags.c_contiguous):
            raise TypeError("Set3Dpoints needs a C-contiguous float64 array (it is normalised in place when donorm)")
        n = pt_in.size // 3 if nopoints_in is None else nopoints_in
        check(_lib.load().ictr_odometer_set3dpoints(self._h, dp(pt_in), n))

    def SetPose(self, p_in, img_ref, img_new):
        p_in = f64c(p_in)
        self._keep = (img_ref, img_new)
        check(_lib.load().ictr_odometer_setpose(self._h, dp(p_in), img_ref._h, img_new._h))

    def SetPose_host(self, p_in, img_ref, img_ref_dx, img_ref_dy, img_new):
        p_in = f64c(p_in)
        n = self.op.lv_f + 1
        keep = [[f32c(a) for a in lst] for lst in (img_ref, img_ref_dx, img_ref_dy, img_new)]
        arrs = [(_lib.FP * n)(*[fp(a) for a in lst]) for lst in keep]
        check(_lib.load().ictr_odometer_setpose_host(self._h, dp(p_in), *arrs))

    def TrackPose(self):
        out = np.empty(6, np.float64)
        check(_lib.load().ictr_odometer_trackpose(self._h, dp(out)))
        return out

    def Get2DPoints(self):
        ptr = _lib.load().ictr_odometer_get2dpoints(self._h)
        if not ptr:
            check(1)
        return np.ctypeslib.as_array(ptr, shape=(2 * self.op.maxpttrack,)).copy()

    def path_name(self):
        L = _lib.load()
        return _path_name(L.ictr_odometer_last_path(self._h), L.ictr_odometer_last_team(self._h))

    def enable_trace(self, on=True):
        check(_lib.load().ictr_odometer_enable_trace(self._h, int(on)))

    def trace(self):
        cap = (self.op.lv_f + 1) * max(1, self.op.maxiter)
        recs = (TraceRec * cap)()
        cnt = C.c_int64()
        check(_lib.load().ictr_odometer_trace(self._h, recs, cap, C.byref(cnt)))
        out = []
        for i in range(min(cnt.value, cap)):
            r = recs[i]
            out.append(dict(level=r.level, iter=r.iter, H=np.array(r.H[:], np.float32).reshape(6, 6),
                            b=np.array(r.b[:], np.float32), dp=np.array(r.dp[:], np.float32),
                            p=np.array(r.p[:], np.float32)))
        return out

    def read_buffer(self, which, count):
        out = np.empty(count, np.float32)
        check(_lib.load().ictr_odometer_read_buffer(self._h, which, fp(out), count))
        return out

    def norm(self):
        ms = np.zeros(3)
        vv = C.c_double()
        check(_lib.load().ictr_odometer_get_norm(self._h, dp(ms), C.byref(vv)))
        return ms, vv.value


class TrackBatch:

    def __init__(self, camobj, op, nproblems):
        self.camobj, self.op, self.B = camobj, op, nproblems
        self._h = C.c_void_p()
        self._keep = {}
        self._keep_all = None
        check(_lib.load().ictr_batch_create(C.byref(self._h), camobj._h, C.byref(op), nproblems))

    def __del__(self):
        if getattr(self, "_h", None) and _lib is not None and getattr(_lib, "load", None):
            _lib.load().ictr_batch_destroy(self._h)
            self._h = None

    def set_stream(self, stream_ptr):
        check(_lib.load().ictr_batch_set_stream(self._h, C.c_void_p(stream_ptr or 0)))

    def set_variant(self, variant):
        check(_lib.load().ictr_batch_set_variant(self._h, int(variant)))

    def set_team(self, target_points, min_points=0, max_points=1 << 30):
        check(_lib.load().ictr_batch_set_team(self._h, int(target_points), int(min_points), int(max_points)))

    def set_peer_exchange(self, p2p_handle):
        check(_lib.load().ictr_batch_set_peer_exchange(self._h, p2p_handle))

    def set_robust(self, clean_invisible=False, compositional=False, huber_k=0.0):
        flags = (1 if clean_invisible else 0) | (2 if compositional else 0) | (4 if huber_k != 0 else 0)
        check(_lib.load().ictr_batch_set_robust(self._h, flags, float(huber_k)))

    def Set3Dpoints(self, problem, pt_in, nopoints_in=None):
        if not (isinstance(pt_in, np.ndarray) and pt_in.dtype == np.float64 and pt_in.flags.c_contiguous):
            raise TypeError("Set3Dpoints needs a C-contiguous float64 array")
        n = pt_in.size // 3 if nopoints_in is None else nopoints_in
        check(_lib.load().ictr_batch_set3dpoints(self._h, problem, dp(pt_in), n))

    def Set3Dpoints_norm(self, problem, pt_in, meanshift, varval, nopoints_in=None):
        if not (isinstance(pt_in, np.ndarray) and pt_in.dtype == np.float64 and pt_in.flags.c_contiguous):
            raise TypeError("Set3Dpoints needs a C-contiguous float64 array")
        n = pt_in.size // 3 if nopoints_in is None else nopoints_in
        ms = f64c(meanshift)
        check(_lib.load().ictr_batch_set3dpoints_norm(self._h, problem, dp(pt_in), n, dp(ms), float(varval)))

    def norm(self, problem):
        ms = np.zeros(3)
        vv = C.c_double()
        check(_lib.load().ictr_batch_get_norm(self._h, problem, dp(ms), C.byref(vv)))
        return ms, vv.value

    def SetPose(self, problem, p_in, img_ref, img_new):
        p_in = f64c(p_in)
        self._keep[problem] = (img_ref, img_new)
        check(_lib.load().ictr_batch_setpose(self._h, problem, dp(p_in), img_ref._h, img_new._h))

    def SetPoseAll(self, poses, img_ref, img_new):
        poses = f64c(poses)
        if poses.shape != (self.B, 6):
            raise ValueError(f"SetPoseAll needs a ({self.B}, 6) array of poses, got {poses.shape}")
        self._keep.clear()
        self._keep_all = (img_ref, img_new)
        check(_lib.load().ictr_batch_setpose_all(self._h, dp(poses), img_ref._h, img_new._h))

    def track_async(self):
        check(_lib.load().ictr_batch_track_async(self._h))

    def poses(self):
        out = np.empty((self.B, 6), np.float64)
        check(_lib.load().ictr_batch_get_poses(self._h, dp(out)))
        return out

    def iterations(self):
        out = np.zeros(self.B, np.int32)
        check(_lib.load().ictr_batch_get_iterations(self._h, out.ctypes.data_as(_lib.IP)))
        return out

    def Get2DPoints(self, problem):
        out = np.empty(2 * self.op.maxpttrack, np.float32)
        check(_lib.load().ictr_batch_get2dpoints(self._h, problem, fp(out)))
        return out

    def read_buffer(self, problem, which, count):
        out = np.empty(count, np.float32)
        check(_lib.load().ictr_batch_read_buffer(self._h, problem, which, fp(out), count))
        return out

    def set_timing(self, on=True):
        check(_lib.load().ictr_batch_set_timing(self._h, int(on)))

    def level_times(self):
        n = self.op.lv_f + 1
        a, b = np.zeros(n, np.float32), np.zeros(n, np.float32)
        check(_lib.load().ictr_batch_get_level_times(self._h, fp(a), fp(b)))
        return a, b

    def kernel_times(self):
        a = np.zeros(self.op.lv_f + 1, np.float32)
        check(_lib.load().ictr_batch_get_kernel_times(self._h, fp(a)))
        return a

    def first_iter_times(self):
        a = np.zeros(self.op.lv_f + 1, np.float32)
        check(_lib.load().ictr_batch_get_first_iter_times(self._h, fp(a)))
        return a

    def kernel_intervals(self):
        n, m = self.op.lv_f + 1, max(1, self.op.maxiter)
        a, b = np.zeros(n * m, np.float32), np.zeros(n * m, np.float32)
        check(_lib.load().ictr_batch_get_kernel_intervals(self._h, fp(a), fp(b)))
        return a.reshape(n, m), b.reshape(n, m)

    def setup_intervals(self):
        n = self.op.lv_f + 1
        a, b = np.zeros(n, np.float32), np.zeros(n, np.float32)
        check(_lib.load().ictr_batch_get_setup_intervals(self._h, fp(a), fp(b)))
        return a, b

    def path_name(self):
        L = _lib.load()
        return _path_name(L.ictr_batch_last_path(self._h), L.ictr_batch_last_team(self._h))

    def last_team(self):
        return int(_lib.load().ictr_batch_last_team(self._h))

    def set_reduction_buffer(self, dev_ptr):
        check(_lib.load().ictr_batch_set_reduction_buffer(self._h, C.c_void_p(dev_ptr or 0)))

    def enable_sharding(self, on=True):
        check(_lib.load().ictr_batch_enable_sharding(self._h, int(on)))

    def reduction_buffer_ptr(self):
        return _lib.load().ictr_batch_reduction_buffer(self._h)

    @property
    def needs_level_allreduce(self):
        return bool(_lib.load().ictr_batch_level_allreduce_needed(self._h))

    def begin(self): check(_lib.load().ictr_batch_begin(self._h))
    def level_accumulate(self, level): check(_lib.load().ictr_batch_level_accumulate(self._h, level))
    def level_finish(self, level): check(_lib.load().ictr_batch_level_finish(self._h, level))
    def iter_accumulate(self, level): check(_lib.load().ictr_batch_iter_accumulate(self._h, level))
    def iter_finish(self, level): check(_lib.load().ictr_batch_iter_finish(self._h, level))
```

profiles/recompute_roofline.py:

```python
#!/usr/bin/env python3
from __future__ import annotations

import argparse
import csv
import sys

PEAK = 8000.0e9
BIG = ("k_iter8", "k_ref8", "k_level_res", "k_iter4", "k_ref4", "k_stream_read")


def short(name):
    for k in BIG:
        if k in name:
            return k
    return None


def from_trace(path, points, reduce_to=None, pairs=None, res_pairs=32, maxiter=10):
    rows = []
    with open(path, newline="") as f:
        for r in csv.DictReader(f):
            k = short(r["Kernel_Name"])
            if k is None:
                continue
            rows.append((int(r["Start_Timestamp"]), int(r["End_Timestamp"]), k, int(r["Grid_Size_Y"]),
                         r["Kernel_Name"].split("(")[0]))
    rows.sort()
    if pairs is None:
        pairs = 16
    if reduce_to:
        rows = [r for r in rows if r[2] in ("k_stream_read", "k_level_res") or r[3] == pairs]
        with open(reduce_to, "w", newline="") as f:
            w = csv.writer(f)
            w.writerow(["Kernel_Name", "Start_Timestamp", "End_Timestamp", "Grid_Size_Y"])
            for s, e, k, gy, full in rows:
                w.writerow([full, s, e, gy])
        print(f"wrote {len(rows)} dispatches to {reduce_to}")
    alone = [True] * len(rows)
    active = []
    for i, (s, e, k, gy, _) in enumerate(rows):
        active = [j for j in active if rows[j][1] > s]
        for j in active:
            alone[i] = alone[j] = False
        active.append(i)
    it_all = [(e - s, gy) for (s, e, k, gy, _) in rows if k == "k_iter8" and gy == pairs]
    it_solo = [(e - s, gy) for a, (s, e, k, gy, _) in zip(alone, rows) if a and k == "k_iter8" and gy == pairs]
    if not it_solo:
        print("no un-overlapped k_iter8 dispatch in this trace")
        return 1
    frac = 0.0

    def report(tag, lst):
        byts = sum(16.0 * 64 * points * gy for _, gy in lst)
        ns = sum(d for d, _ in lst)
        rate = byts / (ns * 1e-9)
        print(f"{tag:28s} {len(lst):6d} launches, mean {ns / len(lst) / 1e3:8.2f} us, pairs/launch "
              f"{sum(gy for _, gy in lst) / len(lst):5.1f}: {rate / 1e9:8.1f} GB/s = {rate / PEAK:.4f} of 8 TB/s")
        return rate / PEAK

    report("k_iter8, all dispatches", it_all)
    frac = report("k_iter8, running alone", it_solo)
    marks = [i for i, r in enumerate(rows) if r[2] == "k_stream_read"]
    if marks:
        tail = [(e - s, gy) for (s, e, k, gy, _) in rows[marks[-1]:] if k == "k_iter8"]
        if tail:
            leg = [(d, gy) for d, gy in tail if gy == pairs]
            frac = report("k_iter8, solo leg (marker)", leg)
    else:
        print("(no k_stream_read marker in this trace: the figure is that of the dispatches running alone)")
    for k in ("k_ref8",):
        lst = [(e - s, gy) for a, (s, e, kk, gy, _) in zip(alone, rows) if a and kk == k]
        if lst:
            ns = sum(d for d, _ in lst)
            print(f"{k + ', running alone':28s} {len(lst):6d} launches, mean {ns / len(lst) / 1e3:8.2f} us")
    groups, prev = [], None
    for i, r in enumerate(rows):
        if r[2] == "k_stream_read":
            if prev is None or i != prev + 1:
                groups.append([i, i])
            groups[-1][1] = i
            prev = i
    res = [(e - s) for (s, e, k, gy, _) in (rows[groups[0][1]:groups[1][0]] if len(groups) >= 2 else rows)
           if k == "k_level_res"]
    if res:
        mean = sum(res) / len(res)
        byts = 16.0 * 64 * points * res_pairs * maxiter
        rate = byts / (mean * 1e-9)
        print(f"{'k_level_resident, headline':28s} {len(res):6d} launches, mean {mean / 1e3:8.2f} us, {byts / 1e9:.2f} GB "
              f"algorithmic per launch ({res_pairs} pairs x {maxiter} iterations): {rate / 1e9:8.1f} GB/s equivalent = "
              f"{rate / PEAK:.4f} of 8 TB/s")
        print(f"roofline.frac = {rate / PEAK:.4f}   (headline kernel k_level_resident)")
        print(f"roofline.streaming_kernel.frac = {frac:.4f}   (k_iter8, solo leg)")
    else:
        print(f"roofline.frac = {frac:.4f}")
    return 0


def from_stats(path, points, pairs):
    calls = tot = 0.0
    with open(path, newline="") as f:
        for r in csv.DictReader(f):
            if "k_iter8" in r["Name"]:
                c = float(r["Calls"])
                calls += c
                tot += c * float(r["AverageNs"])
                print(f"  {r['Name'].split('(')[0]:60s} calls {int(c):6d} avg {float(r['AverageNs']) / 1e3:8.2f} us")
    if calls == 0:
        print("no k_iter8 rows")
        return 1
    mean = tot / calls
    byts = 16.0 * 64 * points * pairs
    rate = byts / (mean * 1e-9)
    print(f"k_iter8: {int(calls)} launches, mean {mean / 1e3:.2f} us, {byts / 1e6:.1f} MB per launch ({pairs} pairs): "
          f"{rate / 1e9:.1f} GB/s")
    print(f"roofline.frac = {rate / PEAK:.4f}   (valid only if nothing overlapped: bench.py --streams 1)")
    return 0


def main():
    ap = argparse.ArgumentParser()
    ap.add_argument("csv")
    ap.add_argument("--points", type=int, default=32400, help="8x8 patches per frame pair (bench default 240 x 135)")
    ap.add_argument("--pairs", type=int, default=None,
                    help="frame pairs per launch = the dispatch's grid size in y (trace input: default 16, bench.py's "
                         "--batch 32 over two engines; --stats input: default 32, one engine)")
    ap.add_argument("--res-pairs", type=int, default=32, help="frame pairs per k_level_resident launch (bench default 32)")
    ap.add_argument("--maxiter", type=int, default=10)
    ap.add_argument("--reduce", default=None, help="trace input: also write the reduced trace here")
    a = ap.parse_args()
    with open(a.csv, newline="") as f:
        header = f.readline()
    if "Start_Timestamp" in header:
        return from_trace(a.csv, a.points, a.reduce, a.pairs, a.res_pairs, a.maxiter)
    return from_stats(a.csv, a.points, a.pairs or 32)


if __name__ == "__main__":
    sys.exit(main())
```

Before: 531,300 Mpix/s.

## Fuse all pyramid levels into one resident launch per tracking

Adds a resident-track form in which a single k_level_resident launch iterates every pyramid level in turn. It is enabled when the launch budget allows and no peer exchange is set. The per-level reference kernels now all run up front, so each level gets its own template, gradient, coefficient and partial-H buffers, and stale patches copy from the next-coarser level's buffers. The aim is to cut two kernel launches and the inter-level launch gaps and drains. The cost is extra device memory for the per-level buffers and a longer, more complex persistent kernel.

New measurement: 530,500 Mpix/s. Within noise of the previous version (-0.1%).

```diff
diff --git a/include/ictr.h b/include/ictr.h
--- a/include/ictr.h
+++ b/include/ictr.h
@@ -158,6 +158,7 @@
 int ictr_batch_get2dpoints(ictr_batch *b, int64_t problem, float *host_out );
 int ictr_batch_set_variant(ictr_batch *b, int variant);
 int ictr_batch_set_team(ictr_batch *b, int target_points, int min_points, int max_points);
+int ictr_batch_set_level_launches(ictr_batch *b, int enable);
 #define ICTR_ROBUST_CLEAN 1
 #define ICTR_ROBUST_COMPOSE 2
 #define ICTR_ROBUST_HUBER 4
diff --git a/invcompcamtrack_amd/_lib.py b/invcompcamtrack_amd/_lib.py
--- a/invcompcamtrack_amd/_lib.py
+++ b/invcompcamtrack_amd/_lib.py
@@ -133,6 +133,7 @@
     "ictr_batch_get2dpoints": (C.c_int, [VP, I64, FP]),
     "ictr_batch_set_variant": (C.c_int, [VP, C.c_int]),
     "ictr_batch_set_team": (C.c_int, [VP, C.c_int, C.c_int, C.c_int]),
+    "ictr_batch_set_level_launches": (C.c_int, [VP, C.c_int]),
     "ictr_batch_set_robust": (C.c_int, [VP, C.c_int, C.c_float]),
     "ictr_batch_read_buffer": (C.c_int, [VP, I64, C.c_int, FP, I64]),
     "ictr_batch_set_timing": (C.c_int, [VP, C.c_int]),
diff --git a/invcompcamtrack_amd/csrc/ictr_dev.h b/invcompcamtrack_amd/csrc/ictr_dev.h
--- a/invcompcamtrack_amd/csrc/ictr_dev.h
+++ b/invcompcamtrack_amd/csrc/ictr_dev.h
@@ -81,8 +81,33 @@
   float *partH;
   float *partb;
   float *red;
+  float *lvT, *lvGx, *lvGy;
+  float *lvcoef;
+  float *lvpartH;
+  long long lv_partH_stride;
   DevTrace trace;
 };
+
+struct LevelBufs {
+  float *T, *Gx, *Gy, *coef, *partH;
+};
+__host__ __device__ __forceinline__ LevelBufs level_bufs(const EngineDev &e, int level) {
+  LevelBufs r = {e.T, e.Gx, e.Gy, e.coef, e.partH};
+  if (e.lvT != nullptr && level > e.lv_l && level <= e.lv_f) {
+    const size_t k = (size_t)(level - e.lv_l - 1);
+    const size_t np = (size_t)e.B * e.M * e.n, nc = (size_t)e.B * e.M * kCoefStride;
+    r.T = e.lvT + k * np;
+    r.Gx = e.lvGx + k * np;
+    r.Gy = e.lvGy + k * np;
+    r.coef = e.lvcoef + k * nc;
+    r.partH = e.lvpartH + k * (size_t)e.lv_partH_stride;
+  }
+  return r;
+}
+__host__ __device__ __forceinline__ LevelBufs stale_bufs(const EngineDev &e, int level) {
+  if (level < e.lv_f) return level_bufs(e, level + 1);
+  return LevelBufs{e.T, e.Gx, e.Gy, e.coef, e.partH};
+}
 
 constexpr int kSeqBlock = 256;
 constexpr int kSeqPPT = 16;
diff --git a/invcompcamtrack_amd/csrc/ictr_host.hip b/invcompcamtrack_amd/csrc/ictr_host.hip
--- a/invcompcamtrack_amd/csrc/ictr_host.hip
+++ b/invcompcamtrack_amd/csrc/ictr_host.hip
@@ -637,7 +637,9 @@
   kFormGraph = 2,
   kFormTrack1Begin = 3,
   kFormResident = 4,
+  kFormResidentTrack = 5,
 };
+static bool form_resident(int form) { return form == kFormResident || form == kFormResidentTrack; }
 struct TrackPlan {
   int form;
   int variant;
@@ -709,6 +711,10 @@
   ProbState *d_st_mirror = nullptr;
   char *h_up_pin = nullptr;
   Mailbox team_mail, res_mail;
+  float *d_lvT = nullptr, *d_lvGx = nullptr, *d_lvGy = nullptr, *d_lvcoef = nullptr, *d_lvpartH = nullptr;
+  int lv_sets = 0;
+  bool lv_failed = false;
+  int level_launches = 0;
   int team_target = 0;
   int team_lo = 128, team_hi = 8192;
   int *h_team_err = nullptr;
@@ -737,6 +743,8 @@
   if (b->team_mail.d) (void)hipFree(b->team_mail.d);
   if (b->res_mail.d) (void)hipFree(b->res_mail.d);
   if (b->d_xseq) (void)hipFree(b->d_xseq);
+  for (void *p : {(void *)b->d_lvT, (void *)b->d_lvGx, (void *)b->d_lvGy, (void *)b->d_lvcoef, (void *)b->d_lvpartH})
+    if (p) (void)hipFree(p);
   b->d_red = b->d_red_own;
   for (void *p : {(void *)b->d_pt3d, (void *)b->d_pt3d_ref, (void *)b->d_pt2d, (void *)b->d_T, (void *)b->d_Gx,
                   (void *)b->d_Gy, (void *)b->d_coef, (void *)b->d_partH, (void *)b->d_partb, (void *)b->d_red,
@@ -809,6 +817,7 @@
   b->team_target = env_int("ICTR_TEAM_TARGET", 0);
   b->team_lo = env_int("ICTR_TEAM_MINPTS", 128);
   b->team_hi = env_int("ICTR_TEAM_MAXPTS", 8192);
+  b->level_launches = env_int("ICTR_LEVEL_LAUNCHES", 0) ? 1 : 0;
   const size_t B = b->B, M = b->M, n = b->n, L = b->nlev;
   const int ppw = (b->n <= 64 && 64 % b->n == 0) ? 64 / b->n : 1;
   const int64_t groups = (b->M + ppw - 1) / ppw;
@@ -899,6 +908,11 @@
   return ICTR_OK;
 }
 
+extern "C" int ictr_batch_set_level_launches(ictr_batch *b, int enable) {
+  if (!b) return fail(ICTR_ERR_INVALID, "batch is NULL");
+  b->level_launches = enable ? 1 : 0;
+  return ICTR_OK;
+}
 extern "C" int ictr_batch_set_variant(ictr_batch *b, int variant) {
   if (!b) return fail(ICTR_ERR_INVALID, "batch is NULL");
   if (variant & ~ICTR_VARIANT_ALL)
@@ -1109,7 +1123,7 @@
 extern "C" float *ictr_batch_reduction_buffer(ictr_batch *b) { return b ? b->d_red : nullptr; }
 
 static LevelLaunch level_launch(const ictr_batch *b, const TrackPlan *p, int level) {
-  const bool res = p && p->form == kFormResident;
+  const bool res = p && form_resident(p->form);
   LevelLaunch ll;
   ll.level = level;
   ll.variant = p ? p->variant : engine_variant(b);
@@ -1206,7 +1220,7 @@
   return team;
 }
 
-static bool resident_plan(const ictr_batch *b, TrackPlan *p) {
+static bool resident_plan(const ictr_batch *b, TrackPlan *p, bool *track_fits) {
   if (b->P != 8 || b->robust || b->sharded || b->op->dopatchnorm || b->op->maxiter < 1) return false;
   const bool xchg = b->xchg.world > 1;
   const bool big_batch = b->maxpts >= 500 && (int64_t)b->B * b->maxpts >= 48000;
@@ -1221,8 +1235,10 @@
     const int slots = (int)std::min<int64_t>(std::min<int64_t>(b->B, max_slots), capacity / (parts + 1));
     if (slots < 1) continue;
     if (np == 16 && slots < b->B && !xchg) continue;
-    if ((int64_t)((b->B + slots - 1) / slots) * b->op->maxiter >= 4000) return false;
+    const int64_t xnum = (int64_t)((b->B + slots - 1) / slots) * b->op->maxiter;
+    if (xnum >= 4000) return false;
     p->res = ResidentGeom{parts, slots, np};
+    *track_fits = xnum * (b->op->lv_f - b->op->lv_l + 1) < 4000;
     return true;
   }
   return false;
@@ -1257,8 +1273,9 @@
   p.variant = v;
   p.team = 1;
   p.mute = (v & ICTR_VARIANT_DEBUG_MUTE) ? 1 : 0;
+  bool track_fits = false;
   const bool resident = !(v & (ICTR_VARIANT_NO_RESIDENT | ICTR_VARIANT_LAUNCHES | ICTR_VARIANT_ANY_SIZE)) &&
-                        resident_plan(b, &p);
+                        resident_plan(b, &p, &track_fits);
   bool t1 = !b->sharded && !b->timing && !(v & ICTR_VARIANT_LAUNCHES) && b->xchg.world <= 1 && b->otf != 2 &&
             !(b->maxpts < 8193 && resident) && b->maxpts >= 1;
   if (t1) {
@@ -1281,7 +1298,8 @@
     p.form = (!separate && up <= track1_blob_bytes()) ? kFormTrack1Begin : kFormTrack1;
     p.project_here = p.form == kFormTrack1 && !separate;
   } else if (resident) {
-    p.form = kFormResident;
+    const bool track = track_fits && b->xchg.world <= 1 && !b->lv_failed && !b->level_launches;
+    p.form = track ? kFormResidentTrack : kFormResident;
     resident_setup_plan(b, cpw_forced() != 0, &p);
   } else if (!b->sharded && !b->timing && !b->graph_broken && !(v & ICTR_VARIANT_NO_GRAPH) &&
              (int64_t)b->maxpts * b->B <= 65536) {
@@ -1403,22 +1421,40 @@
   return launch();
 }
 
-static int launch_resident(ictr_batch *b, const EngineDev &e, const LevelCam &lc, const LevelLaunch &ll,
-                           const TrackPlan &p, hipStream_t s) {
+static int launch_resident(ictr_batch *b, const EngineDev &e, int lv_hi, int lv_lo, const TrackPlan &p, hipStream_t s) {
   const ResidentGeom &g = p.res;
+  LevelCam cams[16];
+  int nblk[16];
+  for (int l = lv_lo; l <= lv_hi; ++l) {
+    cams[l] = level_cam(b->cam, l);
+    nblk[l] = tail_partials(e, level_launch(b, &p, l));
+  }
   Exchange x;
   if (int rc = exchange_prepare(b, &b->res_mail, resident_mail_bytes(g.parts, g.slots), "resident", p.mute, s, &x)) return rc;
   const int bpc = std::max(1, std::min(4, resident_blocks_per_cu(g.np)));
   const int weight = g.slots * (g.parts + 1) * ((4 + bpc - 1) / bpc);
   return team_launch(weight, s, [&]() -> int {
-    HIPCHK(launch_level_resident(e, lc, ll.level, g, tail_partials(e, ll), x, b->xchg.world > 1 ? &b->xchg : nullptr, s));
+    HIPCHK(launch_level_resident(e, cams, nblk, lv_hi, lv_lo, g, x, b->xchg.world > 1 ? &b->xchg : nullptr, s));
     return ICTR_OK;
   });
 }
 
 static int enqueue_level_kernels(ictr_batch *b, const EngineDev &e, const TrackPlan &p, hipStream_t s, bool events) {
   const int mi = b->op->maxiter;
-  const bool resident = p.form == kFormResident;
+  const bool resident = form_resident(p.form);
+  if (p.form == kFormResidentTrack) {
+    const int lf = b->op->lv_f, ll0 = b->op->lv_l;
+    b->evk_valid = false;
+    if (events) HIPCHK(hipEventRecord(b->ev[3 * lf + 0], s));
+    for (int sl = lf; sl >= ll0; --sl) launch_ref_level(e, level_cam(b->cam, sl), level_launch(b, &p, sl), false, s);
+    if (events) HIPCHK(hipEventRecord(b->ev[3 * lf + 1], s));
+    if (int rc = launch_resident(b, e, lf, ll0, p, s)) return rc;
+    if (events) {
+      HIPCHK(hipEventRecord(b->ev[3 * lf + 2], s));
+      b->ev_used[lf] = 1;
+    }
+    return ICTR_OK;
+  }
   const bool tk = !resident && events && (int)b->evk.size() >= 2 * b->nlev * mi && mi <= b->evk_iters;
   b->evk_valid = tk;
   for (int sl = b->op->lv_f; sl >= b->op->lv_l; --sl) {
@@ -1428,7 +1464,7 @@
     launch_ref_level(e, lc, ll, !resident, s);
     if (events) HIPCHK(hipEventRecord(b->ev[3 * sl + 1], s));
     if (resident) {
-      if (int rc = launch_resident(b, e, lc, ll, p, s)) return rc;
+      if (int rc = launch_resident(b, e, sl, sl, p, s)) return rc;
     } else {
       for (int it = 0; it < mi; ++it) {
         const int ke = 2 * (sl * b->evk_iters + it);
@@ -1447,7 +1483,7 @@
 template <class T>
 static void key_put(std::string &k, const T &v) { k.append(reinterpret_cast<const char *>(&v), sizeof(T)); }
 static std::string graph_key(const ictr_batch *b, const EngineDev &e, const TrackPlan &p) {
-  static_assert(sizeof(EngineDev) == 14 * 4 + 14 * 8 + 2 * 4, "EngineDev must have no padding (graph_key)");
+  static_assert(sizeof(EngineDev) == 14 * 4 + 20 * 8 + 2 * 4, "EngineDev must have no padding (graph_key)");
   static_assert(sizeof(TrackPlan) % 4 == 0 && sizeof(LevelCam) == 7 * 4, "plain ints and floats only");
   std::string k;
   key_put(k, e);
@@ -1479,9 +1515,55 @@
   return true;
 }
 
+static bool level_buffers_prepare(ictr_batch *b) {
+  const int sets = b->op->lv_f - b->op->lv_l;
+  if (sets <= b->lv_sets) return true;
+  if (b->lv_failed) return false;
+  float **ptrs[5] = {&b->d_lvT, &b->d_lvGx, &b->d_lvGy, &b->d_lvcoef, &b->d_lvpartH};
+  if (b->lv_sets > 0) {
+    if (hipStreamSynchronize(b->stream) != hipSuccess) (void)hipGetLastError();
+    for (float **p : ptrs) {
+      (void)hipFree(*p);
+      *p = nullptr;
+    }
+    b->lv_sets = 0;
+  }
+  const size_t np = sizeof(float) * (size_t)b->B * b->M * b->n;
+  const size_t bytes[5] = {np, np, np, sizeof(float) * (size_t)b->B * b->M * kCoefStride,
+                           sizeof(float) * (size_t)b->B * b->gridx * kPartHStride};
+  hipError_t er = hipSuccess;
+  for (int i = 0; i < 5 && er == hipSuccess; ++i) {
+    er = hipMalloc((void **)ptrs[i], bytes[i] * sets);
+    if (er == hipSuccess) er = hipMemsetAsync(*ptrs[i], 0, bytes[i] * sets, b->stream);
+  }
+  if (er != hipSuccess) {
+    (void)hipGetLastError();
+    for (float **p : ptrs) {
+      if (*p) (void)hipFree(*p);
+      *p = nullptr;
+    }
+    b->lv_failed = true;
+    return false;
+  }
+  b->lv_sets = sets;
+  return true;
+}
+
 static int enqueue_levels(ictr_batch *b) {
-  const EngineDev e = engine_dev(b);
+  EngineDev e = engine_dev(b);
   TrackPlan &p = b->plan;
+  if (p.form == kFormResidentTrack) {
+    if (level_buffers_prepare(b)) {
+      e.lvT = b->d_lvT;
+      e.lvGx = b->d_lvGx;
+      e.lvGy = b->d_lvGy;
+      e.lvcoef = b->d_lvcoef;
+      e.lvpartH = b->d_lvpartH;
+      e.lv_partH_stride = (long long)b->B * b->gridx * kPartHStride;
+    } else {
+      p.form = kFormResident;
+    }
+  }
   if (b->xchg.world > 1 && p.form != kFormResident)
     return fail(ICTR_ERR_STATE, "a peer exchange is set (sharded resident form) but this tracking cannot run in the "
                                 "resident-iteration form (8x8 patches, no robustness option, no patch normalisation, builder-"
@@ -1548,7 +1630,7 @@
     return fail(ICTR_ERR_HIP, "%s: a workgroup waited in vain for its peers' partial sums (in-launch exchange timed out "
                               "after %.3f s; are all workgroups of the launch resident?); the results of this tracking "
                               "are invalid",
-                b->plan.form == kFormResident ? "resident-iteration form (k_level_resident)" : "one-launch tracker, team form (k_track1_p8)",
+                form_resident(b->plan.form) ? "resident-iteration form (k_level_resident)" : "one-launch tracker, team form (k_track1_p8)",
                 team_timeout_s());
   return ICTR_OK;
 }
diff --git a/invcompcamtrack_amd/csrc/ictr_kernels.hip b/invcompcamtrack_amd/csrc/ictr_kernels.hip
--- a/invcompcamtrack_amd/csrc/ictr_kernels.hip
+++ b/invcompcamtrack_amd/csrc/ictr_kernels.hip
@@ -673,10 +673,16 @@
   const PlaneSet pl = e.planes[b * e.nlev + level];
   const float *__restrict__ pt2d = e.pt2d + ((size_t)b * e.nlev + level) * 2 * M;
   const float *__restrict__ p3r = e.pt3d_ref + (size_t)b * 3 * M;
-  float *T = e.T + (size_t)b * M * 64;
-  float *Gx = e.Gx + (size_t)b * M * 64;
-  float *Gy = e.Gy + (size_t)b * M * 64;
-  float *coefb = e.coef + (size_t)b * M * kCoefStride;
+  const LevelBufs lb = level_bufs(e, level), sb = stale_bufs(e, level);
+  const bool stale_copy = sb.T != lb.T;
+  float *T = lb.T + (size_t)b * M * 64;
+  float *Gx = lb.Gx + (size_t)b * M * 64;
+  float *Gy = lb.Gy + (size_t)b * M * 64;
+  float *coefb = lb.coef + (size_t)b * M * kCoefStride;
+  const float *Ts = sb.T + (size_t)b * M * 64;
+  const float *Gxs = sb.Gx + (size_t)b * M * 64;
+  const float *Gys = sb.Gy + (size_t)b * M * 64;
+  const float *coefs = sb.coef + (size_t)b * M * kCoefStride;
   gconst_f32 pref = (gconst_f32)pl.ref;
   gconst_f32x4 ppack = (gconst_f32x4)pl.pack;
   const int sw = lc.sw;
@@ -728,7 +734,9 @@
       c4[1] = make_float4(cx[4], cx[5], cy[0], cy[1]);
       c4[2] = make_float4(cy[2], cy[3], cy[4], cy[5]);
     } else {
-      const float4 a0 = c4[0], a1 = c4[1], a2 = c4[2];
+      const float4 *s4 = reinterpret_cast<const float4 *>(coefs + (size_t)ip * kCoefStride);
+      const float4 a0 = s4[0], a1 = s4[1], a2 = s4[2];
+      if (stale_copy && pv) c4[0] = a0, c4[1] = a1, c4[2] = a2;
       cx[0] = a0.x; cx[1] = a0.y; cx[2] = a0.z; cx[3] = a0.w; cx[4] = a1.x; cx[5] = a1.y;
       cy[0] = a1.z; cy[1] = a1.w; cy[2] = a2.x; cy[3] = a2.y; cy[4] = a2.z; cy[5] = a2.w;
     }
@@ -864,7 +872,13 @@
     for (unsigned long long stale = __builtin_amdgcn_ballot_w64(pv && !vis); stale; stale &= stale - 1) {
       const int j = __builtin_ctzll(stale);
       const size_t po = (size_t)(i0 + j) * 64;
-      patch_sums((Gx + po)[lane], (Gy + po)[lane], j);
+      const float gxs = (Gxs + po)[lane], gys = (Gys + po)[lane];
+      if (stale_copy) {
+        (T + po)[lane] = (Ts + po)[lane];
+        (Gx + po)[lane] = gxs;
+        (Gy + po)[lane] = gys;
+      }
+      patch_sums(gxs, gys, j);
     }
     {
       const float4 k0 = rec4[lane * 4 + 1], k1 = rec4[lane * 4 + 2], k2 = rec4[lane * 4 + 3];
@@ -893,7 +907,7 @@
   __syncthreads();
   if (threadIdx.x < kHUnique) {
     const float v = (sW[0][threadIdx.x] + sW[1][threadIdx.x]) + (sW[2][threadIdx.x] + sW[3][threadIdx.x]);
-    e.partH[((size_t)b * gridDim.x + blockIdx.x) * kPartHStride + threadIdx.x] = v;
+    lb.partH[((size_t)b * gridDim.x + blockIdx.x) * kPartHStride + threadIdx.x] = v;
   }
 }
 
diff --git a/invcompcamtrack_amd/csrc/ictr_launch.h b/invcompcamtrack_amd/csrc/ictr_launch.h
--- a/invcompcamtrack_amd/csrc/ictr_launch.h
+++ b/invcompcamtrack_amd/csrc/ictr_launch.h
@@ -90,8 +90,8 @@
 size_t resident_mail_bytes(int parts, int slots);
 int resident_points_per_workgroup(int np);
 int resident_blocks_per_cu(int np);
-hipError_t launch_level_resident(const EngineDev &e, const LevelCam &lc, int level, const ResidentGeom &g, int nblk,
-                                 const Exchange &x, const ResXchg *xchg, hipStream_t s);
+hipError_t launch_level_resident(const EngineDev &e, const LevelCam *cams, const int *nblk, int lv_hi, int lv_lo,
+                                 const ResidentGeom &g, const Exchange &x, const ResXchg *xchg, hipStream_t s);
 hipError_t launch_debug_transpose_reduce(const float *vals, float *out, int *patch_of_lane, int *kind_of_lane, int np,
                                          hipStream_t s);
 
diff --git a/invcompcamtrack_amd/csrc/ictr_resident.hip b/invcompcamtrack_amd/csrc/ictr_resident.hip
--- a/invcompcamtrack_amd/csrc/ictr_resident.hip
+++ b/invcompcamtrack_amd/csrc/ictr_resident.hip
@@ -20,11 +20,12 @@
 #endif
 constexpr int kResD = ICTR_RES_D;
 
+constexpr int kResMaxLevels = 16;
 struct ResArgs {
-  LevelCam lc;
-  int level;
+  LevelCam lc[kResMaxLevels];
+  int nblk[kResMaxLevels];
+  int lv_hi, lv_lo;
   int parts, slots;
-  int nblk;
   int dbg_mute;
   int prof_slot;
   ResXchg x;
@@ -248,19 +249,23 @@
     __shared__ float sH[32];
     for (int b = slot, round = 0; b < e.B; b += a.slots, ++round) {
       const ProbState &gst = e.st[b];
-      int active = ((0 < e.maxiter) & (1.0f > e.ratio)) ? 1 : 0;
+      const int active0 = ((0 < e.maxiter) & (1.0f > e.ratio)) ? 1 : 0;
       {
         const unsigned *src = reinterpret_cast<const unsigned *>(&gst);
         unsigned *dst = reinterpret_cast<unsigned *>(&sSt);
         for (int i = tid; i < (int)(sizeof(ProbState) / 4); i += kResThreads) dst[i] = src[i];
       }
+      unsigned xs = 0;
+      for (int level = a.lv_hi; level >= a.lv_lo; --level) {
+      int active = active0;
+      const int nblk = a.nblk[level];
       {
         const int j = tid & 31, sl = tid >> 5;
         double sacc = 0.0;
-        const float *ph = e.partH + (size_t)b * a.nblk * kPartHStride + j;
+        const float *ph = level_bufs(e, level).partH + (size_t)b * nblk * kPartHStride + j;
         if (j < kHUnique) {
 #pragma unroll 8
-          for (int k = sl; k < a.nblk; k += kResThreads / 32) sacc += (double)ph[(size_t)k * kPartHStride];
+          for (int k = sl; k < nblk; k += kResThreads / 32) sacc += (double)ph[(size_t)k * kPartHStride];
         }
         sRedH[sl][j] = sacc;
       }
@@ -272,7 +277,6 @@
         sH[tid] = (float)sacc;
       }
       __syncthreads();
-      unsigned xs = 0;
       if (wave == 0) {
         float hl = lane < kHUnique ? sH[lane] : 0.0f;
         if (a.x.world > 1) {
@@ -337,7 +341,7 @@
           float G[12];
           ws_load_state(S, sSt, lane, G);
           ws_load_factor(S, sSt, lane);
-          ws_iterate(S, (float)bsum, sopt, a.level, b, lane, G);
+          ws_iterate(S, (float)bsum, sopt, level, b, lane, G);
           ws_store_state(S, sSt, lane, G);
           float gv = 0.0f;
 #pragma unroll
@@ -358,8 +362,9 @@
         __syncthreads();
         active = __builtin_amdgcn_readfirstlane(__builtin_bit_cast(int, sG[12]));
       }
+      if (wave == 0 && a.x.world > 1 && lane == 0) a.x.xseq[b] = xs;
+      }
       if (wave == 0) {
-        if (a.x.world > 1 && lane == 0) a.x.xseq[b] = xs;
         const unsigned *src = reinterpret_cast<const unsigned *>(&sSt);
         unsigned *dst = reinterpret_cast<unsigned *>(e.st + b);
         for (int i = lane; i < (int)(sizeof(ProbState) / 4); i += 64) dst[i] = src[i];
@@ -373,10 +378,6 @@
     return;
   }
 
-  const LevelCam lc = a.lc;
-  const int sw = lc.sw;
-  const unsigned off_cd = (unsigned)((lane >> 3) * sw + (lane & 7)) * 4u;
-  const unsigned off_ab = off_cd + (unsigned)sw * 4u;
   float4 *const recs = sRecW[wave];
   float *const tw = sT[wave] + lane;
   const int my_patch = tr_patch_of_lane<NP>(lane);
@@ -385,23 +386,34 @@
     res_setprio((slot + round) & 3);
     const ProbState &gst = e.st[b];
     const int npts = gst.npts;
-    int active = ((0 < e.maxiter) & (1.0f > e.ratio)) ? 1 : 0;
-    if (!active) continue;
+    if (!((0 < e.maxiter) & (1.0f > e.ratio))) continue;
     const int i0 = part * kResQ + wave * kResPPW;
     const int cnt = min(kResPPW, max(0, npts - i0));
+    const bool pv = lane < cnt;
+    float X = 0.0f, Y = 0.0f, Z = 1.0f;
+    if (pv) {
+      const float *p3 = e.pt3d + (size_t)b * 3 * M;
+      X = p3[i0 + lane], Y = p3[i0 + lane + M], Z = p3[i0 + lane + 2 * M];
+    }
+    for (int level = a.lv_hi; level >= a.lv_lo; --level) {
+    const LevelCam lc = a.lc[level];
+    const int sw = lc.sw;
+    const unsigned off_cd = (unsigned)((lane >> 3) * sw + (lane & 7)) * 4u;
+    const unsigned off_ab = off_cd + (unsigned)sw * 4u;
+    const LevelBufs lb = level_bufs(e, level);
+    int active = 1;
     const float *cur_plane;
     {
-      const unsigned long long pc64 = reinterpret_cast<unsigned long long>(e.planes[b * e.nlev + a.level].cur);
+      const unsigned long long pc64 = reinterpret_cast<unsigned long long>(e.planes[b * e.nlev + level].cur);
       const unsigned lo = __builtin_amdgcn_readfirstlane((unsigned)pc64), hi = __builtin_amdgcn_readfirstlane((unsigned)(pc64 >> 32));
       cur_plane = reinterpret_cast<const float *>(((unsigned long long)hi << 32) | lo);
     }
     const __amdgpu_buffer_rsrc_t rcur =
         __builtin_amdgcn_make_buffer_rsrc(const_cast<float *>(cur_plane), 0, 0x7fffffff, 0x00020000);
     f32x2_t Gxy[kResPPW];
-    const float *gT = e.T + ((size_t)b * M + i0) * 64 + lane;
-    const float *gGx = e.Gx + ((size_t)b * M + i0) * 64 + lane;
-    const float *gGy = e.Gy + ((size_t)b * M + i0) * 64 + lane;
-    const bool pv = lane < cnt;
+    const float *gT = lb.T + ((size_t)b * M + i0) * 64 + lane;
+    const float *gGx = lb.Gx + ((size_t)b * M + i0) * 64 + lane;
+    const float *gGy = lb.Gy + ((size_t)b * M + i0) * 64 + lane;
     float c6[6] = {0.0f, 0.0f, 0.0f, 0.0f, 0.0f, 0.0f};
     const int nbytes = __builtin_amdgcn_readfirstlane(cnt * 256);
     auto bounded = [&](const float *q) {
@@ -426,16 +438,11 @@
       for (int u = 0; u < 8; ++u) tw[(j0 + u) * 64] = t8[u];
     }
     if (my_patch < cnt && tr_primary_lane<NP>(lane)) {
-      const float *cl = e.coef + ((size_t)b * M + i0 + my_patch) * kCoefStride + (my_kind ? 6 : 0);
+      const float *cl = lb.coef + ((size_t)b * M + i0 + my_patch) * kCoefStride + (my_kind ? 6 : 0);
 #pragma unroll
       for (int k = 0; k < 6; ++k) c6[k] = cl[k];
     }
-    float X = 0.0f, Y = 0.0f, Z = 1.0f;
-    if (pv) {
-      const float *p3 = e.pt3d + (size_t)b * 3 * M;
-      X = p3[i0 + lane], Y = p3[i0 + lane + M], Z = p3[i0 + lane + 2 * M];
-    }
-    if (tid < 12) sG[tid] = gst.G[tid];
+    if (level == a.lv_hi && tid < 12) sG[tid] = gst.G[tid];
     __syncthreads();
 
     while (active) {
@@ -501,7 +508,9 @@
       RES_MARK(2)
       RES_STAMP(tr_row, tr_it, 1)
       {
-        const float val = F * lane_gather(vis_f, my_patch);
+        int lane_p = lane;
+        asm volatile("" : "+v"(lane_p));
+        const float val = F * lane_gather(vis_f, tr_patch_of_lane<NP>(lane_p));
         float o = 0.0f;
 #pragma unroll
         for (int k = 0; k < 6; ++k) {
@@ -539,6 +548,7 @@
     }
     RES_MARK(5)
     __syncthreads();
+    }
   }
 #ifdef ICTR_RES_PROF
   if (slot == a.prof_slot && part == 0 && tid == 0)
@@ -574,9 +584,11 @@
   static const int n[2] = {res_occupancy<16>(), res_occupancy<32>()};
   return n[np == 32 ? 1 : 0];
 }
-hipError_t launch_level_resident(const EngineDev &e, const LevelCam &lc, int level, const ResidentGeom &g, int nblk,
-                                 const Exchange &x, const ResXchg *xchg, hipStream_t s) {
+hipError_t launch_level_resident(const EngineDev &e, const LevelCam *cams, const int *nblk, int lv_hi, int lv_lo,
+                                 const ResidentGeom &g, const Exchange &x, const ResXchg *xchg, hipStream_t s) {
+  if (lv_lo < 0 || lv_hi < lv_lo || lv_hi >= kResMaxLevels) return hipErrorInvalidValue;
   ResArgs a;
+  memset(&a, 0, sizeof(a));
   if (xchg)
     a.x = *xchg;
   else
@@ -585,9 +597,12 @@
     const char *ps = getenv("ICTR_RES_PROF_SLOT");
     a.prof_slot = ps ? atoi(ps) : 0;
   }
-  a.nblk = nblk;
-  a.lc = lc;
-  a.level = level;
+  for (int l = lv_lo; l <= lv_hi; ++l) {
+    a.lc[l] = cams[l];
+    a.nblk[l] = nblk[l];
+  }
+  a.lv_hi = lv_hi;
+  a.lv_lo = lv_lo;
   a.parts = g.parts;
   a.slots = g.slots;
   a.dbg_mute = x.mute;
diff --git a/invcompcamtrack_amd/tracker.py b/invcompcamtrack_amd/tracker.py
--- a/invcompcamtrack_amd/tracker.py
+++ b/invcompcamtrack_amd/tracker.py
@@ -250,7 +250,9 @@
     name = {0: "k_iter* (per-iteration launches)", 1: "k_track1 (one launch per tracking)",
             2: "k_iter* (per-iteration launches replayed as one hipGraph)",
             3: "k_track1 (one launch per tracking, begin phase and read-back included)",
-            4: "k_level_resident (one launch per level: all iterations, templates resident in registers)"}.get(form, "?")
+            4: "k_level_resident (one launch per level: all iterations, templates resident in registers)",
+            5: "k_level_resident (one launch per tracking: all iterations of all levels, templates resident in "
+               "registers)"}.get(form, "?")
     return name + (f" x {team} workgroups per problem" if team > 1 else "")
 
 
@@ -364,6 +366,9 @@
     def set_team(self, target_points, min_points=0, max_points=1 << 30):
         check(_lib.load().ictr_batch_set_team(self._h, int(target_points), int(min_points), int(max_points)))
 
+    def set_level_launches(self, on=True):
+        check(_lib.load().ictr_batch_set_level_launches(self._h, int(bool(on))))
+
     def set_peer_exchange(self, p2p_handle):
         check(_lib.load().ictr_batch_set_peer_exchange(self._h, p2p_handle))
 
diff --git a/profiles/recompute_roofline.py b/profiles/recompute_roofline.py
--- a/profiles/recompute_roofline.py
+++ b/profiles/recompute_roofline.py
@@ -80,14 +80,16 @@
                 groups.append([i, i])
             groups[-1][1] = i
             prev = i
-    res = [(e - s) for (s, e, k, gy, _) in (rows[groups[0][1]:groups[1][0]] if len(groups) >= 2 else rows)
-           if k == "k_level_res"]
+    window = rows[groups[0][1]:groups[1][0]] if len(groups) >= 2 else rows
+    res = [(e - s) for (s, e, k, gy, _) in window if k == "k_level_res"]
     if res:
         mean = sum(res) / len(res)
-        byts = 16.0 * 64 * points * res_pairs * maxiter
+        nref = sum(1 for (s, e, k, gy, _) in window if k == "k_ref8")
+        levels = max(1, round(nref / len(res)))
+        byts = 16.0 * 64 * points * res_pairs * maxiter * levels
         rate = byts / (mean * 1e-9)
         print(f"{'k_level_resident, headline':28s} {len(res):6d} launches, mean {mean / 1e3:8.2f} us, {byts / 1e9:.2f} GB "
-              f"algorithmic per launch ({res_pairs} pairs x {maxiter} iterations): {rate / 1e9:8.1f} GB/s equivalent = "
+              f"algorithmic per launch ({res_pairs} pairs x {maxiter} iterations x {levels} level(s)): {rate / 1e9:8.1f} GB/s equivalent = "
               f"{rate / PEAK:.4f} of 8 TB/s")
         print(f"roofline.frac = {rate / PEAK:.4f}   (headline kernel k_level_resident)")
         print(f"roofline.streaming_kernel.frac = {frac:.4f}   (k_iter8, solo leg)")
```
